# zhizdev/mvdfusion

Hardware: AMD Instinct MI355X
Metric: denoising-steps/sec (higher is better)
Workload: dtype f16x3 (f16 MFMA operands split hi+lo, 3 partial products, fp32 accumulate); 1 GPU; BASELINE.json configs[1]: V=4 views x 256^2 images (32x32 latents), D=1, 50-step DDIM (eta 1), cfg 2.5, SD1.x UNet 320ch + 10 view-aligned transformers + GridAttn, random-init (deterministic fill) weights; views=4, latent=32, depth_samples=1, parallelism=single GPU, CFG pair batched as 2V, hipgraph=True, gemm_tuning=mvdfusion_amd/tuned/gemm_f16.json: 426 problems; 0 problems tuned in this run

## Files before the change

include/mvd_hip.h:

```cpp
#ifndef MVD_HIP_H
#define MVD_HIP_H
#include <stddef.h>
#include <stdint.h>
#ifdef __cplusplus
extern "C" {
#endif

typedef void* mvd_stream_t;

#define MVD_VERSION 100
#define MVD_PREC_X1 1
#define MVD_PREC_X3 3
#define MVD_PREC_X4 4

int mvd_version(void);
const char* mvd_last_error(void);
int mvd_operand_format(void);

size_t mvd_packed_weight_bytes(int N, int K);
int mvd_pack_linear_weight(const float* w, int N, int K, int ldw, int geglu, float scale, void* packed,
                           mvd_stream_t stream);
int mvd_pack_linear_weight_t(const float* wt, int N, int K, int ldw, float scale, void* packed, mvd_stream_t stream);
int mvd_pack_conv3x3_weight(const float* w, int Cout, int Cin, int cin_pad, float scale, void* packed,
                            mvd_stream_t stream);

#define MVD_A_DENSE 0
#define MVD_A_CONV3X3 1

#define MVD_EPI_STORE 0
#define MVD_EPI_GEGLU 1
#define MVD_EPI_QKV 2

#define MVD_ACT_NONE 0
#define MVD_ACT_GELU 1
#define MVD_ACT_SILU 2
#define MVD_ACT_QUICKGELU 3

#define MVD_GEMM_TILES 5
#define MVD_GEMM_LOOPS 8
#define MVD_GEMM_CFG_STRIDE 32
#define MVD_B_PACKED 0
#define MVD_B_PLANES 1

typedef struct mvd_prefetch_item_s {
  const void* ptr;
  unsigned long long bytes;
  int start_after;
  int consumer;
} mvd_prefetch_item;

typedef struct mvd_gemm_desc {
  int M, N, K;
  const void* A;
  int lda;
  int a_mode;
  int B, Hin, Win, Cin, Hout, Wout, stride, upsample;
  int no_pad_tl;
  const void* Wp;
  int b_mode;
  int ldb;
  float acc_scale;
  int prec;
  int epi;
  int act;
  float* out;
  int ldo;
  void* out_sp;
  int ldp;
  int n_store;
  const float* bias;
  const float* bias_b;
  int rows_per_batch;
  int ldbb;
  const float* colscale;
  const float* res;
  int ldr;
  void *q_hi, *q_lo, *k_hi, *k_lo, *vt_hi, *vt_lo;
  int heads, dhead, L, Lpad;
  float qscale;
  int splitk;
  float* workspace;
  size_t workspace_elems;
  int cfg;
  long long* gn_stats;
  int gn_hw, gn_groups;
  float* rs_out;
  int* rs_count;
  int rs_ld;
  const float* ln_stats;
  const int* ln_count;
  const float* ln_colsum;
  int ln_ld, ln_dim;
  float ln_eps;
  void* gna_out_sp;
  const float* gna_gamma;
  const float* gna_beta;
  float gna_eps;
  int gna_flags;
  const float* cat_b;
  int cat_cb;
  void* cat_raw_sp;
  const float* acc_scale_dev;
  const struct mvd_prefetch_item_s* pf_items;
  int pf_n;
  int tap_mode;
  const void* A2;
  int lda2, Cin2;
} mvd_gemm_desc;
#define MVD_TAPS_FULL 0
#define MVD_TAPS_UP4 1
#define MVD_TAPS_CENTRE_TAIL 2
#define MVD_GNA_SILU 1
#define MVD_GNA_ROUND_F16 2
#define MVD_GNA_OUT_UNUSED 4

int mvd_gemm(const mvd_gemm_desc* d, mvd_stream_t stream);
int mvd_gemm_cfg_supported(const mvd_gemm_desc* d, int cfg);

int mvd_split_planes(const float* x, void* sp, size_t rows, int cols, int ldx, int ldp, mvd_stream_t stream);
int mvd_split_planes_scaled(const float* x, void* sp, size_t rows, int cols, int ldx, int ldp, const float* scale_dev, mvd_stream_t stream);

int mvd_gemv(const float* W, const float* bias, const float* x, float* y, int M, int N, int K, int ldx, int ldy,
             int act_in, int act_out, mvd_stream_t stream);

int mvd_groupnorm_chunks(int HW);
int mvd_groupnorm_nhwc(const float* x, void* y_sp, const float* gamma, const float* beta, int B, int HW, int C,
                       int groups, float eps, int silu, double* ws, size_t ws_elems, mvd_stream_t stream);
int mvd_groupnorm_from_stats(const float* x, void* y_sp, const float* gamma, const float* beta, const long long* stats, int B, int HW,
                             int C, int groups, float eps, int silu, mvd_stream_t stream);
int mvd_softmax_rows(const float* x, void* y_sp, int rows, int cols, int ldx, float scale, float out_scale,
                     mvd_stream_t stream);

int mvd_layernorm(const float* x, void* y_sp, float* y_f32, const float* w, const float* b, int rows, int C, float eps,
                  int w_plus_one, mvd_stream_t stream);
int mvd_layernorm_groups(const float* x, void* y_sp, float* y_f32, const float* w, const float* b, int ldw, int rows, int rows_per_group,
                         int C, float eps, int w_plus_one, mvd_stream_t stream);

size_t mvd_attn_qk_plane_elems(int B, int heads, int L, int dhead);
size_t mvd_attn_vt_plane_elems(int B, int heads, int L, int dhead);
int mvd_attn_lpad(int L);
int mvd_attention(const void* q_hi, const void* q_lo, const void* k_hi, const void* k_lo, const void* vt_hi,
                  const void* vt_lo, void* out_sp, int ldo, int B, int heads, int L, int Lkeys, int dhead, int prec,
                  mvd_stream_t stream);

int mvd_pixel_cross_attn(const float* q, const float* k, const float* v, void* out_sp, int P, int D, int heads,
                         int dhead, mvd_stream_t stream);

int mvd_unet_input(const float* x, const float* input_latents, void* out_sp, int V, int S, int cpad, int cfg,
                   mvd_stream_t stream);
int mvd_unet_input_scenes(const float* x, const float* input_latents, void* out_sp, int nscene, int V, int S, int cpad, int cfg,
                          mvd_stream_t stream);
int mvd_concat_channels(const float* a, int Ca, const float* b, int Cb, float* out, void* out_sp, int rows, long long* gn_stats,
                        int gn_hw, int gn_groups, mvd_stream_t stream);
int mvd_concat_groupnorm_fits(int Ca, int Cb, int hw, int groups);
int mvd_concat_groupnorm(const float* a, int Ca, const float* b, int Cb, float* out, void* raw_sp, void* y_sp, const float* gamma,
                         const float* beta, long long* gn_stats, int B, int hw, int groups, float eps, int silu, mvd_stream_t stream);
int mvd_area_pool(const float* vol, void* out_sp, int B, int S, int D, int C, int factor, int ldp, mvd_stream_t stream);
int mvd_fill_zero(float* p, size_t n, mvd_stream_t stream);

#define MVD_STEP_STRIDE 8
int mvd_timestep_embedding(const float* steps, const int* iter, const float* freqs, float* out, int dim,
                           mvd_stream_t stream);
int mvd_timestep_embedding_scenes(const float* steps, const int* iter, const float* freqs, float* out, int dim, int nscene,
                                  int steps_scene_stride, mvd_stream_t stream);
int mvd_advance_iter(int* iter, mvd_stream_t stream);

#define MVD_CAM_RECORD 20
#define MVD_TOKEN_DIM 723
#define MVD_TOKEN_LD 736
int mvd_zembed(const float* lat, const float* w, const float* b, float* feat, int N, int S, mvd_stream_t stream);
int mvd_gridattn_tokens(const float* x, const float* depth_noise, const float* steps, const int* iter,
                        const float* grid_lin ,
                        const float* feat, const float* in_feat, const float* cams, const float* in_cam,
                        void* tokens_sp, int V, int q0, int Vq, int S, int D, float depth_scale, float depth_shift,
                        mvd_stream_t stream);
int mvd_gridattn_tokens_scenes(const float* x, const float* depth_noise, const float* steps, const int* iter, const float* grid_lin,
                               const float* feat, const float* in_feat, const float* cams, const float* in_cam, void* tokens_sp,
                               int nscene, int V, int q0, int Vq, int S, int D, float depth_scale, float depth_shift,
                               mvd_stream_t stream);
int mvd_gridattn_tokens_scenes_t(const float* x, const float* depth_noise, const float* steps, const int* iter, const float* grid_lin,
                                 const float* feat, const float* in_feat, const float* cams, const float* in_cam, void* tokens_sp,
                                 int nscene, int V, int q0, int Vq, int S, int D, float depth_scale, float depth_shift,
                                 int steps_scene_stride, mvd_stream_t stream);
int mvd_gridattn_fused_slots(void);
size_t mvd_gridattn_fused_stream_bytes(void);
size_t mvd_gridattn_fused_vec_floats(void);
int mvd_gridattn_fused(const float* x, const float* depth_noise, const float* steps, const int* iter, const float* grid_lin,
                       const float* feat, const float* in_feat, const float* cams, const float* in_cam, const void* wstream,
                       const float* vecs, void* pooled_sp, int V, int q0, int Vq, int S, int D, float depth_scale,
                       float depth_shift, int prec ,
                       mvd_stream_t stream);
int mvd_gridattn_fused_scenes(const float* x, const float* depth_noise, const float* steps, const int* iter, const float* grid_lin,
                              const float* feat, const float* in_feat, const float* cams, const float* in_cam, const void* wstream,
                              const float* vecs, void* pooled_sp, int nscene, int V, int q0, int Vq, int S, int D, float depth_scale,
                              float depth_shift, int prec, mvd_stream_t stream);
int mvd_gridattn_fused_scenes_t(const float* x, const float* depth_noise, const float* steps, const int* iter, const float* grid_lin,
                                const float* feat, const float* in_feat, const float* cams, const float* in_cam, const void* wstream,
                                const float* vecs, void* pooled_sp, int nscene, int V, int q0, int Vq, int S, int D, float depth_scale,
                                float depth_shift, int prec, int steps_scene_stride, int vecs_scene_stride, mvd_stream_t stream);
int mvd_gridattn_tokens_window(const float* x, const float* depth_noise, const float* steps, const int* iter, const float* grid_lin,
                               const float* feat, const float* in_feat, const float* cams, const float* in_cam, void* tokens_sp,
                               int nscene, int V, int q0, int Vq, int S, int D, float depth_scale, float depth_shift,
                               int steps_scene_stride, int window, mvd_stream_t stream);
int mvd_gridattn_fused_window(const float* x, const float* depth_noise, const float* steps, const int* iter, const float* grid_lin,
                              const float* feat, const float* in_feat, const float* cams, const float* in_cam, const void* wstream,
                              const float* vecs, void* pooled_sp, int nscene, int V, int q0, int Vq, int S, int D, float depth_scale,
                              float depth_shift, int prec, int steps_scene_stride, int vecs_scene_stride, int window,
                              mvd_stream_t stream);
int mvd_view_mha(const float* qkv, void* out_sp, int Nseq, int V, int heads, int dhead,
                 mvd_stream_t stream);
int mvd_view_pool(const float* x, const float* w, const float* b, void* out_sp, int Nseq, int V, int C,
                  mvd_stream_t stream);

int mvd_cfg_ddim_update(const float* eps_nhwc, int ldc, float* x, float* x0, float* eps_out,
                        const float* ddim_noise, size_t noise_stride ,
                        const float* steps, const int* iter, int V, int S, int cfg, float cfg_scale, int do_update,
                        mvd_stream_t stream);

int mvd_pin_views(float* x, float* x0, const float* known, const float* noise, size_t noise_stride ,
                  const float* steps, const int* iter, int groups, int group_views, int K, int S, int mode, mvd_stream_t stream);

#define MVD_FUSE_FOREGROUND 1
#define MVD_FUSE_STAGE_AUTO 0
#define MVD_FUSE_STAGE_GLOBAL 1
#define MVD_FUSE_STAGE_LDS 2
int mvd_fuse_points(const float* lat, const float* rgb, const float* cams, const float* ndc_lin, float* xyz, float* color,
                    uint8_t* support, uint8_t* conflict, uint8_t* flags, int nscene, int V, int S, int up, float depth_scale,
                    float depth_shift, float lo, float hi, float tau, int stage, mvd_stream_t stream);
size_t mvd_compact_points_scratch(size_t npts);
int mvd_compact_points(const float* xyz, const float* color, const uint8_t* support, const uint8_t* conflict, const uint8_t* flags,
                       size_t npts, int min_support, int max_conflicts, float* out_xyz, float* out_color, uint8_t* out_support,
                       int* out_index, unsigned* count, void* scratch, size_t scratch_bytes, mvd_stream_t stream);

#define MVD_SPLAT_MAX_RADIUS 4
#define MVD_RENDER_FILL 1
#define MVD_RENDER_SPLAT 2
#define MVD_RENDER_RESOLVE 4
#define MVD_RENDER_ALL 7
size_t mvd_render_points_scratch(int ncam, int P);
int mvd_render_points(const float* xyz, const float* color, const int* scene_start, const float* cams, size_t n, int nscene, int M, int P,
                      int radius, float znear, float empty_depth, const float* background, int* index, float* depth, float* rgb,
                      void* scratch, size_t scratch_bytes, mvd_stream_t stream);
int mvd_render_points_stages(const float* xyz, const float* color, const int* scene_start, const float* cams, size_t n, int nscene, int M,
                             int P, int radius, float znear, float empty_depth, const float* background, int* index, float* depth,
                             float* rgb, void* scratch, size_t scratch_bytes, int stages, mvd_stream_t stream);

size_t mvd_render_mesh_scratch(int ncam, int P);
int mvd_render_mesh(const float* vertices, const float* colors, const int* faces, const int* vertex_start, const int* face_start,
                    const float* cams, size_t nvert, size_t nface, int nscene, int M, int P, int cull, float znear, float empty_depth,
                    const float* background, int* face_out, float* depth, float* bary, float* normal, float* rgb, void* scratch,
                    size_t scratch_bytes, mvd_stream_t stream);
int mvd_render_mesh_stages(const float* vertices, const float* colors, const int* faces, const int* vertex_start, const int* face_start,
                           const float* cams, size_t nvert, size_t nface, int nscene, int M, int P, int cull, float znear,
                           float empty_depth, const float* background, int* face_out, float* depth, float* bary, float* normal, float* rgb,
                           void* scratch, size_t scratch_bytes, int stages, mvd_stream_t stream);

#define MVD_NN_AUTO 0
#define MVD_NN_BRUTE 1
#define MVD_NN_GRID 2
#define MVD_NN_BUILD 1
#define MVD_NN_QUERY 2
#define MVD_NN_ALL 3
size_t mvd_nearest_points_scratch(size_t nt, int nscene, int method, int grid);
int mvd_nearest_points(const float* query, const int* query_start, const float* target, const int* target_start, size_t nq, size_t nt,
                       int nscene, int method, int grid, int* index, float* dist2, void* scratch, size_t scratch_bytes,
                       mvd_stream_t stream);
int mvd_nearest_points_stages(const float* query, const int* query_start, const float* target, const int* target_start, size_t nq,
                              size_t nt, int nscene, int method, int grid, int* index, float* dist2, void* scratch, size_t scratch_bytes,
                              int stages, mvd_stream_t stream);

#define MVD_KNN_MAX_K 32
#define MVD_NORMALS_MAX_K 256
#define MVD_NORMALS_SWEEPS 10
int mvd_knn_points(const float* query, const int* query_start, const float* target, const int* target_start, size_t nq, size_t nt,
                   int nscene, int k, int method, int grid, int* index, float* dist2, void* scratch, size_t scratch_bytes,
                   mvd_stream_t stream);
int mvd_knn_points_stages(const float* query, const int* query_start, const float* target, const int* target_start, size_t nq, size_t nt,
                          int nscene, int k, int method, int grid, int* index, float* dist2, void* scratch, size_t scratch_bytes,
                          int stages, mvd_stream_t stream);
int mvd_point_normals(const float* target, size_t nt, const int* index, size_t n, int k, const float* points, const float* toward,
                      float* normal, float* variation, mvd_stream_t stream);

#define MVD_ALIGN_SCALE 1
#define MVD_ALIGN_NO_STEP 2
#define MVD_ALIGN_CHUNK 1024
#define MVD_ALIGN_SUMS 19
#define MVD_ALIGN_HISTORY 3
#define MVD_ALIGN_MAX_ITERS 1024
size_t mvd_align_scratch(size_t nq, size_t nt, int nscene, int method, int grid);
int mvd_align_solve(const double* sums, int flags, double* step, double* scale);
int mvd_align_apply(const float* src, const int* src_start, size_t n, int nscene, const double* transform, float* out,
                    mvd_stream_t stream);
int mvd_align_fit(const float* moved, const int* start, const float* target, const int* index, const float* dist2, size_t n, size_t nt,
                  int nscene, int flags, float max_dist2, double* transform, double* history_row, void* scratch, size_t scratch_bytes,
                  mvd_stream_t stream);
int mvd_align_icp(const float* source, const int* source_start, const float* target, const int* target_start, size_t nq, size_t nt,
                  int nscene, int method, int grid, int iters, int flags, float max_dist2, double* transform, double* history,
                  float* moved, int* index, float* dist2, void* scratch, size_t scratch_bytes, mvd_stream_t stream);

#define MVD_PLANE_NO_STEP 2
#define MVD_PLANE_SUMS 30
#define MVD_PLANE_HISTORY 4
#define MVD_PLANE_EPS_RANK 1e-9
size_t mvd_plane_scratch(size_t nq, size_t nt, int nscene, int method, int grid);
int mvd_plane_solve(const double* sums, double* step, int* rank);
int mvd_plane_fit(const float* moved, const int* start, const float* target, const float* normals, const int* index, const float* dist2,
                  size_t n, size_t nt, int nscene, int flags, float max_dist2, double* transform, double* history_row, void* scratch,
                  size_t scratch_bytes, mvd_stream_t stream);
int mvd_plane_icp(const float* source, const int* source_start, const float* target, const int* target_start, const float* normals,
                  size_t nq, size_t nt, int nscene, int method, int grid, int iters, float max_dist2, double* transform, double* history,
                  float* moved, int* index, float* dist2, void* scratch, size_t scratch_bytes, mvd_stream_t stream);

#define MVD_MESH_SPAN 3
size_t mvd_nearest_on_mesh_scratch(size_t nf, int nscene, int method, int grid);
int mvd_nearest_on_mesh(const float* query, const int* query_start, const float* vertices, const int* faces, const int* face_start, size_t nq,
                        size_t nv, size_t nf, int nscene, int method, int grid, int* face, float* dist2, float* point, float* bary,
                        int* region, float* normal, void* scratch, size_t scratch_bytes, mvd_stream_t stream);
int mvd_nearest_on_mesh_stages(const float* query, const int* query_start, const float* vertices, const int* faces, const int* face_start,
                               size_t nq, size_t nv, size_t nf, int nscene, int method, int grid, int* face, float* dist2, float* point,
                               float* bary, int* region, float* normal, void* scratch, size_t scratch_bytes, int stages,
                               mvd_stream_t stream);
size_t mvd_mesh_icp_scratch(size_t nq, size_t nf, int nscene, int method, int grid);
int mvd_mesh_icp(const float* source, const int* source_start, const float* vertices, const int* faces, const int* face_start, size_t nq,
                 size_t nv, size_t nf, int nscene, int method, int grid, int iters, float max_dist2, double* transform, double* history,
                 float* moved, int* face, float* dist2, float* point, float* normal, void* scratch, size_t scratch_bytes,
                 mvd_stream_t stream);

int mvd_tsdf_integrate(const float* lat, const float* rgb, const float* cams, float* tsdf, uint8_t* weight, float* color, uint8_t* cweight,
                       int nscene, int V, int S, int up, int G, float cx, float cy, float cz, float half_extent, float trunc, int carve,
                       float depth_scale, float depth_shift, float lo, float hi, mvd_stream_t stream);
size_t mvd_mesh_scratch(int nscene, int G);
int mvd_mesh_count(const float* tsdf, const uint8_t* weight, int nscene, int G, int* vertex_start, int* face_start, void* scratch,
                   size_t scratch_bytes, mvd_stream_t stream);
int mvd_mesh_emit(const float* tsdf, const uint8_t* weight, const float* color, const uint8_t* cweight, int nscene, int G, float cx, float cy,
                  float cz, float half_extent, const float* fill, float* vertices, float* colors, int* faces, size_t nvert, size_t nface,
                  const void* scratch, size_t scratch_bytes, mvd_stream_t stream);

int mvd_graph_begin(mvd_stream_t stream);
int mvd_graph_end(mvd_stream_t stream, void** graph_exec);
int mvd_graph_launch(void* graph_exec, mvd_stream_t stream);
int mvd_graph_destroy(void* graph_exec);
int mvd_event_create(void** ev);
int mvd_event_record(void* ev, mvd_stream_t stream);
int mvd_event_elapsed_ms(void* start, void* stop, float* ms);
int mvd_event_destroy(void* ev);

int mvd_transpose_planes(const void* x, int src_planes, int rows, int cols, int ldx, void* out_sp, int ldo, mvd_stream_t stream);
int mvd_transpose_planes_scaled(const float* x, int rows, int cols, int ldx, void* out_sp, int ldo, const float* scale_dev,
                                mvd_stream_t stream);
int mvd_im2col3x3_t_planes(const void* x_sp, int B, int H, int W, int Cin, void* out_sp, int ldo, mvd_stream_t stream);
int mvd_pow2_scale(const float* x, size_t n, float* out2, unsigned* scratch2, mvd_stream_t stream);
int mvd_adamw_multi(const void* tensors, int n_tensors, int n_chunks, float lr, float beta1, float beta2, float eps, float weight_decay,
                    float bias_c1, float bias_c2_sqrt, float grad_scale, mvd_stream_t stream);
size_t mvd_col_sum_workspace_doubles(int rows, int cols);
int mvd_col_sum(const float* x, int rows, int cols, int ldx, float* out, double* ws, size_t ws_doubles, mvd_stream_t stream);
int mvd_col_sum_pow2(const float* x, int rows, int cols, int ldx, float* out, double* ws, size_t ws_doubles, float* out2, unsigned* scratch1,
                     mvd_stream_t stream);
int mvd_groupnorm_backward(const float* x, const float* dy, const float* gamma, const float* beta, int B, int HW, int C, int groups,
                           float eps, int silu, float* dx, float* dgamma, float* dbeta, float* ws, size_t ws_floats,
                           mvd_stream_t stream);

int mvd_layernorm_backward(const float* x, const float* dy, const float* w, int rows, int C, float eps, float* dx, float* dyxhat,
                           mvd_stream_t stream);
size_t mvd_col_sum_groups_workspace_doubles(int ngroups, int rows_per_group, int cols);
int mvd_col_sum_groups(const float* x, int ngroups, int rows_per_group, int cols, int ldx, float* out, double* ws, size_t ws_doubles,
                       mvd_stream_t stream);
int mvd_layernorm_backward_groups(const float* x, const float* dy, const float* w, int ldw, int rows, int rows_per_group, int C, float eps,
                                  float* dx, float* dyxhat, float* dw, float* db, double* ws, size_t ws_doubles, mvd_stream_t stream);
int mvd_act_planes(const float* x, void* sp, float* y, size_t rows, int cols, int ldx, int ldp, int ldy, int act, mvd_stream_t stream);
int mvd_act_backward(const float* dy, const float* x, float* dx, size_t n, int act, mvd_stream_t stream);
int mvd_geglu_backward(const float* h, const float* dy, int rows, int half, float* dh, mvd_stream_t stream);
int mvd_attention_backward(const float* q, const float* k, const float* v, const float* dout, int B, int heads, int L, int dhead,
                           float* dq, float* dk, float* dv, float* stats, size_t stats_floats, mvd_stream_t stream);
int mvd_pixel_cross_attn_backward(const float* q, const float* k, const float* v, const float* dout, int P, int D, int heads, int dhead,
                                  float* dq, float* dk, float* dv, mvd_stream_t stream);

int mvd_gridattn_tokens_backward(const float* x, const float* depth_noise, const float* steps, const int* iter, const float* grid_lin,
                                 const float* cams, const float* in_cam, const float* dtok, int ldt, long long* dfeat_acc,
                                 long long* din_feat_acc, float scale, int V, int q0, int Vq, int S, int D, float depth_scale,
                                 float depth_shift, mvd_stream_t stream);
int mvd_gridattn_tokens_backward_scenes(const float* x, const float* depth_noise, const float* steps, const int* iter, const float* grid_lin,
                                        const float* cams, const float* in_cam, const float* dtok, int ldt, long long* dfeat_acc,
                                        long long* din_feat_acc, float scale, int nscene, int V, int q0, int Vq, int S, int D,
                                        float depth_scale, float depth_shift, int steps_scene_stride, mvd_stream_t stream);
int mvd_gridattn_tokens_backward_window(const float* x, const float* depth_noise, const float* steps, const int* iter, const float* grid_lin,
                                        const float* cams, const float* in_cam, const float* dtok, int ldt, long long* dfeat_acc,
                                        long long* din_feat_acc, float scale, int nscene, int V, int q0, int Vq, int S, int D,
                                        float depth_scale, float depth_shift, int steps_scene_stride, int window, mvd_stream_t stream);

#ifdef __cplusplus
}
#endif
#endif
```

mvdfusion_amd/csrc/elementwise.hip:

```cpp
#include "common.hpp"
#include "../../include/mvd_hip.h"

namespace {

__device__ __forceinline__ float act_apply(float v, int act) {
  if (act == MVD_ACT_GELU) return gelu_erf(v);
  if (act == MVD_ACT_SILU) return silu_f(v);
  return v;
}

template <int MR>
__global__ __launch_bounds__(256) void gemv_kernel(const float* __restrict__ W, const float* __restrict__ bias,
                                                   const float* __restrict__ x, float* __restrict__ y, int M, int N, int K, int ldx,
                                                   int ldy, int act_in, int act_out) {
  const int lane = threadIdx.x & 63;
  const int n = blockIdx.x * 4 + (threadIdx.x >> 6);
  if (n >= N) return;
  float acc[MR];
#pragma unroll
  for (int m = 0; m < MR; ++m) acc[m] = 0.f;
  const float* wr = W + (size_t)n * K;
  if ((K & 3) == 0) {
    for (int k = lane * 4; k < K; k += 256) {
      const float4 w4 = *(const float4*)(wr + k);
#pragma unroll
      for (int m = 0; m < MR; ++m) {
        if (m < M) {
          float4 x4 = *(const float4*)(x + (size_t)m * ldx + k);
          if (act_in) {
            x4.x = act_apply(x4.x, act_in);
            x4.y = act_apply(x4.y, act_in);
            x4.z = act_apply(x4.z, act_in);
            x4.w = act_apply(x4.w, act_in);
          }
          acc[m] += w4.x * x4.x + w4.y * x4.y + w4.z * x4.z + w4.w * x4.w;
        }
      }
    }
  } else {
    for (int k = lane; k < K; k += 64) {
      const float w1 = wr[k];
#pragma unroll
      for (int m = 0; m < MR; ++m)
        if (m < M) acc[m] += w1 * act_apply(x[(size_t)m * ldx + k], act_in);
    }
  }
#pragma unroll
  for (int m = 0; m < MR; ++m) {
    if (m < M) {
      float v = wave_sum(acc[m]);
      if (lane == 0) {
        if (bias) v += bias[n];
        y[(size_t)m * ldy + n] = act_apply(v, act_out);
      }
    }
  }
}

__global__ __launch_bounds__(256) void unet_input_kernel(const float* __restrict__ x, const float* __restrict__ il,
                                                         u16* __restrict__ out_sp, int V, int Vs, int S, int cpad, int nb) {
  const int SS = S * S;
  const size_t total = (size_t)nb * SS * cpad;
  for (size_t e = (size_t)blockIdx.x * 256 + threadIdx.x; e < total; e += (size_t)gridDim.x * 256) {
    const int c = (int)(e % cpad);
    const int pix = (int)((e / cpad) % SS);
    const int b = (int)(e / ((size_t)cpad * SS));
    const int v = b < V ? b : b - V;
    float o = 0.f;
    if (c < 5) {
      o = x[((size_t)v * 5 + c) * SS + pix];
    } else if (c < 10 && b < V) {
      const float t = il[((size_t)(b / Vs) * 5 + (c - 5)) * SS + pix];
      o = (c < 9) ? t / 0.18215f : t;
    }
    store_sp1(out_sp, e / cpad, cpad, c, o);
  }
}

__global__ __launch_bounds__(256) void concat_kernel(const float4* __restrict__ a, int ca4, const float4* __restrict__ b, int cb4,
                                                     float4* __restrict__ out, u16* __restrict__ out_sp, size_t rows) {
  const int c4 = ca4 + cb4;
  const size_t total = rows * c4;
  for (size_t e = (size_t)blockIdx.x * 256 + threadIdx.x; e < total; e += (size_t)gridDim.x * 256) {
    const size_t r = e / c4;
    const int c = (int)(e - r * c4);
    const float4 v = c < ca4 ? a[r * ca4 + c] : b[r * cb4 + (c - ca4)];
    out[e] = v;
    if (out_sp) store_sp4(out_sp, r, c4 * 4, c * 4, v.x, v.y, v.z, v.w);
  }
}

__global__ __launch_bounds__(256) void concat_stats_kernel(const float4* __restrict__ a, int ca4, const float4* __restrict__ b, int cb4,
                                                           float4* __restrict__ out, u16* __restrict__ out_sp, long long* __restrict__ stats,
                                                           int hw, int groups) {
  __shared__ float cs[2][4][256];
  const int c4n = ca4 + cb4, C = c4n * 4;
  const size_t m0 = (size_t)blockIdx.x * 16;
  const int n0 = blockIdx.y * 256;
  const int c4 = blockIdx.y * 64 + (threadIdx.x & 63), rg = threadIdx.x >> 6;
  float4 s = make_float4(0.f, 0.f, 0.f, 0.f), q = make_float4(0.f, 0.f, 0.f, 0.f);
  if (c4 < c4n) {
    float4 v[4];
#pragma unroll
    for (int r = 0; r < 4; ++r) {
      const size_t row = m0 + rg * 4 + r;
      v[r] = c4 < ca4 ? a[row * ca4 + c4] : b[row * cb4 + (c4 - ca4)];
    }
#pragma unroll
    for (int r = 0; r < 4; ++r) {
      const size_t row = m0 + rg * 4 + r;
      out[row * c4n + c4] = v[r];
      if (out_sp) store_sp4(out_sp, row, C, c4 * 4, v[r].x, v[r].y, v[r].z, v[r].w);
      s.x += v[r].x; s.y += v[r].y; s.z += v[r].z; s.w += v[r].w;
      q.x += v[r].x * v[r].x; q.y += v[r].y * v[r].y; q.z += v[r].z * v[r].z; q.w += v[r].w * v[r].w;
    }
  }
  *(float4*)&cs[0][rg][(threadIdx.x & 63) * 4] = s;
  *(float4*)&cs[1][rg][(threadIdx.x & 63) * 4] = q;
  __syncthreads();
  const int c = threadIdx.x, nn = n0 + c;
  const float cs_ = cs[0][0][c] + cs[0][1][c] + cs[0][2][c] + cs[0][3][c];
  const float cq_ = cs[1][0][c] + cs[1][1][c] + cs[1][2][c] + cs[1][3][c];
  __syncthreads();
  cs[0][0][c] = cs_;
  cs[1][0][c] = cq_;
  __syncthreads();
  if (nn >= C) return;
  const int cg = C / groups;
  const int g = nn / cg, pos = nn - g * cg;
  if (c != 0 && pos != 0) return;
  int len = cg - pos;
  if (len > 256 - c) len = 256 - c;
  float ss = 0.f, qq = 0.f;
  for (int j = 0; j < len; ++j) {
    ss += cs[0][0][c + j];
    qq += cs[1][0][c + j];
  }
  gn_stats_add(stats, (int)(m0 / hw), g, groups, ss, qq);
}

#define MVD_CGN_THREADS 1024
__global__ __launch_bounds__(MVD_CGN_THREADS) void concat_gn_kernel(const float* __restrict__ a, int ca, const float* __restrict__ b, int cb,
                                                                    float* __restrict__ out, u16* __restrict__ raw_sp, u16* __restrict__ y_sp,
                                                                    const float* __restrict__ gamma, const float* __restrict__ beta,
                                                                    long long* __restrict__ stats, int hw, int groups, float eps, int flags) {
  constexpr int NT = MVD_CGN_THREADS, NWV = NT / 64, U = 4;
  extern __shared__ float s_val[];
  __shared__ double s_red[2][NWV];
  __shared__ float s_coef[2][128];
  const int C = ca + cb, cg = C / groups, cg2 = cg >> 1;
  int g, img;
  {
    const int bid = blockIdx.x;
    if ((groups & 7) == 0) {
      const int gpx = groups >> 3, x = bid & 7, r = bid >> 3;
      g = x * gpx + r % gpx;
      img = r / gpx;
    } else {
      g = bid % groups;
      img = bid / groups;
    }
  }
  const int tid = threadIdx.x, lane = tid & 63, wave = tid >> 6;
  const int c0 = g * cg;
  const size_t m0 = (size_t)img * hw;
  const int total = hw * cg2;
  const int dq = NT / cg2, dj = NT - dq * cg2;
  const int rs = tid / cg2, js = tid - rs * cg2;
  const int r0 = tid < total ? rs : 0, j0 = tid < total ? js : 0;
  float s = 0.f, q = 0.f;
  {
    int r = rs, j = js;
    for (int e0 = tid; e0 < total; e0 += NT * U) {
      float2 v[U];
      int rr[U], jj[U];
      bool ok[U];
#pragma unroll
      for (int u = 0; u < U; ++u) {
        ok[u] = e0 + u * NT < total;
        rr[u] = ok[u] ? r : r0;
        jj[u] = ok[u] ? j : j0;
        r += dq;
        j += dj;
        if (j >= cg2) {
          j -= cg2;
          ++r;
        }
      }
#pragma unroll
      for (int u = 0; u < U; ++u) {
        const size_t m = m0 + rr[u];
        const int n = c0 + 2 * jj[u];
        v[u] = *(const float2*)(n < ca ? a + m * ca + n : b + m * cb + (n - ca));
      }
#pragma unroll
      for (int u = 0; u < U; ++u) {
        if (ok[u]) {
          const size_t m = m0 + rr[u];
          const int n = c0 + 2 * jj[u];
          if (out) *(float2*)(out + m * C + n) = v[u];
          if (raw_sp) {
            uint32_t hh, ll;
            split_op16x2(v[u].x, v[u].y, hh, ll);
            u16* pp = raw_sp + sp_index(m, C, n);
            *(uint32_t*)pp = hh;
            *(uint32_t*)(pp + 32) = ll;
          }
          *(float2*)(s_val + 2 * (e0 + u * NT)) = v[u];
          s += v[u].x + v[u].y;
          q += v[u].x * v[u].x + v[u].y * v[u].y;
        }
      }
    }
  }
  {
    const double sd = wave_sum_d((double)s), qd = wave_sum_d((double)q);
    if (lane == 0) {
      s_red[0][wave] = sd;
      s_red[1][wave] = qd;
    }
  }
  __syncthreads();
  double S1 = 0.0, S2 = 0.0;
#pragma unroll
  for (int w = 0; w < NWV; ++w) {
    S1 += s_red[0][w];
    S2 += s_red[1][w];
  }
  const double cnt = (double)hw * cg;
  const double mean = S1 / cnt;
  double var = S2 / cnt - mean * mean;
  if (var < 0.0) var = 0.0;
  const float rstd = (float)(1.0 / sqrt(var + (double)eps));
  if (tid < cg) {
    const float aa = rstd * gamma[c0 + tid];
    s_coef[0][tid] = aa;
    s_coef[1][tid] = beta[c0 + tid] - (float)mean * aa;
  }
  if (tid == 0 && stats) gn_stats_add(stats, img, g, groups, (float)S1, (float)S2);
  __syncthreads();
  {
    int r = rs, j = js;
    for (int e = tid; e < total; e += NT) {
      float2 v = *(const float2*)(s_val + 2 * e);
      v.x = v.x * s_coef[0][2 * j] + s_coef[1][2 * j];
      v.y = v.y * s_coef[0][2 * j + 1] + s_coef[1][2 * j + 1];
      if (flags & 2) {
        v.x = (float)(_Float16)v.x;
        v.y = (float)(_Float16)v.y;
      }
      if (flags & 1) {
        v.x = silu_f(v.x);
        v.y = silu_f(v.y);
      }
      uint32_t hh, ll;
      split_op16x2(v.x, v.y, hh, ll);
      u16* pp = y_sp + sp_index(m0 + r, C, c0 + 2 * j);
      *(uint32_t*)pp = hh;
      *(uint32_t*)(pp + 32) = ll;
      r += dq;
      j += dj;
      if (j >= cg2) {
        j -= cg2;
        ++r;
      }
    }
  }
}

__global__ __launch_bounds__(256) void area_pool_kernel(const float4* __restrict__ vol, u16* __restrict__ out_sp, int B, int S,
                                                        int D, int C4, int f, int ldp) {
  const int So = S / f;
  const size_t total = (size_t)B * So * So * D * C4;
  const float inv = 1.0f / (float)(f * f);
  for (size_t e = (size_t)blockIdx.x * 256 + threadIdx.x; e < total; e += (size_t)gridDim.x * 256) {
    const int c = (int)(e % C4);
    size_t r = e / C4;
    const int d = (int)(r % D);
    r /= D;
    const int ox = (int)(r % So);
    r /= So;
    const int oy = (int)(r % So);
    const int b = (int)(r / So);
    float4 acc = make_float4(0.f, 0.f, 0.f, 0.f);
    for (int dy = 0; dy < f; ++dy)
#pragma unroll 8
      for (int dx = 0; dx < f; ++dx) {
        const float4 v = vol[((((size_t)b * S + oy * f + dy) * S + ox * f + dx) * D + d) * C4 + c];
        acc.x += v.x;
        acc.y += v.y;
        acc.z += v.z;
        acc.w += v.w;
      }
    store_sp4(out_sp, e / C4, ldp, c * 4, acc.x * inv, acc.y * inv, acc.z * inv, acc.w * inv);
  }
}

__global__ __launch_bounds__(256) void fill_zero_kernel(float* p, size_t n) {
  for (size_t e = (size_t)blockIdx.x * 256 + threadIdx.x; e < n; e += (size_t)gridDim.x * 256) p[e] = 0.f;
}

__global__ void timestep_embedding_kernel(const float* __restrict__ steps, const int* __restrict__ iter,
                                          const float* __restrict__ freqs, float* __restrict__ out, int dim, int steps_scene_stride) {
  const float t = steps[((size_t)iter[0] + (size_t)blockIdx.x * steps_scene_stride) * MVD_STEP_STRIDE + 0];
  out += (size_t)blockIdx.x * dim;
  const int half = dim / 2;
  for (int i = threadIdx.x; i < half; i += blockDim.x) {
    const float a = t * freqs[i];
    out[i] = cosf(a);
    out[half + i] = sinf(a);
  }
}

__global__ void advance_iter_kernel(int* iter) {
  if (threadIdx.x == 0) iter[0] += 1;
}

__global__ __launch_bounds__(256) void cfg_ddim_kernel(const float* __restrict__ eps_nhwc, int ldc, float* __restrict__ x,
                                                       float* __restrict__ x0, float* __restrict__ eps_out,
                                                       const float* __restrict__ noise, const float* __restrict__ steps,
                                                       const int* __restrict__ iter, int V, int S, int cfg, float cfg_scale,
                                                       int do_update, size_t noise_stride) {
  const int it = iter[0];
  const float* st = steps + (size_t)it * MVD_STEP_STRIDE;
  const float a_t = st[3], a_prev = st[4], sigma = st[5], s1m = st[6], has_noise = st[7];
  const int SS = S * S;
  const size_t total = (size_t)V * 5 * SS;
  for (size_t e = (size_t)blockIdx.x * 256 + threadIdx.x; e < total; e += (size_t)gridDim.x * 256) {
    const int pix = (int)(e % SS);
    const int c = (int)((e / SS) % 5);
    const int b = (int)(e / ((size_t)5 * SS));
    float ep = eps_nhwc[((size_t)b * SS + pix) * ldc + c];
    if (cfg) {
      const float eu = eps_nhwc[((size_t)(V + b) * SS + pix) * ldc + c];
      ep = eu + cfg_scale * (ep - eu);
    }
    if (eps_out) eps_out[e] = ep;
    if (do_update) {
      const float xv = x[e];
      const float px0 = (xv - s1m * ep) / sqrtf(a_t);
      const float dir = sqrtf(fmaxf(1.0f - a_prev - sigma * sigma, 1e-7f)) * ep;
      float xp = sqrtf(a_prev) * px0 + dir;
      if (has_noise != 0.f) xp = xp + sigma * noise[(size_t)it * noise_stride + e];
      x0[e] = px0;
      x[e] = xp;
    }
  }
}

template <typename T>
__device__ __forceinline__ T pin_axpy(float sa, const T& k, float s1, const T& n);
template <>
__device__ __forceinline__ float pin_axpy<float>(float sa, const float& k, float s1, const float& n) {
  return sa * k + s1 * n;
}
template <>
__device__ __forceinline__ float4 pin_axpy<float4>(float sa, const float4& k, float s1, const float4& n) {
  return make_float4(sa * k.x + s1 * n.x, sa * k.y + s1 * n.y, sa * k.z + s1 * n.z, sa * k.w + s1 * n.w);
}

template <typename T>
__global__ __launch_bounds__(256) void pin_views_kernel(T* __restrict__ x, T* __restrict__ x0, const T* __restrict__ known,
                                                        const T* __restrict__ noise, size_t nstride, const float* __restrict__ steps,
                                                        const int* __restrict__ iter, int group_views, int K, size_t rowlen, size_t total,
                                                        int mode) {
  float sa = 1.f, s1 = 0.f;
  size_t nbase = 0;
  if (mode == 1) {
    const int it = iter[0];
    const float* st = steps + (size_t)it * MVD_STEP_STRIDE;
    sa = st[1];
    s1 = st[6];
    nbase = (size_t)it * nstride;
  }
  for (size_t e = (size_t)blockIdx.x * 256 + threadIdx.x; e < total; e += (size_t)gridDim.x * 256) {
    const size_t p = e / rowlen;
    const size_t off = e - p * rowlen;
    const size_t dst = ((p / K) * group_views + p % K) * rowlen + off;
    const T kv = known[e];
    if (mode == 1) {
      x[dst] = pin_axpy<T>(sa, kv, s1, noise[nbase + e]);
      x0[dst] = kv;
    } else {
      x[dst] = kv;
    }
  }
}

inline int grid_for(size_t total, int cap = 2048) {
  size_t b = (total + 255) / 256;
  if (b > (size_t)cap) b = cap;
  if (b < 1) b = 1;
  return (int)b;
}

}

extern "C" int mvd_gemv(const float* W, const float* bias, const float* x, float* y, int M, int N, int K, int ldx, int ldy,
                        int act_in, int act_out, mvd_stream_t stream) {
  MVD_CHECK_ARG(W && x && y && M > 0 && M <= 16 && N > 0 && K > 0, "mvd_gemv: bad arguments (M <= 16)");
  if ((K & 3) == 0) MVD_CHECK_ARG((ldx & 3) == 0, "mvd_gemv: ldx must be a multiple of 4 when K is");
  hipStream_t s = (hipStream_t)stream;
  dim3 grid(cdiv(N, 4)), block(256);
  if (M <= 1)
    hipLaunchKernelGGL(gemv_kernel<1>, grid, block, 0, s, W, bias, x, y, M, N, K, ldx, ldy, act_in, act_out);
  else if (M <= 4)
    hipLaunchKernelGGL(gemv_kernel<4>, grid, block, 0, s, W, bias, x, y, M, N, K, ldx, ldy, act_in, act_out);
  else
    hipLaunchKernelGGL(gemv_kernel<16>, grid, block, 0, s, W, bias, x, y, M, N, K, ldx, ldy, act_in, act_out);
  MVD_CHECK_LAUNCH("mvd_gemv");
  return 0;
}

extern "C" int mvd_unet_input_scenes(const float* x, const float* input_latents, void* out_sp, int nscene, int V, int S, int cpad, int cfg,
                                     mvd_stream_t stream) {
  MVD_CHECK_ARG(x && input_latents && out_sp && cpad % 32 == 0 && V > 0 && S > 0 && cpad >= 10, "mvd_unet_input: bad arguments");
  MVD_CHECK_ARG(nscene >= 1 && (long long)nscene * V <= 0x3fffffff, "mvd_unet_input_scenes: nscene=%d (>= 1)", nscene);
  const int NV = nscene * V;
  const int nb = cfg ? 2 * NV : NV;
  const size_t total = (size_t)nb * S * S * cpad;
  hipLaunchKernelGGL(unet_input_kernel, dim3(grid_for(total)), dim3(256), 0, (hipStream_t)stream, x, input_latents, (u16*)out_sp, NV, V,
                     S, cpad, nb);
  MVD_CHECK_LAUNCH("mvd_unet_input");
  return 0;
}

extern "C" int mvd_unet_input(const float* x, const float* input_latents, void* out_sp, int V, int S, int cpad, int cfg,
                              mvd_stream_t stream) {
  return mvd_unet_input_scenes(x, input_latents, out_sp, 1, V, S, cpad, cfg, stream);
}

extern "C" int mvd_concat_channels(const float* a, int Ca, const float* b, int Cb, float* out, void* out_sp, int rows,
                                   long long* gn_stats, int gn_hw, int gn_groups, mvd_stream_t stream) {
  if (out_sp) MVD_CHECK_ARG((Ca + Cb) % 32 == 0, "mvd_concat_channels: split-planes output needs (Ca+Cb) %% 32 == 0");
  MVD_CHECK_ARG(a && b && out && rows > 0 && Ca > 0 && Cb > 0 && Ca % 4 == 0 && Cb % 4 == 0,
                "mvd_concat_channels: bad arguments (channel counts must be multiples of 4)");
  if (gn_stats) {
    MVD_CHECK_ARG(rows % 16 == 0 && gn_hw > 0 && gn_hw % 16 == 0 && gn_groups > 0 && (Ca + Cb) % gn_groups == 0,
                  "mvd_concat_channels: gn_stats needs rows %% 16 == 0, gn_hw %% 16 == 0, C %% groups == 0");
    hipLaunchKernelGGL(concat_stats_kernel, dim3(rows / 16, (Ca + Cb + 255) / 256), dim3(256), 0, (hipStream_t)stream, (const float4*)a, Ca / 4,
                       (const float4*)b, Cb / 4, (float4*)out, (u16*)out_sp, gn_stats, gn_hw, gn_groups);
    MVD_CHECK_LAUNCH("mvd_concat_channels/stats");
    return 0;
  }
  const size_t total = (size_t)rows * (Ca + Cb) / 4;
  hipLaunchKernelGGL(concat_kernel, dim3(grid_for(total)), dim3(256), 0, (hipStream_t)stream, (const float4*)a, Ca / 4,
                     (const float4*)b, Cb / 4, (float4*)out, (u16*)out_sp, (size_t)rows);
  MVD_CHECK_LAUNCH("mvd_concat_channels");
  return 0;
}

extern "C" int mvd_concat_groupnorm_fits(int Ca, int Cb, int hw, int groups) {
  const int C = Ca + Cb;
  if (groups <= 0 || C % groups || (Ca & 1) || (Cb & 1)) return 0;
  const int cg = C / groups;
  return (cg & 1) == 0 && cg <= 128 && (size_t)hw * cg * 4 <= 128 * 1024 ? 1 : 0;
}

extern "C" int mvd_concat_groupnorm(const float* a, int Ca, const float* b, int Cb, float* out, void* raw_sp, void* y_sp, const float* gamma,
                                    const float* beta, long long* gn_stats, int B, int hw, int groups, float eps, int silu,
                                    mvd_stream_t stream) {
  MVD_CHECK_ARG(a && b && y_sp && gamma && beta && B > 0 && hw > 0, "mvd_concat_groupnorm: null pointer / bad shape");
  MVD_CHECK_ARG((Ca + Cb) % 32 == 0 && mvd_concat_groupnorm_fits(Ca, Cb, hw, groups),
                "mvd_concat_groupnorm: needs (Ca+Cb) %% 32 == 0, even Ca / Cb / group width <= 128 and hw * (C / groups) * 4 <= 128 KiB of LDS "
                "(Ca=%d Cb=%d hw=%d groups=%d): use mvd_concat_channels + mvd_groupnorm_from_stats", Ca, Cb, hw, groups);
  MVD_CHECK_ARG(((uintptr_t)a & 7) == 0 && ((uintptr_t)b & 7) == 0 && ((uintptr_t)out & 7) == 0 && ((uintptr_t)y_sp & 127) == 0 &&
                    ((uintptr_t)raw_sp & 127) == 0, "mvd_concat_groupnorm: alignment");
  const size_t lds = (size_t)hw * ((Ca + Cb) / groups) * 4;
  {
    static unsigned long long raised = 0;
    const hipError_t e = mvd_raise_dynamic_lds((const void*)concat_gn_kernel, 128 * 1024, &raised);
    MVD_CHECK_ARG(e == hipSuccess, "mvd_concat_groupnorm: hipFuncSetAttribute(MaxDynamicSharedMemorySize): %s", hipGetErrorString(e));
  }
  hipLaunchKernelGGL(concat_gn_kernel, dim3(B * groups), dim3(MVD_CGN_THREADS), lds, (hipStream_t)stream, a, Ca, b, Cb, out, (u16*)raw_sp,
                     (u16*)y_sp, gamma, beta, gn_stats, hw, groups, eps, silu);
  MVD_CHECK_LAUNCH("mvd_concat_groupnorm");
  return 0;
}

extern "C" int mvd_area_pool(const float* vol, void* out_sp, int B, int S, int D, int C, int factor, int ldp,
                             mvd_stream_t stream) {
  MVD_CHECK_ARG(vol && out_sp && C % 32 == 0 && B > 0 && S > 0 && D > 0 && C % 4 == 0 && factor >= 1 && S % factor == 0,
                "mvd_area_pool: bad arguments");
  if (ldp == 0) ldp = C;
  MVD_CHECK_ARG(ldp >= C && ldp % 32 == 0 && ((uintptr_t)out_sp & 127) == 0, "mvd_area_pool: ldp=%d must be >= C, %% 32 == 0", ldp);
  const int So = S / factor;
  const size_t total = (size_t)B * So * So * D * (C / 4);
  hipLaunchKernelGGL(area_pool_kernel, dim3(grid_for(total)), dim3(256), 0, (hipStream_t)stream, (const float4*)vol,
                     (u16*)out_sp, B, S, D, C / 4, factor, ldp);
  MVD_CHECK_LAUNCH("mvd_area_pool");
  return 0;
}

extern "C" int mvd_fill_zero(float* p, size_t n, mvd_stream_t stream) {
  MVD_CHECK_ARG(p != nullptr, "mvd_fill_zero: null pointer");
  if (n == 0) return 0;
  hipLaunchKernelGGL(fill_zero_kernel, dim3(grid_for(n)), dim3(256), 0, (hipStream_t)stream, p, n);
  MVD_CHECK_LAUNCH("mvd_fill_zero");
  return 0;
}

extern "C" int mvd_timestep_embedding(const float* steps, const int* iter, const float* freqs, float* out, int dim,
                                      mvd_stream_t stream) {
  MVD_CHECK_ARG(steps && iter && freqs && out && dim > 0 && dim % 2 == 0, "mvd_timestep_embedding: bad arguments");
  hipLaunchKernelGGL(timestep_embedding_kernel, dim3(1), dim3(256), 0, (hipStream_t)stream, steps, iter, freqs, out, dim, 0);
  MVD_CHECK_LAUNCH("mvd_timestep_embedding");
  return 0;
}

extern "C" int mvd_timestep_embedding_scenes(const float* steps, const int* iter, const float* freqs, float* out, int dim, int nscene,
                                             int steps_scene_stride, mvd_stream_t stream) {
  MVD_CHECK_ARG(steps && iter && freqs && out && dim > 0 && dim % 2 == 0, "mvd_timestep_embedding: bad arguments");
  MVD_CHECK_ARG(nscene >= 1 && nscene <= 65535 && steps_scene_stride >= 0 && (nscene > 1 || steps_scene_stride == 0),
                "mvd_timestep_embedding_scenes: nscene=%d (1 ... 65535), steps_scene_stride=%d (>= 0; 0 when nscene = 1)", nscene,
                steps_scene_stride);
  hipLaunchKernelGGL(timestep_embedding_kernel, dim3(nscene), dim3(256), 0, (hipStream_t)stream, steps, iter, freqs, out, dim,
                     steps_scene_stride);
  MVD_CHECK_LAUNCH("mvd_timestep_embedding_scenes");
  return 0;
}

extern "C" int mvd_advance_iter(int* iter, mvd_stream_t stream) {
  MVD_CHECK_ARG(iter != nullptr, "mvd_advance_iter: null pointer");
  hipLaunchKernelGGL(advance_iter_kernel, dim3(1), dim3(64), 0, (hipStream_t)stream, iter);
  MVD_CHECK_LAUNCH("mvd_advance_iter");
  return 0;
}

extern "C" int mvd_cfg_ddim_update(const float* eps_nhwc, int ldc, float* x, float* x0, float* eps_out,
                                   const float* ddim_noise, size_t noise_stride, const float* steps, const int* iter, int V,
                                   int S, int cfg, float cfg_scale, int do_update, mvd_stream_t stream) {
  MVD_CHECK_ARG(eps_nhwc && steps && iter && V > 0 && S > 0 && ldc >= 5, "mvd_cfg_ddim_update: bad arguments");
  if (do_update) MVD_CHECK_ARG(x && x0 && ddim_noise, "mvd_cfg_ddim_update: update needs x, x0, ddim_noise");
  const size_t total = (size_t)V * 5 * S * S;
  hipLaunchKernelGGL(cfg_ddim_kernel, dim3(grid_for(total)), dim3(256), 0, (hipStream_t)stream, eps_nhwc, ldc, x, x0, eps_out,
                     ddim_noise, steps, iter, V, S, cfg, cfg_scale, do_update, noise_stride);
  MVD_CHECK_LAUNCH("mvd_cfg_ddim_update");
  return 0;
}

extern "C" int mvd_pin_views(float* x, float* x0, const float* known, const float* noise, size_t noise_stride, const float* steps,
                             const int* iter, int groups, int group_views, int K, int S, int mode, mvd_stream_t stream) {
  MVD_CHECK_ARG(x && known && groups > 0 && group_views > 0 && S > 0 && (mode == 0 || mode == 1),
                "mvd_pin_views: bad arguments (null x / known, groups=%d, group_views=%d, S=%d, mode=%d)", groups, group_views, S, mode);
  MVD_CHECK_ARG(K > 0 && K <= group_views, "mvd_pin_views: K=%d pinned views of a %d-view group (0 < K <= group_views)", K, group_views);
  MVD_CHECK_ARG((long long)groups * group_views <= 0x3fffffff, "mvd_pin_views: groups * group_views too large");
  const size_t row = (size_t)5 * S * S;
  if (mode == 1)
    MVD_CHECK_ARG(x0 && noise && steps && iter && noise_stride >= (size_t)groups * K * row,
                  "mvd_pin_views: mode 1 needs x0, noise, steps, iter and noise_stride >= groups * K * 5 * S * S");
  const size_t total = (size_t)groups * K * row;
  hipStream_t s = (hipStream_t)stream;
  if (((size_t)S * S) % 4 == 0) {
    MVD_CHECK_ARG(((uintptr_t)x & 15) == 0 && ((uintptr_t)known & 15) == 0, "mvd_pin_views: x / known must be 16-byte aligned");
    if (mode == 1)
      MVD_CHECK_ARG(((uintptr_t)x0 & 15) == 0 && ((uintptr_t)noise & 15) == 0 && noise_stride % 4 == 0,
                    "mvd_pin_views: x0 / noise must be 16-byte aligned and noise_stride a multiple of 4");
    hipLaunchKernelGGL(pin_views_kernel<float4>, dim3(grid_for(total / 4)), dim3(256), 0, s, (float4*)x, (float4*)x0, (const float4*)known,
                       (const float4*)noise, noise_stride / 4, steps, iter, group_views, K, row / 4, total / 4, mode);
  } else {
    hipLaunchKernelGGL(pin_views_kernel<float>, dim3(grid_for(total)), dim3(256), 0, s, x, x0, known, noise, noise_stride, steps, iter,
                       group_views, K, row, total, mode);
  }
  MVD_CHECK_LAUNCH("mvd_pin_views");
  return 0;
}
```

mvdfusion_amd/engine.py:

```python
import os

import torch

from . import hip


GN_SLOTS = 256
GN_SLOT_ELEMS = 64 * 32 * 2


class Workspace:

    def __init__(self, device):
        self.device = torch.device(device)
        self.bufs = {}
        self.frozen = False

    def get(self, tag, shape, dtype=torch.float32, zero=False):
        key = (tag, tuple(int(s) for s in shape), dtype)
        t = self.bufs.get(key)
        if t is None:
            assert not self.frozen, f"workspace buffer {key} requested during graph capture (the eager warm-up step must " \
                                    "allocate every buffer the captured step uses)"
            t = (torch.zeros if zero else torch.empty)(key[1], dtype=dtype, device=self.device)
            self.bufs[key] = t
        return t

    def planes(self, tag, rows, cols):
        assert cols % 32 == 0, (tag, cols)
        return self.get(tag, (rows, 2 * cols), torch.int16)

    def attn_planes(self, B, heads, L, dhead):
        key = ("attn_planes", B, heads, L, dhead)
        t = self.bufs.get(key)
        if t is None:
            assert not self.frozen, f"attention planes {key} requested during graph capture"
            t = hip.alloc_attn_planes(B, heads, L, dhead, self.device)
            self.bufs[key] = t
        return t

    def nbytes(self):
        n = 0
        for v in self.bufs.values():
            for t in (v if isinstance(v, tuple) else (v,)):
                n += t.numel() * t.element_size()
        return n


class Ctx:
    gn_from_producer = True
    ln_fold = True
    gn_fuse = True

    def __init__(self, device, prec=hip.PREC_X4, policy=None):
        self.device = torch.device(device)
        self.ws = Workspace(device)
        self.prec = prec
        self.policy = dict(policy or {})
        self.B = 0
        self.D = 1
        self.context = None
        self.vol_levels = None
        self.emb_bias = None
        self._rot = {}
        self.capturing = False
        self.gemm_ws = torch.empty(64 * 1024 * 1024, dtype=torch.float32, device=self.device)
        self.gn_arena = torch.zeros(GN_SLOTS * GN_SLOT_ELEMS, dtype=torch.int64, device=self.device)
        self._gn_next = 0
        self._gn = {}
        self._rs = {}
        self.next_gn = None
        self._gn_done = {}
        self._unwritten = set()
        self.next_cat = None
        self._cat_done = set()
        self.keep_fp32 = False

    def begin_step(self):
        self._rot.clear()
        self._gn.clear()
        self._gn_done.clear()
        self._unwritten.clear()
        self._cat_done.clear()
        self.next_gn = None
        self.next_cat = None
        self._gn_next = 0
        if self.gn_from_producer:
            hip.check(hip.lib().mvd_fill_zero(hip.ptr(self.gn_arena), self.gn_arena.numel() * 2, hip.stream()))

    def gn_slot(self, out, B, HW, C):
        n = B * 32 * 2
        if n > GN_SLOT_ELEMS or self._gn_next >= GN_SLOTS:
            return None
        st = self.gn_arena[self._gn_next * GN_SLOT_ELEMS:self._gn_next * GN_SLOT_ELEMS + n]
        self._gn_next += 1
        self._gn[out.data_ptr()] = (st, B, HW, C)
        return st

    def _forget(self, out):
        ptr = out.data_ptr()
        self._gn.pop(ptr, None)
        self._unwritten.discard(ptr)
        if self._gn_done:
            for k in [k for k in self._gn_done if k[0] == ptr]:
                del self._gn_done[k]

    def row_stats(self, tag, rows, width):
        key = (tag, int(rows), int(width))
        rs = self._rs.get(key)
        if rs is None:
            assert not self.ws.frozen, f"row statistics {key} requested during graph capture"
            rs = hip.RowStats(rows, width, self.device)
            self._rs[key] = rs
        return rs

    def act(self, shape):
        key = tuple(int(s) for s in shape)
        i = self._rot.get(key, 0)
        self._rot[key] = (i + 1) % 3
        return self.ws.get(f"act{i}", key)

    def prec_of(self, kind):
        return self.policy.get(kind, self.prec)

    def ln_fold_enabled(self):
        return (self.ln_fold and hip.OPERAND_FORMAT == "f16" and self.prec_of("qkv") >= hip.PREC_X3 and
                self.prec_of("geglu") >= hip.PREC_X3 and self.prec_of("proj") >= hip.PREC_X3)

    def gemm(self, A, W, out, gn=None, kind=None, gn_apply=None, **kw):
        kw.setdefault("prec", self.prec_of(kind))
        kw.setdefault("workspace", self.gemm_ws)
        applied = False
        if out is not None:
            self._forget(out)
            handled = False
            if gn is not None and gn_apply is None and self.next_cat is not None and self.gn_fuse and self.gn_from_producer and \
                    gn[1] % 16 == 0 and out.is_contiguous():
                sk, cat, catp, norm, pname, silu = self.next_cat
                N, cb = out.shape[-1], sk.shape[-1]
                if norm.num_groups == 32 and norm.num_channels == N + cb and sk.shape[0] == out.shape[0] == gn[0] * gn[1] and \
                        sk.is_contiguous() and hip.lib().mvd_concat_groupnorm_fits(N, cb, gn[1], 32):
                    st = self.gn_slot(cat, gn[0], gn[1], N + cb)
                    if st is not None:
                        planes = self.ws.planes(pname, out.shape[0], N + cb)
                        kw.update(gn_stats=st, gn_hw=gn[1], gn_groups=32, cat=(sk, catp),
                                  gn_apply=(norm.weight, norm.bias, norm.eps, (hip.GNA_SILU if silu else 0) | hip.GNA_OUT_UNUSED, planes))
                        self._gn.pop(cat.data_ptr(), None)
                        self._gn_done[(cat.data_ptr(), id(norm))] = (planes, bool(silu))
                        self._unwritten.add(cat.data_ptr())
                        self._unwritten.add(out.data_ptr())
                        self._cat_done.add(cat.data_ptr())
                        handled = True
            if not handled and gn is not None and self.gn_from_producer and gn[1] % 16 == 0 and out.shape[-1] % 32 == 0:
                st = self.gn_slot(out, gn[0], gn[1], out.shape[-1])
                if st is not None:
                    kw.update(gn_stats=st, gn_hw=gn[1], gn_groups=32)
                    if gn_apply is not None and self.gn_fuse and gn_apply[0].num_groups == 32 and out.is_contiguous():
                        norm, planes, silu, unused = gn_apply
                        kw["gn_apply"] = (norm.weight, norm.bias, norm.eps, (hip.GNA_SILU if silu else 0) | (hip.GNA_OUT_UNUSED if unused else 0),
                                          planes)
                        applied = True
                    elif gn_apply is None and self.next_gn is not None and self.gn_fuse and out.is_contiguous():
                        norm, pname, silu = self.next_gn
                        if norm.num_groups == 32 and norm.num_channels == out.shape[-1] and out.shape[0] == gn[0] * gn[1]:
                            planes = self.ws.planes(pname, out.shape[0], out.shape[-1])
                            kw["gn_apply"] = (norm.weight, norm.bias, norm.eps, hip.GNA_SILU if silu else 0, planes)
                            self._gn_done[(out.data_ptr(), id(norm))] = (planes, bool(silu))
        if gn is not None:
            if os.environ.get("MVD_GN_DEBUG") and not self.capturing:
                print(f"[gn] kind={kind} M={out.shape[0]} N={out.shape[-1]} explicit={gn_apply is not None} hint={self.next_gn is not None} "
                      f"cat={self.next_cat is not None} -> fused_apply={'gn_apply' in kw} cat={'cat' in kw}", flush=True)
            if gn_apply is None:
                self.next_gn = None
                self.next_cat = None
        r = hip.gemm(A, W, out, **kw)
        if gn_apply is not None and not applied:
            self.groupnorm(out, gn_apply[1], gn_apply[0], gn[0], gn[1], out.shape[-1], gn_apply[2])
        return r

    def groupnorm(self, x, y, norm, B, HW, C, silu):
        done = self._gn_done.pop((x.data_ptr(), id(norm)), None)
        if done is not None and done[0].data_ptr() == y.data_ptr() and done[0].shape == y.shape and done[1] == bool(silu) and silu in (True, False):
            return y
        if x.data_ptr() in self._unwritten:
            raise RuntimeError("GroupNorm of a tensor whose fused producer left the fp32 data unwritten (Ctx.concat(need_out=False))")
        ent = self._gn.get(x.data_ptr())
        if ent is not None and ent[1:] == (B, HW, C) and norm.num_groups == 32:
            return hip.groupnorm_from_stats(x, y, norm.weight, norm.bias, ent[0], B, HW, C, norm.eps, silu)
        ws = self.ws.get("gn_ws", (B * hip.lib().mvd_groupnorm_chunks(HW) * 32 * 2,), torch.float64)
        return hip.groupnorm(x, y, norm.weight, norm.bias, B, HW, C, norm.eps, silu, ws)

    def concat(self, a, ca, b, cb, out, out_planes, B, HW, gn_apply=None, need_out=True):
        self._forget(out)
        st = None
        if gn_apply is not None and self.gn_fuse and self.gn_from_producer and HW % 16 == 0 and (ca + cb) % 32 == 0 and \
                gn_apply[0].num_groups == 32 and gn_apply[0].num_channels == ca + cb and \
                hip.lib().mvd_concat_groupnorm_fits(ca, cb, HW, 32):
            norm, pname, silu = gn_apply
            st = self.gn_slot(out, B, HW, ca + cb)
            planes = self.ws.planes(pname, B * HW, ca + cb)
            hip.check(hip.lib().mvd_concat_groupnorm(hip.ptr(a), ca, hip.ptr(b), cb, hip.ptr(out) if need_out else None, hip.ptr(out_planes),
                                                     hip.ptr(planes), hip.ptr(norm.weight), hip.ptr(norm.bias),
                                                     hip.ptr(st) if st is not None else None, B, HW, 32, norm.eps, 1 if silu else 0,
                                                     hip.stream()))
            if not need_out:
                self._gn.pop(out.data_ptr(), None)
                self._unwritten.add(out.data_ptr())
            self._gn_done[(out.data_ptr(), id(norm))] = (planes, bool(silu))
            return out
        if self.gn_from_producer and HW % 16 == 0 and (ca + cb) % 32 == 0:
            st = self.gn_slot(out, B, HW, ca + cb)
        hip.check(hip.lib().mvd_concat_channels(hip.ptr(a), ca, hip.ptr(b), cb, hip.ptr(out), hip.ptr(out_planes), B * HW,
                                                hip.ptr(st) if st is not None else None, HW, 32, hip.stream()))
        return out

    def layernorm(self, x, y, norm, rows, C):
        return hip.layernorm(x, y, norm.weight, norm.bias, rows, C, norm.eps)

    def gemv_rows(self, W, bias, x, y, act_in=hip.ACT_NONE, act_out=hip.ACT_NONE):
        for r in range(0, x.shape[0], 16):
            hip.gemv(W, bias, x[r:r + 16], y[r:r + 16], act_in, act_out)
        return y


def ddim_step_table(scheduler_tables, ddim, iters):
    rows = []
    for index in iters:
        t = int(ddim["timesteps"][index])
        sac = float(scheduler_tables["sqrt_alphas_cumprod"][t])
        s1m = float(scheduler_tables["sqrt_one_minus_alphas_cumprod"][t])
        dstd = (scheduler_tables["sqrt_one_minus_alphas_cumprod"][t] / scheduler_tables["sqrt_alphas_cumprod"][t] / 10.0)
        rows.append([float(t), sac, float(dstd), float(ddim["alphas"][index]), float(ddim["alphas_prev"][index]),
                     float(ddim["sigmas"][index]), float(ddim["sqrt_one_minus_alphas"][index]),
                     1.0 if index > 0 else 0.0])
        del s1m
    return torch.tensor(rows, dtype=torch.float32)
```

mvdfusion_amd/hip.py:

```python
import ctypes as C
import os

import torch

_HERE = os.path.dirname(os.path.abspath(__file__))
LIB_PATHS = {"f16": os.path.join(_HERE, "csrc", "libmvd_hip.so"), "bf16": os.path.join(_HERE, "csrc", "libmvd_hip_bf16.so")}
if os.environ.get("MVD_HIP_LIB"):
    LIB_PATHS["f16"] = os.environ["MVD_HIP_LIB"]
LIB_PATH = LIB_PATHS["f16"]
OPERAND_FORMAT = os.environ.get("MVD_OPERAND_FORMAT", "f16")

PREC_X1, PREC_X3, PREC_X4 = 1, 3, 4
PREC_KINDS = ("conv", "skip", "proj", "qkv", "attn", "out", "geglu", "ffproj", "xattn", "ga")


def parse_precision(name):
    base, _, over = name.partition(":")
    names = {"f16": ("f16", PREC_X1), "bf16": ("bf16", PREC_X1), "f16x3": ("f16", PREC_X3), "f16x4": ("f16", PREC_X4),
             "bf16x3": ("bf16", PREC_X3), "bf16x4": ("bf16", PREC_X4)}
    if base not in names:
        raise ValueError(f"precision '{name}': base must be one of {sorted(names)}")
    fmt, default = names[base]
    policy = {}
    for item in filter(None, over.split(",")):
        k, _, v = item.partition("=")
        k = k.strip()
        if k not in PREC_KINDS or int(v) not in (PREC_X1, PREC_X3, PREC_X4):
            raise ValueError(f"precision policy '{name}': '{item}' is not <kind>=<1|3|4> with kind in {PREC_KINDS}")
        policy[k] = int(v)
    return fmt, default, policy
A_DENSE, A_CONV3X3 = 0, 1
TAPS_FULL, TAPS_CENTRE_TAIL = 0, 2
TAPS_UP4 = 1
EPI_STORE, EPI_GEGLU, EPI_QKV = 0, 1, 2
ACT_NONE, ACT_GELU, ACT_SILU, ACT_QUICKGELU = 0, 1, 2, 3
STEP_STRIDE = 8
CAM_RECORD = 20
TOKEN_DIM, TOKEN_LD = 723, 736
FUSE_FOREGROUND = 1
FUSE_STAGE_AUTO, FUSE_STAGE_GLOBAL, FUSE_STAGE_LDS = 0, 1, 2
SPLAT_MAX_RADIUS = 4
RENDER_FILL, RENDER_SPLAT, RENDER_RESOLVE, RENDER_ALL = 1, 2, 4, 7
NN_AUTO, NN_BRUTE, NN_GRID = 0, 1, 2
NN_BUILD, NN_QUERY, NN_ALL = 1, 2, 3
NN_MAX_GRID = 256
KNN_MAX_K = 32
NORMALS_MAX_K, NORMALS_SWEEPS = 256, 10
ALIGN_SCALE, ALIGN_NO_STEP = 1, 2
ALIGN_CHUNK = 1024
ALIGN_SUMS, ALIGN_HISTORY = 19, 3
PLANE_NO_STEP = 2
PLANE_SUMS, PLANE_HISTORY = 30, 4
PLANE_EPS_RANK = 1e-9
ALIGN_MAX_ITERS = 1024
MESH_SPAN = 3

_vp, _i, _f, _sz = C.c_void_p, C.c_int, C.c_float, C.c_size_t
c_void_p = C.c_void_p


class GemmDesc(C.Structure):
    _fields_ = [
        ("M", _i), ("N", _i), ("K", _i),
        ("A", _vp), ("lda", _i), ("a_mode", _i),
        ("B", _i), ("Hin", _i), ("Win", _i), ("Cin", _i), ("Hout", _i), ("Wout", _i), ("stride", _i), ("upsample", _i), ("no_pad_tl", _i),
        ("Wp", _vp), ("b_mode", _i), ("ldb", _i), ("acc_scale", _f), ("prec", _i),
        ("epi", _i), ("act", _i), ("out", _vp), ("ldo", _i), ("out_sp", _vp), ("ldp", _i),
        ("n_store", _i),
        ("bias", _vp), ("bias_b", _vp), ("rows_per_batch", _i), ("ldbb", _i), ("colscale", _vp), ("res", _vp), ("ldr", _i),
        ("q_hi", _vp), ("q_lo", _vp), ("k_hi", _vp), ("k_lo", _vp), ("vt_hi", _vp), ("vt_lo", _vp),
        ("heads", _i), ("dhead", _i), ("L", _i), ("Lpad", _i), ("qscale", _f),
        ("splitk", _i), ("workspace", _vp), ("workspace_elems", _sz), ("cfg", _i),
        ("gn_stats", _vp), ("gn_hw", _i), ("gn_groups", _i),
        ("rs_out", _vp), ("rs_count", _vp), ("rs_ld", _i),
        ("ln_stats", _vp), ("ln_count", _vp), ("ln_colsum", _vp), ("ln_ld", _i), ("ln_dim", _i), ("ln_eps", _f),
        ("gna_out_sp", _vp), ("gna_gamma", _vp), ("gna_beta", _vp), ("gna_eps", _f), ("gna_flags", _i),
        ("cat_b", _vp), ("cat_cb", _i), ("cat_raw_sp", _vp),
        ("acc_scale_dev", _vp), ("pf_items", _vp), ("pf_n", _i),
        ("tap_mode", _i), ("A2", _vp), ("lda2", _i), ("Cin2", _i),
    ]


class PrefetchItem(C.Structure):
    _fields_ = [("ptr", _vp), ("bytes", C.c_ulonglong), ("start_after", _i), ("consumer", _i)]


SIGNATURES = {
    "mvd_version": (_i, []),
    "mvd_last_error": (C.c_char_p, []),
    "mvd_packed_weight_bytes": (_sz, [_i, _i]),
    "mvd_operand_format": (_i, []),
    "mvd_pack_linear_weight": (_i, [_vp, _i, _i, _i, _i, _f, _vp, _vp]),
    "mvd_pack_linear_weight_t": (_i, [_vp, _i, _i, _i, _f, _vp, _vp]),
    "mvd_pack_conv3x3_weight": (_i, [_vp, _i, _i, _i, _f, _vp, _vp]),
    "mvd_gemm": (_i, [C.POINTER(GemmDesc), _vp]),
    "mvd_gemm_cfg_supported": (_i, [C.POINTER(GemmDesc), _i]),
    "mvd_split_planes": (_i, [_vp, _vp, _sz, _i, _i, _i, _vp]),
    "mvd_gemv": (_i, [_vp, _vp, _vp, _vp, _i, _i, _i, _i, _i, _i, _i, _vp]),
    "mvd_groupnorm_chunks": (_i, [_i]),
    "mvd_groupnorm_nhwc": (_i, [_vp, _vp, _vp, _vp, _i, _i, _i, _i, _f, _i, _vp, _sz, _vp]),
    "mvd_layernorm": (_i, [_vp, _vp, _vp, _vp, _vp, _i, _i, _f, _i, _vp]),
    "mvd_layernorm_groups": (_i, [_vp, _vp, _vp, _vp, _vp, _i, _i, _i, _i, _f, _i, _vp]),
    "mvd_softmax_rows": (_i, [_vp, _vp, _i, _i, _i, _f, _f, _vp]),
    "mvd_attn_qk_plane_elems": (_sz, [_i, _i, _i, _i]),
    "mvd_attn_vt_plane_elems": (_sz, [_i, _i, _i, _i]),
    "mvd_attn_lpad": (_i, [_i]),
    "mvd_attention": (_i, [_vp] * 7 + [_i, _i, _i, _i, _i, _i, _i, _vp]),
    "mvd_pixel_cross_attn": (_i, [_vp, _vp, _vp, _vp, _i, _i, _i, _i, _vp]),
    "mvd_unet_input": (_i, [_vp, _vp, _vp, _i, _i, _i, _i, _vp]),
    "mvd_unet_input_scenes": (_i, [_vp, _vp, _vp, _i, _i, _i, _i, _i, _vp]),
    "mvd_concat_channels": (_i, [_vp, _i, _vp, _i, _vp, _vp, _i, _vp, _i, _i, _vp]),
    "mvd_concat_groupnorm_fits": (_i, [_i, _i, _i, _i]),
    "mvd_concat_groupnorm": (_i, [_vp, _i, _vp, _i, _vp, _vp, _vp, _vp, _vp, _vp, _i, _i, _i, _f, _i, _vp]),
    "mvd_transpose_planes": (_i, [_vp, _i, _i, _i, _i, _vp, _i, _vp]),
    "mvd_im2col3x3_t_planes": (_i, [_vp, _i, _i, _i, _i, _vp, _i, _vp]),
    "mvd_col_sum_workspace_doubles": (_sz, [_i, _i]),
    "mvd_col_sum": (_i, [_vp, _i, _i, _i, _vp, _vp, _sz, _vp]),
    "mvd_col_sum_groups_workspace_doubles": (_sz, [_i, _i, _i]),
    "mvd_col_sum_groups": (_i, [_vp, _i, _i, _i, _i, _vp, _vp, _sz, _vp]),
    "mvd_col_sum_pow2": (_i, [_vp, _i, _i, _i, _vp, _vp, _sz, _vp, _vp, _vp]),
    "mvd_gridattn_tokens_backward": (_i, [_vp, _vp, _vp, _vp, _vp, _vp, _vp, _vp, _i, _vp, _vp, _f, _i, _i, _i, _i, _i, _f, _f, _vp]),
    "mvd_gridattn_tokens_backward_scenes": (_i, [_vp, _vp, _vp, _vp, _vp, _vp, _vp, _vp, _i, _vp, _vp, _f, _i, _i, _i, _i, _i, _i, _f, _f, _i,
                                                 _vp]),
    "mvd_gridattn_tokens_backward_window": (_i, [_vp, _vp, _vp, _vp, _vp, _vp, _vp, _vp, _i, _vp, _vp, _f, _i, _i, _i, _i, _i, _i, _f, _f, _i,
                                                 _i, _vp]),
    "mvd_layernorm_backward": (_i, [_vp, _vp, _vp, _i, _i, _f, _vp, _vp, _vp]),
    "mvd_layernorm_backward_groups": (_i, [_vp, _vp, _vp, _i, _i, _i, _i, _f, _vp, _vp, _vp, _vp, _vp, _sz, _vp]),
    "mvd_geglu_backward": (_i, [_vp, _vp, _i, _i, _vp, _vp]),
    "mvd_act_planes": (_i, [_vp, _vp, _vp, _sz, _i, _i, _i, _i, _i, _vp]),
    "mvd_act_backward": (_i, [_vp, _vp, _vp, _sz, _i, _vp]),
    "mvd_attention_backward": (_i, [_vp, _vp, _vp, _vp, _i, _i, _i, _i, _vp, _vp, _vp, _vp, _sz, _vp]),
    "mvd_pixel_cross_attn_backward": (_i, [_vp, _vp, _vp, _vp, _i, _i, _i, _i, _vp, _vp, _vp, _vp]),
    "mvd_groupnorm_backward": (_i, [_vp, _vp, _vp, _vp, _i, _i, _i, _i, _f, _i, _vp, _vp, _vp, _vp, _sz, _vp]),
    "mvd_groupnorm_from_stats": (_i, [_vp, _vp, _vp, _vp, _vp, _i, _i, _i, _i, _f, _i, _vp]),
    "mvd_area_pool": (_i, [_vp, _vp, _i, _i, _i, _i, _i, _i, _vp]),
    "mvd_fill_zero": (_i, [_vp, _sz, _vp]),
    "mvd_pow2_scale": (_i, [_vp, _sz, _vp, _vp, _vp]),
    "mvd_split_planes_scaled": (_i, [_vp, _vp, _sz, _i, _i, _i, _vp, _vp]),
    "mvd_transpose_planes_scaled": (_i, [_vp, _i, _i, _i, _vp, _i, _vp, _vp]),
    "mvd_adamw_multi": (_i, [_vp, _i, _i, _f, _f, _f, _f, _f, _f, _f, _f, _vp]),
    "mvd_timestep_embedding": (_i, [_vp, _vp, _vp, _vp, _i, _vp]),
    "mvd_timestep_embedding_scenes": (_i, [_vp, _vp, _vp, _vp, _i, _i, _i, _vp]),
    "mvd_advance_iter": (_i, [_vp, _vp]),
    "mvd_zembed": (_i, [_vp, _vp, _vp, _vp, _i, _i, _vp]),
    "mvd_gridattn_tokens": (_i, [_vp] * 10 + [_i, _i, _i, _i, _i, _f, _f, _vp]),
    "mvd_gridattn_tokens_scenes": (_i, [_vp] * 10 + [_i, _i, _i, _i, _i, _i, _f, _f, _vp]),
    "mvd_gridattn_tokens_scenes_t": (_i, [_vp] * 10 + [_i, _i, _i, _i, _i, _i, _f, _f, _i, _vp]),
    "mvd_gridattn_fused_slots": (_i, []),
    "mvd_gridattn_fused_stream_bytes": (_sz, []),
    "mvd_gridattn_fused_vec_floats": (_sz, []),
    "mvd_gridattn_fused": (_i, [_vp] * 12 + [_i, _i, _i, _i, _i, _f, _f, _i, _vp]),
    "mvd_gridattn_fused_scenes": (_i, [_vp] * 12 + [_i, _i, _i, _i, _i, _i, _f, _f, _i, _vp]),
    "mvd_gridattn_fused_scenes_t": (_i, [_vp] * 12 + [_i, _i, _i, _i, _i, _i, _f, _f, _i, _i, _i, _vp]),
    "mvd_gridattn_tokens_window": (_i, [_vp] * 10 + [_i, _i, _i, _i, _i, _i, _f, _f, _i, _i, _vp]),
    "mvd_gridattn_fused_window": (_i, [_vp] * 12 + [_i, _i, _i, _i, _i, _i, _f, _f, _i, _i, _i, _i, _vp]),
    "mvd_view_mha": (_i, [_vp, _vp, _i, _i, _i, _i, _vp]),
    "mvd_view_pool": (_i, [_vp, _vp, _vp, _vp, _i, _i, _i, _vp]),
    "mvd_cfg_ddim_update": (_i, [_vp, _i, _vp, _vp, _vp, _vp, _sz, _vp, _vp, _i, _i, _i, _f, _i, _vp]),
    "mvd_pin_views": (_i, [_vp, _vp, _vp, _vp, _sz, _vp, _vp, _i, _i, _i, _i, _i, _vp]),
    "mvd_fuse_points": (_i, [_vp] * 9 + [_i, _i, _i, _i, _f, _f, _f, _f, _f, _i, _vp]),
    "mvd_compact_points_scratch": (_sz, [_sz]),
    "mvd_compact_points": (_i, [_vp] * 5 + [_sz, _i, _i, _vp, _vp, _vp, _vp, _vp, _vp, _sz, _vp]),
    "mvd_render_points_scratch": (_sz, [_i, _i]),
    "mvd_render_points": (_i, [_vp] * 4 + [_sz, _i, _i, _i, _i, _f, _f, C.POINTER(_f), _vp, _vp, _vp, _vp, _sz, _vp]),
    "mvd_render_points_stages": (_i, [_vp] * 4 + [_sz, _i, _i, _i, _i, _f, _f, C.POINTER(_f), _vp, _vp, _vp, _vp, _sz, _i, _vp]),
    "mvd_render_mesh_scratch": (_sz, [_i, _i]),
    "mvd_render_mesh": (_i, [_vp] * 6 + [_sz, _sz, _i, _i, _i, _i, _f, _f, C.POINTER(_f)] + [_vp] * 6 + [_sz, _vp]),
    "mvd_render_mesh_stages": (_i, [_vp] * 6 + [_sz, _sz, _i, _i, _i, _i, _f, _f, C.POINTER(_f)] + [_vp] * 6 + [_sz, _i, _vp]),
    "mvd_nearest_points_scratch": (_sz, [_sz, _i, _i, _i]),
    "mvd_nearest_points": (_i, [_vp] * 4 + [_sz, _sz, _i, _i, _i, _vp, _vp, _vp, _sz, _vp]),
    "mvd_nearest_points_stages": (_i, [_vp] * 4 + [_sz, _sz, _i, _i, _i, _vp, _vp, _vp, _sz, _i, _vp]),
    "mvd_knn_points": (_i, [_vp] * 4 + [_sz, _sz, _i, _i, _i, _i, _vp, _vp, _vp, _sz, _vp]),
    "mvd_knn_points_stages": (_i, [_vp] * 4 + [_sz, _sz, _i, _i, _i, _i, _vp, _vp, _vp, _sz, _i, _vp]),
    "mvd_point_normals": (_i, [_vp, _sz, _vp, _sz, _i, _vp, _vp, _vp, _vp, _vp]),
    "mvd_align_scratch": (_sz, [_sz, _sz, _i, _i, _i]),
    "mvd_align_solve": (_i, [_vp, _i, _vp, _vp]),
    "mvd_align_apply": (_i, [_vp, _vp, _sz, _i, _vp, _vp, _vp]),
    "mvd_align_fit": (_i, [_vp] * 5 + [_sz, _sz, _i, _i, _f, _vp, _vp, _vp, _sz, _vp]),
    "mvd_align_icp": (_i, [_vp] * 4 + [_sz, _sz, _i, _i, _i, _i, _i, _f] + [_vp] * 6 + [_sz, _vp]),
    "mvd_plane_scratch": (_sz, [_sz, _sz, _i, _i, _i]),
    "mvd_plane_solve": (_i, [_vp, _vp, _vp]),
    "mvd_plane_fit": (_i, [_vp] * 6 + [_sz, _sz, _i, _i, _f, _vp, _vp, _vp, _sz, _vp]),
    "mvd_plane_icp": (_i, [_vp] * 5 + [_sz, _sz, _i, _i, _i, _i, _f] + [_vp] * 6 + [_sz, _vp]),
    "mvd_nearest_on_mesh_scratch": (_sz, [_sz, _i, _i, _i]),
    "mvd_nearest_on_mesh": (_i, [_vp] * 5 + [_sz, _sz, _sz, _i, _i, _i] + [_vp] * 7 + [_sz, _vp]),
    "mvd_nearest_on_mesh_stages": (_i, [_vp] * 5 + [_sz, _sz, _sz, _i, _i, _i] + [_vp] * 7 + [_sz, _i, _vp]),
    "mvd_mesh_icp_scratch": (_sz, [_sz, _sz, _i, _i, _i]),
    "mvd_mesh_icp": (_i, [_vp] * 5 + [_sz, _sz, _sz, _i, _i, _i, _i, _f] + [_vp] * 8 + [_sz, _vp]),
    "mvd_tsdf_integrate": (_i, [_vp] * 7 + [_i, _i, _i, _i, _i, _f, _f, _f, _f, _f, _i, _f, _f, _f, _f, _vp]),
    "mvd_mesh_scratch": (_sz, [_i, _i]),
    "mvd_mesh_count": (_i, [_vp, _vp, _i, _i, _vp, _vp, _vp, _sz, _vp]),
    "mvd_mesh_emit": (_i, [_vp] * 4 + [_i, _i, _f, _f, _f, _f, C.POINTER(_f), _vp, _vp, _vp, _sz, _sz, _vp, _sz, _vp]),
    "mvd_graph_begin": (_i, [_vp]),
    "mvd_graph_end": (_i, [_vp, C.POINTER(_vp)]),
    "mvd_graph_launch": (_i, [_vp, _vp]),
    "mvd_graph_destroy": (_i, [_vp]),
    "mvd_event_create": (_i, [C.POINTER(_vp)]),
    "mvd_event_record": (_i, [_vp, _vp]),
    "mvd_event_elapsed_ms": (_i, [_vp, _vp, C.POINTER(_f)]),
    "mvd_event_destroy": (_i, [_vp]),
}

_lib = None


def lib():
    global _lib
    if _lib is None:
        path = LIB_PATHS[OPERAND_FORMAT]
        if not os.path.exists(path):
            raise RuntimeError(
                f"{path} not found: build it with `python -m mvdfusion_amd.csrc.build` "
                "(or `python -c 'import __graft_entry__ as g; g.build()'`). mvdfusion_amd has no CPU fallback.")
        l = C.CDLL(path)
        for name, (res, args) in SIGNATURES.items():
            fn = getattr(l, name)
            fn.restype, fn.argtypes = res, args
        assert l.mvd_operand_format() == {"f16": 0xf16, "bf16": 0xbf16}[OPERAND_FORMAT]
        _lib = l
        load_default_tuned()
    return _lib


def set_operand_format(fmt):
    global OPERAND_FORMAT
    assert fmt in LIB_PATHS
    if _lib is not None and fmt != OPERAND_FORMAT:
        raise RuntimeError(f"operand format already fixed to {OPERAND_FORMAT} for this process")
    OPERAND_FORMAT = fmt


def check(rc):
    if rc != 0:
        raise RuntimeError(f"mvd_hip error {rc}: {lib().mvd_last_error().decode()}")


try:
    _raw_stream = torch._C._cuda_getCurrentRawStream
    _cur_device = torch._C._cuda_getDevice
except AttributeError:
    _raw_stream = None


def stream():
    if _raw_stream is not None:
        return C.c_void_p(_raw_stream(_cur_device()))
    return C.c_void_p(torch.cuda.current_stream().cuda_stream)


def ptr(t):
    if t is None:
        return None
    return C.c_void_p(t.data_ptr())


def _req(t, dtype=torch.float32):
    assert t.is_cuda and t.dtype == dtype and t.is_contiguous(), (t.device, t.dtype, t.shape, t.stride())
    return t


class PackedWeight:

    __slots__ = ("data", "N", "K", "n_real", "bias", "geglu", "conv_cin", "acc_scale", "tail_cin", "up4")

    def __init__(self, data, N, K, n_real, bias, geglu=False, conv_cin=0, acc_scale=1.0, tail_cin=0, up4=False):
        self.data, self.N, self.K, self.n_real, self.bias, self.geglu, self.conv_cin = data, N, K, n_real, bias, geglu, conv_cin
        self.acc_scale = acc_scale
        self.tail_cin = tail_cin
        self.up4 = up4


class RowStats:

    __slots__ = ("slots", "count", "ld")

    def __init__(self, rows, n_max, device):
        self.ld = (n_max + 31) // 32
        self.slots = torch.zeros(rows, self.ld, 2, dtype=torch.float32, device=device)
        self.count = torch.zeros(1, dtype=torch.int32, device=device)


class LnFold:

    __slots__ = ("w", "colsum", "dim", "eps")

    def __init__(self, weight, bias, norm, geglu=False):
        Wd = weight.detach().double()
        g, b = norm.weight.detach().double(), norm.bias.detach().double()
        Wf = Wd * g[None, :]
        bf = Wd @ b + (bias.detach().double() if bias is not None else 0.0)
        self.w = pack_linear(Wf.float().contiguous(), bf.float().contiguous(), geglu=geglu)
        Np = self.w.N if not geglu else Wd.shape[0]
        cs = torch.zeros(max(Np, Wd.shape[0]), dtype=torch.float32, device=weight.device)
        cs[:Wd.shape[0]] = Wf.sum(dim=1).float()
        self.colsum, self.dim, self.eps = cs, int(Wd.shape[1]), float(norm.eps)


class PlanesOperand:

    __slots__ = ("data", "N", "K", "n_real", "bias", "geglu", "conv_cin", "acc_scale", "ld")

    def __init__(self, planes, N=None, K=None, bias=None, acc_scale=1.0, ld=None):
        assert planes.dtype == torch.int16 and planes.dim() == 2
        self.data, self.ld = planes, int(ld if ld is not None else planes.shape[-1] // 2)
        self.N = int(N if N is not None else planes.shape[0])
        self.K = int(K if K is not None else self.ld)
        assert self.N % 16 == 0 and self.K % 32 == 0 and self.K <= self.ld, (self.N, self.K, self.ld)
        self.n_real, self.bias, self.geglu, self.conv_cin, self.acc_scale = self.N, bias, False, 0, acc_scale


_PARAM_MAX = {}


def register_param_maxima(params):
    import weakref
    ps = [p for p in params if p.dtype == torch.float32 and p.numel() > 0]
    _PARAM_MAX.clear()
    if not ps:
        return 0
    with torch.no_grad():
        try:
            norms = torch._foreach_norm([p.detach().reshape(-1) for p in ps], float("inf"))
        except Exception:
            norms = [torch.linalg.vector_norm(p.detach().reshape(-1), ord=float("inf")) for p in ps]
        vals = torch.stack([n.reshape(()) for n in norms]).tolist()
    for p, v in zip(ps, vals):
        _PARAM_MAX[p.data_ptr()] = (weakref.ref(p), p.numel(), float(v), p._version)
    return len(ps)


def forget_param_maxima():
    _PARAM_MAX.clear()


def _known_max(t):
    ent = _PARAM_MAX.get(t.data_ptr())
    if ent is None:
        return None
    ref, numel, mx, version = ent
    p = ref()
    if p is None or p.data_ptr() != t.data_ptr() or numel != t.numel() or p._version != version:
        return None
    return mx


def _pack_scale(w, like=None):
    import math
    mx = None
    srcs = [w] if like is None else (list(like) if isinstance(like, (list, tuple)) else [like])
    known = [_known_max(s.detach()) for s in srcs]
    if all(k is not None for k in known):
        mx = max(known)
    if mx is None:
        mx = float(torch.linalg.vector_norm(w.detach().reshape(-1), ord=float("inf")))
    if not (mx > 0.0) or not math.isfinite(mx):
        return 1.0
    return 2.0 ** (10 - math.floor(math.log2(mx)))


def pack_linear(weight, bias=None, geglu=False, like=None):
    w = weight.detach().reshape(weight.shape[0], -1).contiguous().float()
    N, K = w.shape
    Np, Kp = (N + 15) // 16 * 16, (K + 31) // 32 * 32
    data = torch.empty(lib().mvd_packed_weight_bytes(N, K), dtype=torch.uint8, device=w.device)
    scale = _pack_scale(w, like if like is not None else weight)
    check(lib().mvd_pack_linear_weight(ptr(w), N, K, K, int(geglu), scale, ptr(data), stream()))
    b = None
    if bias is not None:
        b = torch.zeros(Np, dtype=torch.float32, device=w.device)
        b[:N] = bias.detach().float()
    return PackedWeight(data, Np, Kp, N, b, geglu, acc_scale=1.0 / scale)


def pack_linear_t(weight, like=None):
    w = weight.detach()
    assert w.dim() == 2 and w.dtype == torch.float32 and w.is_contiguous()
    K, N = w.shape
    Np, Kp = (N + 15) // 16 * 16, (K + 31) // 32 * 32
    data = torch.empty(lib().mvd_packed_weight_bytes(N, K), dtype=torch.uint8, device=w.device)
    scale = _pack_scale(w, like if like is not None else weight)
    check(lib().mvd_pack_linear_weight_t(ptr(w), N, K, N, scale, ptr(data), stream()))
    return PackedWeight(data, Np, Kp, N, None, False, acc_scale=1.0 / scale)


def pack_linear_cat(weights):
    return pack_linear(torch.cat([w.detach().float() for w in weights], dim=0), like=list(weights))


def pack_conv3x3(weight, bias=None, like=None):
    w = weight.detach().contiguous().float()
    Cout, Cin = w.shape[0], w.shape[1]
    cin_pad = (Cin + 31) // 32 * 32
    Np = (Cout + 15) // 16 * 16
    data = torch.empty(Np * 9 * cin_pad * 4, dtype=torch.uint8, device=w.device)
    scale = _pack_scale(w, like if like is not None else weight)
    check(lib().mvd_pack_conv3x3_weight(ptr(w), Cout, Cin, cin_pad, scale, ptr(data), stream()))
    b = None
    if bias is not None:
        b = torch.zeros(Np, dtype=torch.float32, device=w.device)
        b[:Cout] = bias.detach().float()
    return PackedWeight(data, Np, 9 * cin_pad, Cout, b, conv_cin=cin_pad, acc_scale=1.0 / scale)


def tap_schedule(cin, cin2=0):
    assert cin % 32 == 0 and cin2 % 32 == 0
    return [(0, cb, tap) for cb in range(cin // 32) for tap in range(9)] + [(1, cb, 4) for cb in range(cin2 // 32)]


def up4_schedule(weight):
    w = weight.detach()
    assert w.dim() == 4 and tuple(w.shape[2:]) == (3, 3)
    rows = torch.tensor([[[1, 0, 0], [0, 1, 1]], [[1, 1, 0], [0, 0, 1]]], dtype=torch.float64, device=w.device)
    wq = torch.einsum("ayk,cxl,oikl->acoiyx", rows, rows, w.double()).reshape(4, w.shape[0], w.shape[1], 2, 2).to(w.dtype)
    nb = (w.shape[1] + 31) // 32
    return wq, [(par, cb, tap) for par in range(4) for cb in range(nb) for tap in range(4)]


def pack_conv3x3_up4(weight, bias=None):
    wq, _ = up4_schedule(weight.detach().float())
    Cout, Cin = wq.shape[1], wq.shape[2]
    cin_pad, Np = (Cin + 31) // 32 * 32, (Cout + 15) // 16 * 16
    K = 4 * cin_pad
    m = torch.zeros(4, Cout, cin_pad, 4, dtype=torch.float32, device=wq.device)
    m[:, :, :Cin] = wq.reshape(4, Cout, Cin, 4)
    m = m.reshape(4, Cout, cin_pad // 32, 32, 4).permute(0, 1, 2, 4, 3).reshape(4, Cout, K).contiguous()
    img = Np * K * 4
    data = torch.empty(4 * img, dtype=torch.uint8, device=wq.device)
    scale = _pack_scale(m)
    for par in range(4):
        check(lib().mvd_pack_linear_weight(ptr(m[par]), Cout, K, K, 0, scale, ptr(data[par * img:]), stream()))
    b = None
    if bias is not None:
        b = torch.zeros(Np, dtype=torch.float32, device=wq.device)
        b[:Cout] = bias.detach().float()
    return PackedWeight(data, Np, K, Cout, b, conv_cin=cin_pad, acc_scale=1.0 / scale, up4=True)


UP4_MIN_ROWS = int(os.environ.get("MVD_UP4_MIN_ROWS", "128"))

# ... 204 lines not shown
    return out


GEMM_SEQUENCE = None
SELF_PREFETCH_MIN = int(os.environ.get("MVD_SELF_PREFETCH_MIN", "0"))


class WeightPrefetcher:

    def __init__(self, device, window=24 << 20, max_items=24, gn_hosts=0, self_min=None):
        self.device = device
        self.window, self.max_items = int(window), int(max_items)
        self.self_min = int(SELF_PREFETCH_MIN if self_min is None else self_min)
        self.gn_hosts = bool(gn_hosts)
        self.seq, self.recording, self.table, self.n, self.launch_idx, self.shares = [], False, None, 0, 0, {}

    class _Following:
        def __init__(self, pf, record):
            self.pf, self.record = pf, record

        def __enter__(self):
            global GEMM_SEQUENCE
            self.prev, GEMM_SEQUENCE = GEMM_SEQUENCE, self.pf
            self.pf.recording = self.record
            self.pf.launch_idx = 0
            if self.record:
                self.pf.seq = []
            return self.pf

        def __exit__(self, *exc):
            global GEMM_SEQUENCE
            GEMM_SEQUENCE = self.prev
            if self.record and exc[0] is None:
                self.pf._build()
            self.pf.recording = False
            return False

    def following(self, record=False):
        return WeightPrefetcher._Following(self, record)

    def note(self, d, W):
        j = self.launch_idx
        self.launch_idx += 1
        is_ws = bool(d.cfg) and _cfg_parts(d.cfg)[1] == WS_LOOP
        host = 1 if is_ws else (2 if (d.gna_out_sp and d.splitk != 1 and self.gn_hosts) else 0)
        if self.recording:
            packed = not isinstance(W, PlanesOperand)
            self.seq.append((W.data.data_ptr(), W.data.numel() * W.data.element_size(), host) if packed else (0, 0, host))
            return
        if host and j in self.shares:
            first, n = self.shares[j]
            d.pf_items, d.pf_n = self.table.data_ptr() + first * C.sizeof(PrefetchItem), n

    def _build(self):
        items = []
        self.shares = {}
        hosts = [j for j, e in enumerate(self.seq) if e[2]]
        sure = [j for j, e in enumerate(self.seq) if e[2] == 1]
        for j in hosts:
            nxt = [k for k in sure if k > j]
            end = nxt[0] if nxt else len(self.seq) - 1
            first, acc, seen = len(items), 0, set()
            if self.self_min > 0 and self.seq[j][2] == 1 and self.seq[j][1] >= self.self_min:
                items.append((self.seq[j][0], self.seq[j][1], j, j))
                seen.add(self.seq[j][0])
            for k in range(j + 1, end + 1):
                ptr_, nbytes, _ = self.seq[k]
                if not nbytes or ptr_ in seen or acc + nbytes > self.window or len(items) - first >= self.max_items:
                    continue
                seen.add(ptr_)
                acc += nbytes
                items.append((ptr_, nbytes, j, k))
            if len(items) > first:
                self.shares[j] = (first, len(items) - first)
        self.n = len(items)
        arr = (PrefetchItem * max(self.n, 1))()
        for i, (ptr_, nbytes, sa, cons) in enumerate(items):
            arr[i].ptr, arr[i].bytes, arr[i].start_after, arr[i].consumer = ptr_, nbytes, sa, cons
        self.table = torch.frombuffer(bytearray(bytes(arr)), dtype=torch.uint8).clone().to(self.device)
        self.items = items


CFG_STRIDE = 32
GNA_SILU, GNA_ROUND_F16, GNA_OUT_UNUSED = 1, 2, 4
TUNE_CACHE_VERSION = 12
GEMM_TILES = ((64, 64, 2, 2), (128, 128, 2, 4), (128, 80, 4, 1), (64, 80, 4, 1), (128, 160, 4, 2))
GEMM_LOOPS = (2, 3, 4, None, 6, 7, "patch", "ws")
REMOVED_LOOPS = tuple(i for i, l in enumerate(GEMM_LOOPS) if l is None)
PATCH_LOOP = 6
WS_LOOP = 7


def _cfg_parts(cfg):
    return (cfg - 1) // CFG_STRIDE, ((cfg - 1) % CFG_STRIDE) >> 1, (cfg - 1) & 1


def make_cfg(tile, loop, order=0):
    return 1 + CFG_STRIDE * tile + 2 * loop + order


def _cfg_valid(cfg, epi, b_mode=0):
    tile, loop, _ = _cfg_parts(cfg)
    if loop >= len(GEMM_LOOPS):
        return False
    bm, bn, wm, wn = GEMM_TILES[tile]
    waves = wm * wn
    return loop not in REMOVED_LOOPS and (loop != 2 or waves == 8) and (loop != 5 or waves == 4) and \
        (loop != PATCH_LOOP or tile in (1, 2, 4)) and (tile < 2 or epi == EPI_STORE) and \
        (loop != WS_LOOP or tile == 1 or (tile in (2, 4) and epi == EPI_STORE))


_ALL_CONFIGS = tuple(c for c in range(1, CFG_STRIDE * len(GEMM_TILES) + 1) if _cfg_valid(c, EPI_STORE))
GEMM_CONFIGS = tuple(c for c in _ALL_CONFIGS if _cfg_parts(c)[1] != PATCH_LOOP)
PATCH_CONFIGS = tuple(c for c in _ALL_CONFIGS if _cfg_parts(c)[1] == PATCH_LOOP)
GEMM_CONFIGS_CONV = GEMM_CONFIGS + PATCH_CONFIGS


def gemm_configs(epi=EPI_STORE, b_mode=0, conv=False):
    return tuple(c for c in (GEMM_CONFIGS_CONV if conv else GEMM_CONFIGS) if _cfg_valid(c, epi, b_mode))


def cfg_supported(d, cfg):
    return bool(lib().mvd_gemm_cfg_supported(C.byref(d), cfg))


def kernel_symbol(cfg, prec, conv):
    if not cfg:
        return f"gemm_kernel<auto, {prec}, {1 if conv else 0}>"
    tile, loop, _ = _cfg_parts(cfg)
    bm, bn, wm, wn = GEMM_TILES[tile]
    if loop == PATCH_LOOP:
        return f"conv_patch_kernel<{bm}, {bn}, {wm}, {wn}, {prec}>"
    if loop == WS_LOOP:
        cm, cn = {1: (2, 2), 2: (4, 1), 4: (2, 2)}[tile]
        return f"gemm_ws_kernel<{bm}, {bn}, {cm}, {cn}, {prec}, {1 if conv else 0}>"
    return f"gemm_kernel<{bm}, {bn}, {wm}, {wn}, {prec}, {1 if conv else 0}, {GEMM_LOOPS[loop]}>"


def gemm_fingerprint():
    import glob
    import hashlib
    h = hashlib.sha256()
    root = os.path.dirname(_HERE)
    pats = ("mvdfusion_amd/csrc/gemm*.hip", "mvdfusion_amd/csrc/gemm*.hpp", "mvdfusion_amd/csrc/common.hpp")
    for f in sorted(f for pat in pats for f in glob.glob(os.path.join(root, pat))):
        h.update(os.path.relpath(f, root).encode())
        h.update(open(f, "rb").read())
    return h.hexdigest()[:16]


def default_tuned_path(fmt=None):
    return os.path.join(_HERE, "tuned", f"gemm_{fmt or OPERAND_FORMAT}.json")


TUNED_IN_RUN = 0
TUNED_SOURCE = None


def load_default_tuned():
    global TUNED_SOURCE
    env = os.environ.get("MVD_TUNE_CACHE", "")
    if env == "0":
        TUNED_SOURCE = "none (MVD_TUNE_CACHE=0): tuned in this run"
        return 0
    path = env or default_tuned_path()
    if not os.path.exists(path):
        TUNED_SOURCE = f"none ({os.path.relpath(path, os.path.dirname(_HERE))} missing): tuned in this run"
        return 0
    n = load_tuned(path, require_fingerprint=os.environ.get("MVD_TUNE_CACHE_ANY") != "1")
    rel = os.path.relpath(path, os.path.dirname(_HERE))
    TUNED_SOURCE = f"{rel}: {n} problems" if n else f"none ({rel} was tuned on other GEMM sources or another cfg encoding): tuned in this run"
    return n


def save_tuned(path, merge=False):
    import json
    entries = {}
    if merge and os.path.exists(path):
        doc = json.load(open(path))
        if _tuned_doc_ok(doc) and doc.get("gemm_fingerprint") == gemm_fingerprint():
            entries = {tuple(k): tuple(v) for k, v in doc["entries"]}
    entries.update(_TUNED)
    os.makedirs(os.path.dirname(os.path.abspath(path)), exist_ok=True)
    with open(path, "w") as f:
        json.dump({"version": TUNE_CACHE_VERSION, "cfg_stride": CFG_STRIDE, "operand_format": OPERAND_FORMAT,
                   "gemm_fingerprint": gemm_fingerprint(),
                   "entries": sorted([list(k), list(v)] for k, v in entries.items())}, f, indent=0)


def _tuned_doc_ok(doc):
    return isinstance(doc, dict) and doc.get("version") == TUNE_CACHE_VERSION and doc.get("cfg_stride") == CFG_STRIDE and \
        doc.get("operand_format") == OPERAND_FORMAT


def load_tuned(path, require_fingerprint=False):
    import json
    doc = json.load(open(path))
    if not _tuned_doc_ok(doc) or (require_fingerprint and doc.get("gemm_fingerprint") != gemm_fingerprint()):
        return 0
    n = 0
    for k, v in doc["entries"]:
        cfg = int(v[0])
        if cfg != 0 and not (1 <= cfg <= CFG_STRIDE * len(GEMM_TILES) and _cfg_parts(cfg)[1] < len(GEMM_LOOPS) and
                             _cfg_parts(cfg)[1] not in REMOVED_LOOPS):
            continue
        _TUNED[tuple(k)] = tuple(v)
        n += 1
    return n


LAST_CFG = 0
AUTOTUNE = False
AUTOTUNE_MIN_FLOPS = 0.0
_TUNED = {}


_TRASH = None
TUNE_SPLITS = os.environ.get("MVD_TUNE_SPLITS") == "1"
TUNE_COLD = True


def _flush_caches():
    global _TRASH
    if _TRASH is None:
        _TRASH = torch.zeros(160 * 1024 * 1024, dtype=torch.float32, device="cuda")
    _TRASH.add_(1.0)


def release_tuning_buffers():
    global _TRASH
    _TRASH = None


_TUNE_STATS = {}


def _autotune(d, A=None, reps=4, trials=int(os.environ.get("MVD_TUNE_TRIALS", "3")), W_data=None):
    best, best_ms = (0, d.splitk), float("inf")
    e0, e1 = Event(), Event()
    stats_ptr, d.gn_stats = d.gn_stats, None
    if d.gna_out_sp:
        n = (d.M // d.gn_hw) * d.gn_groups * 2
        n = (n, str(A.device) if A is not None else "cuda")
        scratch = _TUNE_STATS.get(n)
        if scratch is None:
            scratch = _TUNE_STATS[n] = torch.zeros(n[0], dtype=torch.int64, device=A.device if A is not None else "cuda")
        d.gn_stats = scratch.data_ptr()
    skip = set()
    skip |= {int(t) for t in os.environ.get("MVD_TUNE_EXCLUDE_LOOPS", "").split(",") if t}
    fixed_split = d.splitk
    cands = [(c, sk) for c in gemm_configs(d.epi, d.b_mode, conv=d.a_mode == A_CONV3X3) if cfg_supported(d, c) and _cfg_parts(c)[1] not in skip
             for sk in ((0, 1) if d.splitk == 0 else (d.splitk,))]
    timed, second_pass = [], False
    wp0 = d.Wp
    rot = [wp0]
    if TUNE_COLD and A is not None and d.b_mode == 0:
        if W_data is not None and W_data.data_ptr() == wp0:
            rot += [W_data.clone(), W_data.clone()]
    ptrs = [wp0] + [t.data_ptr() for t in rot[1:]]
    for cfg, sk in cands:
        d.cfg, d.splitk = cfg, sk
        check(lib().mvd_gemm(C.byref(d), stream()))
        ms = float("inf")
        if TUNE_COLD and A is not None:
            for _ in range(trials + 1):
                _flush_caches()
                A.view(-1)[:A.numel() // 2 * 2].view(torch.int32).sum()
                e0.record()
                for wp in ptrs:
                    d.Wp = wp
                    check(lib().mvd_gemm(C.byref(d), stream()))
                e1.record()
                ms = min(ms, e0.elapsed_ms(e1) / len(ptrs))
            d.Wp = wp0
        else:
            for _ in range(trials):
                e0.record()
                for _ in range(reps):
                    check(lib().mvd_gemm(C.byref(d), stream()))
                e1.record()
                ms = min(ms, e0.elapsed_ms(e1))
        if sk != 1:
            ms += 0.0015
        timed.append((ms, cfg, sk))
        if ms < best_ms * 0.99:
            best, best_ms = (cfg, sk), ms
        if len(timed) == len(cands) and TUNE_SPLITS and fixed_split == 0 and not second_pass:
            second_pass = True
            nk = d.K // 32
            extra = [s_ for s_ in (2, 3, 4, 6, 8, 12, 16, 24, 32) if s_ <= max(1, nk // 2)]
            top = sorted(timed)[:3]
            cands.extend((c, s_) for _, c, _ in top for s_ in extra if (c, s_) not in cands)
    d.gn_stats = stats_ptr
    return best


def gemv(W, bias, x, y, act_in=ACT_NONE, act_out=ACT_NONE):
    M, K = x.shape
    N = W.shape[0]
    check(lib().mvd_gemv(ptr(W), ptr(bias), ptr(x), ptr(y), M, N, K, x.stride(0), y.stride(0), act_in, act_out, stream()))
    return y


def groupnorm(x, y, gamma, beta, B, HW, Cc, eps, silu, ws):
    check(lib().mvd_groupnorm_nhwc(ptr(x), ptr(y), ptr(gamma), ptr(beta), B, HW, Cc, 32, eps, int(silu), ptr(ws), ws.numel(),
                                   stream()))
    return y


def groupnorm_from_stats(x, y, gamma, beta, stats, B, HW, Cc, eps, silu, groups=32):
    check(lib().mvd_groupnorm_from_stats(ptr(x), ptr(y), ptr(gamma), ptr(beta), ptr(stats), B, HW, Cc, groups, eps, int(silu), stream()))
    return y


def layernorm(x, y, w, b, rows, Cc, eps=1e-5, w_plus_one=False, y_f32=None):
    check(lib().mvd_layernorm(ptr(x), ptr(y), ptr(y_f32), ptr(w), ptr(b), rows, Cc, eps, int(w_plus_one), stream()))
    return y


def layernorm_groups(x, y, w, b, rows, Cc, rows_per_group, eps=1e-5, w_plus_one=False, y_f32=None):
    assert w.stride(0) == b.stride(0) and w.stride(-1) == 1 and b.stride(-1) == 1, (w.stride(), b.stride())
    check(lib().mvd_layernorm_groups(ptr(x), ptr(y), ptr(y_f32), ptr(w), ptr(b), w.stride(0), rows, int(rows_per_group), Cc, eps,
                                     int(w_plus_one), stream()))
    return y


def softmax_rows(x, y, scale=1.0, out_scale=1.0):
    rows, cols = x.shape
    check(lib().mvd_softmax_rows(ptr(x), ptr(y), rows, cols, x.stride(0), float(scale), float(out_scale), stream()))
    return y


def attention(planes, out, B, heads, L, dhead, prec=PREC_X4, Lkeys=0):
    qh, ql, kh, kl, vh, vl = planes
    check(lib().mvd_attention(ptr(qh), ptr(ql), ptr(kh), ptr(kl), ptr(vh), ptr(vl), ptr(out), out.shape[-1] // 2, B, heads,
                              L, Lkeys, dhead, prec, stream()))
    return out


def alloc_attn_planes(B, heads, L, dhead, device):
    nqk = lib().mvd_attn_qk_plane_elems(B, heads, L, dhead)
    nvt = lib().mvd_attn_vt_plane_elems(B, heads, L, dhead)
    mk = lambda n: torch.zeros(n, dtype=torch.int16, device=device)
    return (mk(nqk), mk(nqk), mk(nqk), mk(nqk), mk(nvt), mk(nvt))


class Graph:

    def __init__(self):
        self.exec = C.c_void_p()

    def __enter__(self):
        self._side = torch.cuda.Stream()
        self._side.wait_stream(torch.cuda.current_stream())
        self._ctx = torch.cuda.stream(self._side)
        self._ctx.__enter__()
        check(lib().mvd_graph_begin(stream()))
        return self

    def __exit__(self, et, ev, tb):
        rc = lib().mvd_graph_end(stream(), C.byref(self.exec))
        self._ctx.__exit__(et, ev, tb)
        torch.cuda.current_stream().wait_stream(self._side)
        if et is None:
            check(rc)
        return False

    def launch(self):
        check(lib().mvd_graph_launch(self.exec, stream()))

    def __del__(self):
        try:
            if self.exec:
                lib().mvd_graph_destroy(self.exec)
        except Exception:
            pass


class Event:
    def __init__(self):
        self.h = C.c_void_p()
        check(lib().mvd_event_create(C.byref(self.h)))

    def record(self):
        check(lib().mvd_event_record(self.h, stream()))

    def elapsed_ms(self, stop):
        ms = C.c_float()
        check(lib().mvd_event_elapsed_ms(self.h, stop.h, C.byref(ms)))
        return ms.value
```

mvdfusion_amd/unet.py:

```python
import math

import torch
import torch.nn as nn

from . import hip
from .attention import SpatialTransformer, ViewAlignedFeatureTransformer
from .engine import Ctx


class GroupNorm32(nn.GroupNorm):
    pass


def normalization(channels):
    return GroupNorm32(32, channels)


class TimestepBlock(nn.Module):
    pass


class Upsample(nn.Module):
    def __init__(self, channels, use_conv, dims=2, out_channels=None, padding=1):
        super().__init__()
        self.channels, self.out_channels = channels, out_channels or channels
        self.conv = nn.Conv2d(self.channels, self.out_channels, 3, padding=padding)
        self._p = self._p4 = None

    def run(self, ctx, x, H, W, out=None):
        if hip.use_up4(ctx.B, H, W, training=ctx.keep_fp32):
            if self._p4 is None:
                self._p4 = hip.pack_conv3x3_up4(self.conv.weight, self.conv.bias)
            wp = self._p4
        else:
            if self._p is None:
                self._p = hip.pack_conv3x3(self.conv.weight, self.conv.bias)
            wp = self._p
        if out is None:
            out = ctx.act((ctx.B * 4 * H * W, self.out_channels))
        xp = hip.split_planes(x, ctx.ws.planes("updown.x", ctx.B * H * W, self.channels))
        ctx.gemm(xp, wp, out, conv=dict(B=ctx.B, Hin=H, Win=W, Cin=self.channels, Hout=2 * H, Wout=2 * W,
                                            stride=1, upsample=1), gn=(ctx.B, 4 * H * W), kind="conv")
        return out, 2 * H, 2 * W


class Downsample(nn.Module):
    def __init__(self, channels, use_conv, dims=2, out_channels=None, padding=1):
        super().__init__()
        self.channels, self.out_channels = channels, out_channels or channels
        self.op = nn.Conv2d(self.channels, self.out_channels, 3, stride=2, padding=padding)
        self._p = None

    def run(self, ctx, x, H, W, out=None):
        if self._p is None:
            self._p = hip.pack_conv3x3(self.op.weight, self.op.bias)
        Ho, Wo = H // 2, W // 2
        if out is None:
            out = ctx.act((ctx.B * Ho * Wo, self.out_channels))
        xp = hip.split_planes(x, ctx.ws.planes("updown.x", ctx.B * H * W, self.channels))
        ctx.gemm(xp, self._p, out, conv=dict(B=ctx.B, Hin=H, Win=W, Cin=self.channels, Hout=Ho, Wout=Wo, stride=2,
                                            upsample=0), gn=(ctx.B, Ho * Wo), kind="conv")
        return out, Ho, Wo


class ResBlock(TimestepBlock):

    def __init__(self, channels, emb_channels, dropout, out_channels=None, dims=2, use_checkpoint=False,
                 use_scale_shift_norm=False):
        super().__init__()
        assert not use_scale_shift_norm
        self.channels, self.out_channels = channels, out_channels or channels
        self.in_layers = nn.Sequential(normalization(channels), nn.SiLU(),
                                       nn.Conv2d(channels, self.out_channels, 3, padding=1))
        self.emb_layers = nn.Sequential(nn.SiLU(), nn.Linear(emb_channels, self.out_channels))
        self.out_layers = nn.Sequential(normalization(self.out_channels), nn.SiLU(), nn.Dropout(p=dropout),
                                        nn.Conv2d(self.out_channels, self.out_channels, 3, padding=1))
        self.skip_connection = nn.Identity() if self.out_channels == channels else \
            nn.Conv2d(channels, self.out_channels, 1)
        self._p = None

    def packed(self, fuse_skip=True):
        c1, c2, sk = self.in_layers[2], self.out_layers[3], self.skip_connection
        fuse = bool(fuse_skip) and not isinstance(sk, nn.Identity)
        if self._p is None:
            self._p = (hip.pack_conv3x3(c1.weight, None), None, None)
        if self._p[1] is None or bool(self._p[1].tail_cin) != fuse:
            w2 = hip.pack_conv3x3_tail(c2.weight, c2.bias, sk.weight, sk.bias) if fuse else hip.pack_conv3x3(c2.weight, c2.bias)
            wsk = None if fuse or isinstance(sk, nn.Identity) else hip.pack_linear(sk.weight, sk.bias)
            self._p = (self._p[0], w2, wsk)
        return self._p

    def run(self, ctx, x, H, W, out=None, x_planes=None):
        B, Ci, Co = ctx.B, self.channels, self.out_channels
        M = B * H * W
        w1, w2, wsk = self.packed(fuse_skip=ctx.prec_of("skip") == ctx.prec_of("conv"))
        geo = dict(B=B, Hin=H, Win=W, Hout=H, Wout=W, stride=1, upsample=0)
        a = ctx.ws.planes("res.a", M, Ci)
        ctx.groupnorm(x, a, self.in_layers[0], B, H * W, Ci, silu=True)
        h = ctx.ws.get("res.h", (M, Co))
        a2 = ctx.ws.planes("res.a2", M, Co)
        eb = ctx.emb_bias[self]
        ctx.gemm(a, w1, h, conv=dict(Cin=Ci, **geo), bias=False, bias_b=eb, rows_per_batch=M // eb.shape[0],
                 gn=(B, H * W), kind="conv",
                 gn_apply=(self.out_layers[0], a2, True, True))
        if (wsk is not None or w2.tail_cin) and x_planes is None:
            x_planes = hip.split_planes(x, ctx.ws.planes("res.xp", M, Ci))
        if out is None:
            out = ctx.act((M, Co))
        if w2.tail_cin:
            ctx.gemm(a2, w2, out, conv=dict(Cin=Co, **geo), a2=x_planes, gn=(B, H * W), kind="conv")
            return out
        skip = x
        if wsk is not None:
            skip = ctx.ws.get("res.skip", (M, Co))
            ctx.gemm(x_planes, wsk, skip, kind="skip")
        ctx.gemm(a2, w2, out, conv=dict(Cin=Co, **geo), res=skip, gn=(B, H * W), kind="conv")
        return out


def gn_hint(layer):
    from .attention import SpatialTransformer, ViewAlignedFeatureTransformer
    if isinstance(layer, tuple):
        return layer
    if isinstance(layer, ResBlock):
        return layer.in_layers[0], "res.a", True
    if isinstance(layer, SpatialTransformer):
        return layer.norm, "tf.n", False
    if isinstance(layer, ViewAlignedFeatureTransformer):
        return layer.aligned_attn_norm, "tf.n", False
    return None


class TimestepEmbedSequential(nn.Sequential, TimestepBlock):
    def run(self, ctx, x, H, W, out=None, x_planes=None, next_layer=None, next_cat=None):
        n = len(self)
        for i, layer in enumerate(self):
            dst = out if i == n - 1 else None
            ctx.next_gn = gn_hint(self[i + 1] if i + 1 < n else next_layer)
            ctx.next_cat = next_cat if i == n - 1 else None
            if isinstance(layer, (Upsample, Downsample)):
                x, H, W = layer.run(ctx, x, H, W, out=dst)
            elif isinstance(layer, ResBlock):
                x = layer.run(ctx, x, H, W, out=dst, x_planes=x_planes if i == 0 else None)
            else:
                x = layer.run(ctx, x, H, W, out=dst)
            ctx.next_gn = None
            ctx.next_cat = None
        return x, H, W


class _StemConv(nn.Conv2d):
    _p = None

    def run(self, ctx, x, H, W, out):
        if self._p is None:
            self._p = hip.pack_conv3x3(self.weight, self.bias)
        ctx.gemm(x, self._p, out, conv=dict(B=ctx.B, Hin=H, Win=W, Cin=self._p.conv_cin, Hout=H, Wout=W, stride=1,
                                            upsample=0), gn=(ctx.B, H * W), kind="conv")
        return out


class UNetModel(nn.Module):
    def __init__(self, image_size, in_channels, model_channels, out_channels, num_res_blocks, attention_resolutions,
                 dropout=0, channel_mult=(1, 2, 4, 8), conv_resample=True, dims=2, num_classes=None,
                 use_checkpoint=False, use_fp16=False, num_heads=-1, num_head_channels=-1, num_heads_upsample=-1,
                 use_scale_shift_norm=False, resblock_updown=False, use_new_attention_order=False,
                 use_spatial_transformer=True, use_view_aligned_transformer=True, transformer_depth=1,
                 context_dim=None, n_embed=None, legacy=True):
        super().__init__()
        assert use_view_aligned_transformer and use_spatial_transformer and context_dim is not None
        assert dims == 2 and num_classes is None and not resblock_updown and n_embed is None and conv_resample
        assert num_heads != -1 and num_head_channels == -1, "this build supports the num_heads form (configs/*.yaml)"
        if isinstance(context_dim, (list, tuple)) or type(context_dim).__name__ == "ListConfig":
            context_dim = list(context_dim)[0]
        channel_mult = tuple(channel_mult)
        attention_resolutions = tuple(attention_resolutions)
        self.image_size, self.in_channels, self.model_channels = image_size, in_channels, model_channels
        self.out_channels, self.num_res_blocks, self.channel_mult = out_channels, num_res_blocks, channel_mult
        self.attention_resolutions, self.num_heads, self.context_dim = attention_resolutions, num_heads, context_dim
        ted = model_channels * 4
        self.time_embed = nn.Sequential(nn.Linear(model_channels, ted), nn.SiLU(), nn.Linear(ted, ted))

        def res(cin, cout):
            return ResBlock(cin, ted, dropout, out_channels=cout, use_checkpoint=use_checkpoint)

        def st(c):
            return SpatialTransformer(c, num_heads, c // num_heads, depth=transformer_depth, context_dim=context_dim)

        def vaft(c):
            return ViewAlignedFeatureTransformer(c, num_heads, c // num_heads, depth=transformer_depth,
                                                 context_dim=context_dim, image_size=image_size)

        self.input_blocks = nn.ModuleList([TimestepEmbedSequential(_StemConv(in_channels, model_channels, 3, padding=1))])
        skip_chans = [model_channels]
        ch, ds = model_channels, 1
        for level, mult in enumerate(channel_mult):
            for _ in range(num_res_blocks):
                layers = [res(ch, mult * model_channels)]
                ch = mult * model_channels
                if ds in attention_resolutions:
                    layers.append(st(ch))
                self.input_blocks.append(TimestepEmbedSequential(*layers))
                skip_chans.append(ch)
            if level != len(channel_mult) - 1:
                self.input_blocks.append(TimestepEmbedSequential(Downsample(ch, True, out_channels=ch)))
                skip_chans.append(ch)
                ds *= 2
        self.middle_block = TimestepEmbedSequential(res(ch, ch), st(ch), vaft(ch), res(ch, ch))
        self.output_blocks = nn.ModuleList([])
        for level, mult in list(enumerate(channel_mult))[::-1]:
            for i in range(num_res_blocks + 1):
                layers = [res(ch + skip_chans.pop(), model_channels * mult)]
                ch = model_channels * mult
                if ds in attention_resolutions:
                    layers += [st(ch), vaft(ch)]
                if level and i == num_res_blocks:
                    layers.append(Upsample(ch, True, out_channels=ch))
                    ds //= 2
                self.output_blocks.append(TimestepEmbedSequential(*layers))
        self.out = nn.Sequential(normalization(ch), nn.SiLU(), nn.Conv2d(model_channels, out_channels, 3, padding=1))
        self._head = None
        self._temb = None
        self._xattn = None
        self._head_saved = None
        self._record = None

    def get_cross_attn_parameters(self, finetune_cross_attn, finetune_view_attn):
        out = []
        for name, p in self.named_parameters():
            if finetune_cross_attn and any(k in name for k in (".norm.", ".proj_in.", ".transformer_blocks.", ".proj_out.")):
                out.append(p)
            if finetune_view_attn and ".aligned_attn_" in name:
                out.append(p)
        return out

    def disable_unet_grad(self):
        for name, p in self.named_parameters():
            if ".aligned_attn_" not in name:
                p.requires_grad_(False)

    def _resblocks(self):
        return [m for m in self.modules() if isinstance(m, ResBlock)]

    def time_biases(self, ctx, t_sin):
        if self._temb is None:
            blocks = self._resblocks()
            w = torch.cat([b.emb_layers[1].weight.detach() for b in blocks], 0).contiguous()
            bias = torch.cat([b.emb_layers[1].bias.detach() + b.in_layers[2].bias.detach() for b in blocks], 0).contiguous()
            offs, o = {}, 0
            for b in blocks:
                offs[b] = (o, o + b.out_channels)
                o += b.out_channels
            self._temb = (w, bias, offs)
        w, bias, offs = self._temb
        ted = self.model_channels * 4
        R = t_sin.shape[0]
        e1, emb = ctx.ws.get("temb.e1", (R, ted)), ctx.ws.get("temb.emb", (R, ted))
        out = ctx.ws.get("temb.bias", (R, w.shape[0]))
        ctx.gemv_rows(self.time_embed[0].weight, self.time_embed[0].bias, t_sin, e1, act_out=hip.ACT_SILU)
        ctx.gemv_rows(self.time_embed[2].weight, self.time_embed[2].bias, e1, emb)
        ctx.gemv_rows(w, bias, emb, out, act_in=hip.ACT_SILU)
        ctx.emb_bias = {b: out[:, lo:hi] for b, (lo, hi) in offs.items()}

    def cross_attn_vectors(self, ctx):
        if self._xattn is None:
            sts = [m for m in self.modules() if isinstance(m, SpatialTransformer)]
            ws, bs, offs, o = [], [], {}, 0
            for st in sts:
                a2 = st.transformer_blocks[0].attn2
                wo, wv = a2.to_out[0].weight.detach().double(), a2.to_v.weight.detach().double()
                ws.append((wo @ wv).float())
                bs.append(a2.to_out[0].bias.detach().float())
                offs[st] = (o, o + st.in_channels)
                o += st.in_channels
            self._xattn = (torch.cat(ws, 0).contiguous(), torch.cat(bs, 0).contiguous(), offs, o)
        w, bias, offs, total = self._xattn
        out = ctx.ws.get("xattn.vec", (ctx.context.shape[0], total))
        ctx.gemv_rows(w, bias, ctx.context, out)
        ctx.xattn_vec = {st: out[:, lo:hi] for st, (lo, hi) in offs.items()}

    def run(self, ctx, x_in, t_sin, S):
        B = ctx.B
        self.time_biases(ctx, t_sin)
        self.cross_attn_vectors(ctx)
        hs = []
        H = W = S
        h = x_in
        rec = self._record
        for bi, blk in enumerate(self.input_blocks):
            if rec is not None:
                rec.append((blk, h.clone(), H, W, 0))
            if bi == 0:
                o = ctx.ws.get("hs0", (B * H * W, self.model_channels))
                ctx.next_gn = gn_hint(self.input_blocks[1][0])
                h = blk[0].run(ctx, h, H, W, o)
                ctx.next_gn = None
            else:
                last = blk[-1]
                Ho, Wo = (H // 2, W // 2) if isinstance(last, Downsample) else (H, W)
                co = last.out_channels if isinstance(last, (ResBlock, Downsample)) else last.in_channels
                o = ctx.ws.get(f"hs{bi}", (B * Ho * Wo, co))
                nxt = self.input_blocks[bi + 1][0] if bi + 1 < len(self.input_blocks) else self.middle_block[0]
                h, H, W = blk.run(ctx, h, H, W, out=o, next_layer=nxt)
            hs.append((h, H, W))
        if rec is not None:
            rec.append((self.middle_block, h.clone(), H, W, 0))
        keep = rec is not None or ctx.keep_fp32

        def cat_hint(nblk, co, Hn, Wn):
            first = nblk[0]
            if keep or not isinstance(first, ResBlock) or isinstance(first.skip_connection, nn.Identity):
                return None
            nsk = hs[-1][0]
            Mn = B * Hn * Wn
            return (nsk, ctx.ws.get("cat", (Mn, co + nsk.shape[-1])), ctx.ws.planes("catp", Mn, co + nsk.shape[-1])) + gn_hint(first)

        def out_geometry(blk, H, W):
            last = blk[-1]
            co = last.out_channels if isinstance(last, (ResBlock, Upsample)) else last.in_channels
            return (co, 2 * H, 2 * W) if isinstance(last, Upsample) else (co, H, W)

        h, H, W = self.middle_block.run(ctx, h, H, W, next_cat=cat_hint(self.output_blocks[0], *out_geometry(self.middle_block, H, W)))
        for bi, blk in enumerate(self.output_blocks):
            sk, _, _ = hs.pop()
            M = B * H * W
            ca, cb = h.shape[-1], sk.shape[-1]
            cat = ctx.ws.get("cat", (M, ca + cb))
            catp = ctx.ws.planes("catp", M, ca + cb)
            first = blk[0]
            if cat.data_ptr() in ctx._cat_done:
                ctx._cat_done.discard(cat.data_ptr())
            else:
                need_cat = keep or not isinstance(first, ResBlock) or isinstance(first.skip_connection, nn.Identity)
                ctx.concat(h, ca, sk, cb, cat, catp, B, H * W, gn_apply=gn_hint(first), need_out=need_cat)
            if rec is not None:
                rec.append((blk, cat.clone(), H, W, ca))
            last_blk = bi + 1 == len(self.output_blocks)
            h, H, W = blk.run(ctx, cat, H, W, x_planes=catp, next_layer=(self.out[0], "res.a", True) if last_blk else None,
                              next_cat=None if last_blk else cat_hint(self.output_blocks[bi + 1], *out_geometry(blk, H, W)))
        if self._head is None:
            self._head = hip.pack_conv3x3(self.out[2].weight, self.out[2].bias)
        M = B * H * W
        a = ctx.ws.planes("res.a", M, self.model_channels)
        ctx.groupnorm(h, a, self.out[0], B, H * W, self.model_channels, silu=True)
        y = ctx.ws.get("head", (M, 8))
        ctx.gemm(a, self._head, y, conv=dict(B=B, Hin=H, Win=W, Cin=self.model_channels, Hout=H, Wout=W, stride=1,
                                             upsample=0), ldo=8, kind="conv")
        self._head_saved = (h, a)
        return y


class UNetWrapper(nn.Module):

    def __init__(self, unet_config, unet_path=None, drop_conditions=False, drop_scheme="default", use_zero_123=False,
                 finetune_unet=False, finetune_cross_attn=False, finetune_view_attn=True, remove_keys=()):
        super().__init__()
        params = unet_config.get("params", unet_config) if hasattr(unet_config, "get") else unet_config
        self.unet_model = UNetModel(**dict(params))
        if unet_path:
            from .load_model import load_unet_checkpoint
            load_unet_checkpoint(self.unet_model, unet_path, remove_keys=remove_keys)
        if not finetune_unet:
            self.unet_model.disable_unet_grad()
        self.drop_conditions, self.drop_scheme, self.use_zero_123 = drop_conditions, drop_scheme, use_zero_123
        self.finetune_unet, self.finetune_cross_attn, self.finetune_view_attn = \
            finetune_unet, finetune_cross_attn, finetune_view_attn

    def get_trainable_parameters(self):
        if self.finetune_unet:
            return self.unet_model.parameters()
        return self.unet_model.get_cross_attn_parameters(finetune_cross_attn=self.finetune_cross_attn,
                                                         finetune_view_attn=self.finetune_view_attn)

    def level_channels(self):
        u = self.unet_model
        return [u.model_channels * m for m in u.channel_mult]

    def level0_operand(self, ctx, B, S, D):
        rows = B * S * S * D
        if D == 1:
            c0 = self.level_channels()[0]
            return ctx.ws.get("ovol0", (rows, 2 * (c0 + 768)), torch.int16, zero=True), c0
        return ctx.ws.get("vol0", (rows, 2 * 768), torch.int16, zero=True), 0

    def volume_pyramid(self, ctx, vol, B, S, D):
        levels = [self.level0_operand(ctx, B, S, D)]
        Cc = vol.shape[-1]
        chans = self.level_channels()
        for i in range(1, len(self.unet_model.channel_mult)):
            f = 2 ** i
            rows = B * (S // f) * (S // f) * D
            if D == 1:
                ld, col = chans[i] + Cc, chans[i]
                o = ctx.ws.get(f"ovol{i}", (rows, 2 * ld), torch.int16, zero=True)
            else:
                ld, col = Cc, 0
                o = ctx.ws.planes(f"vol{i}", rows, Cc)
            hip.check(hip.lib().mvd_area_pool(hip.ptr(vol), hip.c_void_p(o.data_ptr() + 4 * col), B, S, D, Cc, f, ld, hip.stream()))
            levels.append((o, col))
        return levels
```

mvdfusion_amd/view_attn_efficient2.py:

```python
import torch
import torch.nn as nn

from . import hip
from .cameras import pack_cameras


_G4_VEC_BLOCK, _G4_VEC_MISC = 3328, 3 * 3328


def window_size(keep_top_k_views, top_k):
    return 2 * (int(top_k) // 2) + 1 if keep_top_k_views else 0


def window_view_table(V, top_k):
    half = int(top_k) // 2
    return (torch.arange(-half, half + 1)[:, None] + torch.arange(int(V))[None, :]) % int(V)


_MT_INDEX = {}


def _microtile_index(dev):
    t = _MT_INDEX.get(str(dev))
    if t is None:
        perm = torch.tensor([(4 * c + j) if j < 4 else (16 + 4 * c + j - 4) for c in range(4) for j in range(8)], device=dev)
        R, c8 = torch.arange(16, device=dev), torch.arange(8, device=dev)
        gran = (R >> 3)[:, None].expand(16, 8)
        pos = ((R & 7) * 8)[:, None] + (c8[None, :] ^ ((R >> 1) & 7)[:, None])
        t = _MT_INDEX[str(dev)] = (perm, gran, pos)
    return t


def _microtiles(W, scale, bf16):
    N, K = W.shape
    assert N % 16 == 0 and K % 32 == 0, (N, K)
    w = (W.detach().double() * scale).float()
    dt = torch.bfloat16 if bf16 else torch.float16
    hi = w.to(dt)
    lo = (w - hi.float()).to(dt)
    perm, gran, pos = _microtile_index(W.device)

    def chunks(t):
        return t.contiguous().view(torch.int16).view(N // 16, 16, K // 32, 32)[..., perm].reshape(N // 16, 16, K // 32, 4, 8)

    data = torch.cat([chunks(hi), chunks(lo)], dim=3).permute(0, 2, 1, 3, 4)
    img = torch.empty(N // 16, K // 32, 2, 64, 8, dtype=torch.int16, device=W.device)
    img[:, :, gran, pos, :] = data
    return img.reshape(N // 16, K // 32, 1024)


def pack_fused_stream(ga, bf16=False):
    C = ga.hidden_size
    blocks = list(ga.aggregation_transformer.layer_list)
    assert C == 256 and len(blocks) == 3 and all(b.num_heads == 8 and b.mlp.fc1.out_features == 512 for b in blocks)
    dev = ga.pre_layer_b[0].weight.device
    vecs = torch.zeros(hip.lib().mvd_gridattn_fused_vec_floats(), dtype=torch.float32, device=dev)
    tiles = []

    def scaled(Wt, like):
        sc = hip._pack_scale(Wt.detach(), like=like)
        return _microtiles(Wt, sc, bf16), 1.0 / sc

    def put(o, t):
        t = t.detach().float().reshape(-1)
        vecs[o:o + t.numel()] = t

    wpre = torch.zeros(C, 736, device=dev)
    wpre[:, :723] = ga.pre_layer_b[0].weight.detach().float()
    pre, s_pre = scaled(wpre, ga.pre_layer_b[0].weight)
    tiles.append(pre.permute(1, 0, 2).reshape(-1, 1024))
    put(_G4_VEC_MISC, ga.pre_layer_b[0].bias)
    wl = ga.aggregation_transformer.weight_layer
    put(_G4_VEC_MISC + 256, wl.weight)
    put(_G4_VEC_MISC + 512, wl.bias)
    host = {_G4_VEC_MISC + 520: s_pre}
    for bi, blk in enumerate(blocks):
        q, s_q = scaled(blk.attn.qkv.weight.detach().float(), blk.attn.qkv.weight)
        pj, s_p = scaled(blk.attn.proj.weight.detach().float(), blk.attn.proj.weight)
        f1, s_1 = scaled(blk.mlp.fc1.weight.detach().float(), blk.mlp.fc1.weight)
        f2, s_2 = scaled(blk.mlp.fc2.weight.detach().float(), blk.mlp.fc2.weight)
        for hd in range(8):
            rows = [2 * hd, 2 * hd + 1, 16 + 2 * hd, 16 + 2 * hd + 1, 32 + 2 * hd, 32 + 2 * hd + 1]
            tiles.append(q[rows].permute(1, 0, 2).reshape(-1, 1024))
            tiles.append(pj[:, hd])
        for ch in range(8):
            tiles.append(f1[4 * ch:4 * ch + 4].permute(1, 0, 2).reshape(-1, 1024))
            tiles.append(f2[:, 2 * ch:2 * ch + 2].permute(1, 0, 2).reshape(-1, 1024))
        o = bi * _G4_VEC_BLOCK
        put(o + 1536, blk.attn.qkv.bias)
        put(o + 2304, blk.attn.proj.bias)
        put(o + 2560, blk.mlp.fc1.bias)
        put(o + 3072, blk.mlp.fc2.bias)
        for k, v in enumerate((s_q, s_p, s_1, s_2)):
            host[_G4_VEC_MISC + 521 + 4 * bi + k] = v
    idx = sorted(host)
    vecs[torch.tensor(idx, device=dev)] = torch.tensor([host[k] for k in idx], dtype=torch.float32).to(dev)
    stream = torch.cat(tiles, 0).contiguous()
    assert stream.shape[0] == 16 * hip.lib().mvd_gridattn_fused_slots(), stream.shape
    return stream, vecs


class _TimmAttention(nn.Module):
    def __init__(self, dim, num_heads):
        super().__init__()
        self.num_heads = num_heads
        self.qkv = nn.Linear(dim, dim * 3, bias=True)
        self.proj = nn.Linear(dim, dim)


class _TimmMlp(nn.Module):
    def __init__(self, dim, hidden):
        super().__init__()
        self.fc1 = nn.Linear(dim, hidden)
        self.fc2 = nn.Linear(hidden, dim)


class DiTBlock(nn.Module):

    def __init__(self, hidden_size, num_heads, cond_dim=None, mlp_ratio=4.0):
        super().__init__()
        cond_dim = hidden_size if cond_dim is None else cond_dim
        self.attn = _TimmAttention(hidden_size, num_heads)
        self.mlp = _TimmMlp(hidden_size, int(hidden_size * mlp_ratio))
        self.adaLN_modulation = nn.Sequential(nn.SiLU(), nn.Linear(cond_dim, 6 * hidden_size, bias=True))
        self.hidden_size, self.num_heads = hidden_size, num_heads
        self._p = None

    def packed(self):
        if self._p is None:
            self._p = (hip.pack_linear(self.attn.qkv.weight, self.attn.qkv.bias),
                       hip.pack_linear(self.attn.proj.weight, self.attn.proj.bias),
                       hip.pack_linear(self.mlp.fc1.weight, self.mlp.fc1.bias),
                       hip.pack_linear(self.mlp.fc2.weight, self.mlp.fc2.bias))
        return self._p

    def run(self, ctx, h, h_alt, c, T, V):
        C = self.hidden_size
        wqkv, wproj, wfc1, wfc2 = self.packed()
        lin = self.adaLN_modulation[1]
        mod = ctx.ws.get("ga.mod", (1, 6 * C))
        hip.gemv(lin.weight, lin.bias, c, mod, act_in=hip.ACT_SILU)
        sh1, sc1, g1, sh2, sc2, g2 = (mod[0, i * C:(i + 1) * C] for i in range(6))
        ln = ctx.ws.planes("ga.ln", T, C)
        hip.layernorm(h, ln, sc1, sh1, T, C, eps=1e-6, w_plus_one=True)
        qkv = ctx.ws.get("ga.qkv", (T, 3 * C))
        ctx.gemm(ln, wqkv, qkv, kind="ga")
        att = ctx.ws.planes("ga.att", T, C)
        hip.check(hip.lib().mvd_view_mha(hip.ptr(qkv), hip.ptr(att), T // V, V, self.num_heads, C // self.num_heads,
                                         hip.stream()))
        ctx.gemm(att, wproj, h_alt, res=h, colscale=g1, kind="ga")
        hip.layernorm(h_alt, ln, sc2, sh2, T, C, eps=1e-6, w_plus_one=True)
        f1 = ctx.ws.planes("ga.f1", T, wfc1.N)
        ctx.gemm(ln, wfc1, None, act=hip.ACT_GELU, out_planes=f1, kind="ga")
        ctx.gemm(f1, wfc2, h, res=h_alt, colscale=g2, kind="ga")
        return h


class AggregationTransformer(nn.Module):
    def __init__(self, hidden_size, num_layers=3, num_heads=8, mlp_ratio=2.0, use_t=False):
        super().__init__()
        if not use_t:
            raise NotImplementedError
        self.use_t = use_t
        self.layer_list = nn.ModuleList([DiTBlock(hidden_size, num_heads=num_heads, mlp_ratio=mlp_ratio)
                                         for _ in range(num_layers)])
        self.weight_layer = nn.Linear(hidden_size, 1)


class _TimestepEmbedder(nn.Module):
    def __init__(self, hidden_size, frequency_embedding_size=256):
        super().__init__()
        self.mlp = nn.Sequential(nn.Linear(frequency_embedding_size, hidden_size, bias=True), nn.SiLU(),
                                 nn.Linear(hidden_size, hidden_size, bias=True))


class GridAttn(nn.Module):
    def __init__(self, input_size=32, in_channels=4, hidden_size=256, output_dim=768, num_heads=8, mlp_ratio=2.0,
                 num_layers=3, side_length=32, world_scale=0.6, z_near_far_scale=0.8, depth_scale=2.0,
                 depth_shift=0.5, n_pts_per_ray=3, use_t=True, keep_top_k_views=False, top_k=4, device="cpu"):
        super().__init__()
        self.keep_top_k_views, self.top_k = bool(keep_top_k_views), int(top_k)
        assert not self.keep_top_k_views or 1 <= self.window <= 16, f"top_k={top_k}: the window {self.window} exceeds 16 rows per 3-D point"
        assert hidden_size == 256, "the token kernel is specialised for 256-channel feature maps"
        assert in_channels == 5, "mvd_zembed reads 4 VAE + 1 depth latent channels (configs/*.yaml: in_channels: 5)"
        self.input_size, self.hidden_size, self.output_dim = input_size, hidden_size, output_dim
        self.depth_scale, self.depth_shift, self.n_pts_per_ray = depth_scale, depth_shift, n_pts_per_ray
        self.z_near_far_scale = z_near_far_scale
        self.z_embedder = nn.Sequential(nn.Linear(in_channels, 256), nn.GELU())
        self.t_embedder = _TimestepEmbedder(hidden_size)
        self.use_t = use_t
        self.pre_layer_b = nn.Sequential(nn.Linear(256 * 2 + 90 * 2 + 15 * 2 + 1, hidden_size), nn.GELU())
        self.aggregation_transformer = AggregationTransformer(hidden_size, num_layers, num_heads, mlp_ratio, use_t)
        self.final_layer_b = nn.Linear(hidden_size, output_dim)
        for blk in self.aggregation_transformer.layer_list:
            nn.init.constant_(blk.adaLN_modulation[-1].weight, 0)
            nn.init.constant_(blk.adaLN_modulation[-1].bias, 0)
        self._p = None
        self._fused = None

    def packed(self):
        if self._p is None:
            self._p = (hip.pack_linear(self.pre_layer_b[0].weight, self.pre_layer_b[0].bias),
                       hip.pack_linear(self.final_layer_b.weight, self.final_layer_b.bias))
        return self._p

    def packed_fused(self, device):
        if self._fused is None:
            stream, vecs = pack_fused_stream(self, bf16=hip.OPERAND_FORMAT == "bf16")
            self._fused = (stream.to(device), vecs.to(device))
        return self._fused

    @property
    def window(self):
        return window_size(self.keep_top_k_views, self.top_k)

    def rows_per_point(self, V):
        return self.window or int(V)

    def fused_supported(self, V, T):
        blocks = self.aggregation_transformer.layer_list
        R = self.rows_per_point(V)
        Vp = 1 << max(R - 1, 0).bit_length()
        return (V >= 1 and 1 <= R <= 16 and (T // R * Vp) % 64 == 0 and T % R == 0 and self.hidden_size == 256 and len(blocks) == 3 and
                all(b.num_heads == 8 and b.mlp.fc1.out_features == 512 for b in blocks))

    def run(self, ctx, x, depth_noise, steps, it, cams_rec, in_cam_rec, input_latents, c, vol_out, V, S, D, q0=0, Vq=None,
            vol_planes=None, vol_planes_col=0, fused=None, depth_src=None, depth_steps=None, scenes=1, steps_scene_stride=0):
        Vq = V if Vq is None else Vq
        N = int(scenes)
        L = hip.lib()
        assert x.shape[1] == 5, "depth wise efficient attention requires 4+1 channels"
        assert N == 1 or (N > 1 and x.shape[0] == N * V and input_latents.shape[0] == N and q0 == 0 and Vq == V), \
            (N, V, q0, Vq, tuple(x.shape), tuple(input_latents.shape))
        w_pre, w_fin = self.packed()
        z = self.z_embedder[0]
        feat = ctx.ws.get("ga.feat", (N * V, S, S, 256))
        in_feat = ctx.ws.get("ga.infeat", (N, S, S, 256))
        hip.check(L.mvd_zembed(hip.ptr(x), hip.ptr(z.weight), hip.ptr(z.bias), hip.ptr(feat), N * V, S, hip.stream()))
        hip.check(L.mvd_zembed(hip.ptr(input_latents), hip.ptr(z.weight), hip.ptr(z.bias), hip.ptr(in_feat), N, S,
                               hip.stream()))
        nseq = N * Vq * S * S * D
        W = self.window
        R = self.rows_per_point(V)
        T = nseq * R
        dsrc = x if depth_src is None else depth_src
        dsteps = steps if depth_steps is None else depth_steps
        assert (depth_src is None) == (depth_steps is None) and dsrc.shape == x.shape
        grid_lin = ctx.ws.bufs.get(("ga.lin", S))
        if grid_lin is None:
            half = 1.0 / float(S)
            grid_lin = torch.linspace(1.0 - half, -1.0 + half, S, dtype=torch.float32).to(ctx.device)
            ctx.ws.bufs[("ga.lin", S)] = grid_lin
        if fused is None:
            fused = self.fused_supported(V, T // N)
        sst = int(steps_scene_stride)
        if sst:
            assert N > 1 and c.shape[0] == N, (N, tuple(c.shape))
            if fused is False or not self.fused_supported(V, T // N):
                raise NotImplementedError(f"GridAttn.run: per-scene timesteps need the fused aggregation kernel (V={V}, T={T // N} per scene); "
                                          "the unfused chain shares one adaLN modulation")
            fused = True
        if fused:
            assert self.fused_supported(V, T // N), (V, T // N)
            stream, vecs = self.packed_fused(ctx.device)
            nv = vecs.numel()
            vecs = vecs.view(1, nv)
            if sst:
                vecs = ctx.ws.get("ga.vecs_scenes", (N, nv)).copy_(vecs.expand(N, nv))
            for bi, blk in enumerate(self.aggregation_transformer.layer_list):
                lin = blk.adaLN_modulation[1]
                ctx.gemv_rows(lin.weight, lin.bias, c, vecs[:, bi * _G4_VEC_BLOCK:bi * _G4_VEC_BLOCK + 1536], act_in=hip.ACT_SILU)
            pool = ctx.ws.planes("ga.pool", nseq, self.hidden_size)
            hip.check(L.mvd_gridattn_fused_window(hip.ptr(dsrc), hip.ptr(depth_noise), hip.ptr(dsteps), hip.ptr(it), hip.ptr(grid_lin),
                                                  hip.ptr(feat), hip.ptr(in_feat), hip.ptr(cams_rec), hip.ptr(in_cam_rec), hip.ptr(stream),
                                                  hip.ptr(vecs), hip.ptr(pool), N, V, q0, Vq, S, D, float(self.depth_scale),
                                                  float(self.depth_shift), 3 if ctx.prec_of("ga") == 3 else 4, sst, sst * nv, W, hip.stream()))
            ctx.gemm(pool, w_fin, vol_out, M=nseq, out_planes=vol_planes, out_planes_col=vol_planes_col, kind="ga")
            return vol_out
        tokens = ctx.ws.planes("ga.tokens", T, hip.TOKEN_LD)
        hip.check(L.mvd_gridattn_tokens_window(hip.ptr(dsrc), hip.ptr(depth_noise), hip.ptr(dsteps), hip.ptr(it), hip.ptr(grid_lin),
                                               hip.ptr(feat), hip.ptr(in_feat), hip.ptr(cams_rec), hip.ptr(in_cam_rec),
                                               hip.ptr(tokens), N, V, q0, Vq, S, D, float(self.depth_scale), float(self.depth_shift),
                                               0, W, hip.stream()))
        h = ctx.ws.get("ga.h", (T, self.hidden_size))
        h_alt = ctx.ws.get("ga.h_alt", (T, self.hidden_size))
        ctx.gemm(tokens, w_pre, h, act=hip.ACT_GELU, kind="ga")
        for blk in self.aggregation_transformer.layer_list:
            h = blk.run(ctx, h, h_alt, c, T, R)
        wl = self.aggregation_transformer.weight_layer
        pool = ctx.ws.planes("ga.pool", nseq, self.hidden_size)
        hip.check(L.mvd_view_pool(hip.ptr(h), hip.ptr(wl.weight), hip.ptr(wl.bias), hip.ptr(pool), nseq, R, self.hidden_size,
                                  hip.stream()))
        ctx.gemm(pool, w_fin, vol_out, M=nseq, out_planes=vol_planes, out_planes_col=vol_planes_col, kind="ga")
        return vol_out
```

mvdfusion_amd/viewfusion_zero_depth_rgb.py:

```python
import math

import torch
import torch.nn as nn

from . import hip
from .cameras import Cameras, get_camera_slice, get_relative_camera, pack_cameras
from .engine import Ctx, ddim_step_table
from .sampler import DDIMSampler
from .scheduler import DDPMScheduler
from .unet import UNetWrapper
from .view_attn_efficient2 import GridAttn

import os

PREFETCH_WEIGHTS = os.environ.get("MVD_PREFETCH", "ws")
PREFETCH_OPTIONS = {k: int(v) for k, v in (kv.split("=") for kv in os.environ.get("MVD_PREFETCH_OPTS", "").split(",") if kv)}


def _sinusoid_freqs(dim, max_period=10000):
    half = dim // 2
    return torch.exp(-math.log(max_period) * torch.arange(start=0, end=half, dtype=torch.float32) / half)


class StepEngine:

    def __init__(self, model, V, S, D, cfg, device, prec, q0=0, Vq=None, policy=None, scenes=1):
        self.m, self.V, self.S, self.D, self.cfg = model, V, S, D, bool(cfg)
        self.q0, self.Vq = q0, (V if Vq is None else Vq)
        self.N = N = int(scenes)
        if N < 1 or (N > 1 and (self.q0 != 0 or self.Vq != V)):
            raise ValueError(f"StepEngine(scenes={scenes}, q0={q0}, Vq={Vq}, V={V}): view-parallel sharding is single-scene only")
        NV = N * V
        self.ctx = Ctx(device, prec, policy)
        dev = self.ctx.device
        B = 2 * N * self.Vq if cfg else N * self.Vq
        self.B = B
        z = lambda *s: torch.zeros(*s, dtype=torch.float32, device=dev)
        self.x = z(NV, 5, S, S)
        self.x0 = z(NV, 5, S, S)
        self.eps = z(NV, 5, S, S)
        self.input_latents = z(N, 5, S, S)
        self.clip_v_embed = z(NV, 796)
        self.cams = z(NV, hip.CAM_RECORD)
        self.in_cam = z(N, hip.CAM_RECORD)
        self.context = z(B, 768)
        self.vol = z(B * S * S * D, 768)
        self.vol_planes, self.vol_col = model.unet_model.level0_operand(self.ctx, B, S, D)
        self.x_in = torch.zeros(B * S * S, 2 * 32, dtype=torch.int16, device=dev)
        self.iter = torch.zeros(1, dtype=torch.int32, device=dev)
        self.steps = z(1, hip.STEP_STRIDE)
        self.steps_nodiv = z(1, hip.STEP_STRIDE)
        self.prev = z(NV, 5, S, S)
        self.depth_mode = 0
        self.pin = None
        self.known = z(1, 5, S, S)
        self.pin_noise = None
        self.depth_noise = z(1, NV, D, S, S)
        self.ddim_noise = z(1, NV, 5, S, S)
        self.f256 = _sinusoid_freqs(256).to(dev)
        self.funet = _sinusoid_freqs(model.unet_model.unet_model.model_channels).to(dev)
        self.graphs = {}
        self.prefetchers = {}
        self.drop_masks = None
        self.n_rows = 1
        self.steps_scene_stride = 0
        self.done = 0

    def set_conditioning(self, batch_cameras, input_latents, input_cameras, clip_v_embed):
        self.set_conditioning_scenes([(batch_cameras, input_latents, input_cameras, clip_v_embed)])

    def set_conditioning_scenes(self, conds):
        if len(conds) != self.N:
            raise ValueError(f"set_conditioning_scenes: {len(conds)} scenes for a {self.N}-scene engine")
        V, S = self.V, self.S
        for n, (bc, il, ic, ce) in enumerate(conds):
            self.cams[n * V:(n + 1) * V].copy_(pack_cameras(bc).to(self.cams.device))
            self.in_cam[n:n + 1].copy_(pack_cameras(ic).to(self.cams.device))
            self.input_latents[n:n + 1].copy_(il.reshape(1, 5, S, S))
            self.clip_v_embed[n * V:(n + 1) * V].copy_(ce.reshape(V, 796))

    def set_schedule(self, steps_table, depth_noise, ddim_noise):
        self._set_tables(steps_table, depth_noise, ddim_noise, scene_stride=0)

    def set_schedule_scenes(self, steps_table, depth_noise, ddim_noise=None):
        if self.cfg:
            raise ValueError("StepEngine.set_schedule_scenes: per-scene timesteps need a cfg=False engine (the training step); "
                             "guided sampling steps share one timestep")
        if tuple(steps_table.shape) != (self.N, hip.STEP_STRIDE):
            raise ValueError(f"StepEngine.set_schedule_scenes: step table {tuple(steps_table.shape)} for {self.N} scenes "
                             f"(expected ({self.N}, {hip.STEP_STRIDE}))")
        if ddim_noise is None:
            ddim_noise = torch.zeros(1, self.N * self.V, 5, self.S, self.S)
        self._set_tables(steps_table, depth_noise, ddim_noise, scene_stride=1 if self.N > 1 else 0)

    def _set_tables(self, steps_table, depth_noise, ddim_noise, scene_stride):
        dev = self.ctx.device
        if self.steps.shape != steps_table.shape:
            self.graphs.clear()
            self.prefetchers.clear()
            self.steps = steps_table.to(dev).contiguous()
            self.steps_nodiv = self.steps.clone()
            self.depth_noise = depth_noise.to(dev).contiguous()
            self.ddim_noise = ddim_noise.to(dev).contiguous()
        else:
            self.steps.copy_(steps_table)
            self.depth_noise.copy_(depth_noise)
            self.ddim_noise.copy_(ddim_noise)
        self.steps_nodiv.copy_(self.steps)
        self.steps_nodiv[:, 1] = 1.0
        self.steps_scene_stride = scene_stride
        self.n_rows = int(steps_table.shape[0]) - (self.N - 1) * scene_stride
        self.rewind()

    def set_pin(self, mode, known, noise=None):
        dev = self.ctx.device
        nk = int(known.shape[0])
        K = nk // self.N
        if mode not in (0, 1) or K < 1 or K * self.N != nk or K > self.V or tuple(known.shape[1:]) != (5, self.S, self.S):
            raise ValueError(f"StepEngine.set_pin: mode {mode}, known {tuple(known.shape)} for {self.N} scene(s) of {self.V} views at "
                             f"S = {self.S} (expected (N*K, 5, S, S), 1 <= K <= V)")
        if mode == 1 and (noise is None or tuple(noise.shape) != (int(self.steps.shape[0]), nk, 5, self.S, self.S)):
            raise ValueError(f"StepEngine.set_pin: mode 1 needs noise ({int(self.steps.shape[0])}, {nk}, 5, {self.S}, {self.S}), got "
                             f"{None if noise is None else tuple(noise.shape)}")
        if self.known.shape != known.shape:
            self.graphs.clear()
            self.prefetchers.clear()
            self.known = known.to(dev, torch.float32).contiguous().clone()
        else:
            self.known.copy_(known)
        if mode == 1:
            if self.pin_noise is None or self.pin_noise.shape != noise.shape:
                self.graphs.clear()
                self.prefetchers.clear()
                self.pin_noise = noise.to(dev, torch.float32).contiguous().clone()
            else:
                self.pin_noise.copy_(noise)
        self.pin = (int(mode), K)

    def clear_pin(self):
        self.pin = None

    def rewind(self, it=0):
        assert 0 <= it < self.n_rows
        self.iter.fill_(it)
        self.done = it

    def depth_geo(self):
        if self.depth_mode == 0:
            return self.x, self.steps
        return (self.x0 if self.depth_mode == 1 else self.prev), self.steps_nodiv

    def enqueue(self, cfg_scale, do_update, prefetcher=None):
        m, ctx, L = self.m, self.ctx, hip.lib()
        V, S, D, B, q0, Vq, N = self.V, self.S, self.D, self.B, self.q0, self.Vq, self.N
        NVq = N * Vq
        ctx.B, ctx.D = B, D
        ctx.begin_step()
        st = hip.stream
        sst, R = self.steps_scene_stride, self.t_rows
        if sst and do_update:
            raise ValueError("StepEngine: per-scene timesteps (set_schedule_scenes) are a training step: no DDIM update")
        if self.pin is not None:
            mode, K = self.pin
            pn = self.pin_noise if mode == 1 else None
            hip.check(L.mvd_pin_views(hip.ptr(self.x), hip.ptr(self.x0), hip.ptr(self.known), hip.ptr(pn), N * K * 5 * S * S,
                                      hip.ptr(self.steps), hip.ptr(self.iter), N, V, K, S, mode, st()))
        ts = ctx.ws.get("vf.tsin", (R, 256))
        te1 = ctx.ws.get("vf.te1", (R, 256))
        c = ctx.ws.get("vf.c", (R, 256))
        hip.check(L.mvd_timestep_embedding_scenes(hip.ptr(self.steps), hip.ptr(self.iter), hip.ptr(self.f256), hip.ptr(ts), 256, R, sst,
                                                  st()))
        ctx.gemv_rows(m.time_embed[0].weight, m.time_embed[0].bias, ts, te1, act_out=hip.ACT_SILU)
        ctx.gemv_rows(m.time_embed[2].weight, m.time_embed[2].bias, te1, c)
        dsrc, dsteps = self.depth_geo()
        m.view_attn.run(ctx, self.x, self.depth_noise, self.steps, self.iter, self.cams, self.in_cam,
                        self.input_latents, c, self.vol, V, S, D, q0=q0, Vq=Vq, vol_planes=self.vol_planes,
                        vol_planes_col=self.vol_col, depth_src=None if self.depth_mode == 0 else dsrc,
                        depth_steps=None if self.depth_mode == 0 else dsteps, scenes=N, steps_scene_stride=sst)
        p = m.cc_projection
        c1 = ctx.ws.get("vf.cc1", (NVq, 768))
        c2 = ctx.ws.get("vf.cc2", (NVq, 768))
        ctx.gemv_rows(p[0].weight, p[0].bias, self.clip_v_embed[q0:q0 + NVq], c1, act_out=hip.ACT_SILU)
        ctx.gemv_rows(p[2].weight, p[2].bias, c1, c2, act_out=hip.ACT_SILU)
        ctx.gemv_rows(p[4].weight, p[4].bias, c2, self.context[:NVq])
        if self.drop_masks is not None:
            clip_m, vol_m, cat_m = self.drop_masks
            self.context[:NVq] *= clip_m[:, None]
            self.vol.view(B, -1)[:NVq] *= vol_m[:, None]
            vp = self.vol_planes.view(B, S * S * D, -1)
            vp[:NVq, :, 2 * self.vol_col:] *= vol_m.to(torch.int16)[:, None, None]
        ctx.context = self.context
        xq, x0q, epsq = self.x[q0:q0 + NVq], self.x0[q0:q0 + NVq], self.eps[q0:q0 + NVq]
        hip.check(L.mvd_unet_input_scenes(hip.ptr(xq), hip.ptr(self.input_latents), hip.ptr(self.x_in), N, Vq, S, 32,
                                          int(self.cfg), st()))
        if self.drop_masks is not None:
            xin = self.x_in.view(B, S * S, 64)
            cm = self.drop_masks[2].to(torch.int16)[:, None, None]
            xin[:NVq, :, 5:10] *= cm
            xin[:NVq, :, 37:42] *= cm
        unet = m.unet_model.unet_model
        ctx.vol_levels = m.unet_model.volume_pyramid(ctx, self.vol.view(B, S, S, D, 768), B, S, D)
        tsu = ctx.ws.get("vf.tsin_unet", (R, unet.model_channels))
        hip.check(L.mvd_timestep_embedding_scenes(hip.ptr(self.steps), hip.ptr(self.iter), hip.ptr(self.funet), hip.ptr(tsu),
                                                  unet.model_channels, R, sst, st()))
        y = unet.run(ctx, self.x_in, tsu, S)
        hip.check(L.mvd_cfg_ddim_update(hip.ptr(y), 8, hip.ptr(xq), hip.ptr(x0q), hip.ptr(epsq),
                                        hip.ptr(self.ddim_noise[:, q0:q0 + NVq]), N * V * 5 * S * S, hip.ptr(self.steps),
                                        hip.ptr(self.iter), NVq, S, int(self.cfg), float(cfg_scale), int(do_update), st()))
        if do_update:
            hip.check(L.mvd_advance_iter(hip.ptr(self.iter), st()))

    @property
    def t_rows(self):
        return self.N if self.steps_scene_stride else 1

    def step(self, cfg_scale, do_update, use_graph=True):
        key = (float(cfg_scale), bool(do_update), int(self.depth_mode), self.steps_scene_stride, self.pin)
        if self.done >= self.n_rows:
            raise IndexError(f"StepEngine.step: iteration {self.done} is past the {self.n_rows}-row step table "
                             "(set_schedule() / rewind() before stepping again)")
        if do_update:
            self.done += 1
        if not use_graph:
            return self.enqueue(cfg_scale, do_update)
        g = self.graphs.get(key)
        if g is None:
            it0 = self.iter.clone()
            x_keep, x0_keep = self.x.clone(), self.x0.clone()
            hip.AUTOTUNE = True
            try:
                self.enqueue(cfg_scale, do_update)
            finally:
                hip.AUTOTUNE = False
                hip.release_tuning_buffers()
            torch.cuda.synchronize()
            pf = None
            if PREFETCH_WEIGHTS == "ws":
                pf = hip.WeightPrefetcher(self.x.device, **PREFETCH_OPTIONS)
                self.iter.copy_(it0)
                self.x.copy_(x_keep)
                self.x0.copy_(x0_keep)
                with pf.following(record=True):
                    self.enqueue(cfg_scale, do_update)
                torch.cuda.synchronize()
            self.iter.copy_(it0)
            self.x.copy_(x_keep)
            self.x0.copy_(x0_keep)
            g = hip.Graph()
            self.ctx.ws.frozen = True
            try:
                with g:
                    if pf is None:
                        self.enqueue(cfg_scale, do_update)
                    else:
                        with pf.following():
                            self.enqueue(cfg_scale, do_update, prefetcher=pf)
            finally:
                self.ctx.ws.frozen = False
            self.graphs[key] = g
            self.prefetchers[key] = pf
        g.launch()


class _HipTrainingLoss(torch.autograd.Function):

    @staticmethod
    def forward(ctx, model, batch, trainer_config, names, *params):
        loss, grads = model.gradients(batch, trainer_config, noise_source=getattr(model, "_noise_source", None), only_trainable=True)
        ctx.grads = [grads.get(n) for n in names]
        ctx.shapes = [p.shape for p in params]
        return loss.clone()

    @staticmethod
    def backward(ctx, grad_out):
        if getattr(ctx, "_scaled", False):
            raise RuntimeError("_HipTrainingLoss.backward ran twice on one node: the step's gradient buffers were already scaled in place "
                               "(call model(batch, cfg) again instead of retain_graph=True)")
        ctx._scaled = True
        live, seen, spans = [], set(), []
        for g in ctx.grads:
            if g is None:
                continue
            key = (g.untyped_storage().data_ptr(), g.storage_offset(), tuple(g.shape), tuple(g.stride()))
            if key in seen:
                continue
            seen.add(key)
            live.append(g)
            spans.append((g.data_ptr(), g.data_ptr() + g.numel() * g.element_size()) if g.is_contiguous() else None)
        disjoint = all(sp is not None for sp in spans)
        if disjoint:
            srt = sorted(spans)
            disjoint = all(srt[i][1] <= srt[i + 1][0] for i in range(len(srt) - 1))
        if live and disjoint:
            torch._foreach_mul_(live, grad_out.to(live[0].dtype))
            pick = lambda g: g
        else:
            pick = lambda g: g * grad_out.to(g.dtype)
        outs = [torch.zeros(s, dtype=grad_out.dtype, device=grad_out.device) if g is None else pick(g).reshape(s)
                for g, s in zip(ctx.grads, ctx.shapes)]
        return (None, None, None, None, *outs)


class ViewFusion(nn.Module):
    def __init__(self, view_attn_config, unet_config, ddpm_config, vae_config=None, unet_path="", vae_path="",
                 clip_path="", unet_cc_path="", z_scale_factor=0.18215, vae_max_batch=8, objective="noise",
                 loss_type="l2", embed_camera_pose=True, finetune_projection=False, finetune_unet=False,
                 finetune_cross_attn=True, finetune_view_attn=True, feed_prev_depth=False, drop_conditions=False,
                 vae=None, clip_image_encoder=None, precision=None, reference_eval_dropout=False, overwrite_x_noisy=False, **kwargs):
        super().__init__()
        assert embed_camera_pose, "this build implements the embed_camera_pose=True configuration of configs/*.yaml"
        self.finetune_projection, self.finetune_unet, self.z_scale_factor = finetune_projection, finetune_unet, z_scale_factor
        self.vae_max_batch, self.objective, self.loss_type = vae_max_batch, objective, loss_type
        self.embed_camera_pose, self.finetune_cross_attn, self.finetune_view_attn = \
            embed_camera_pose, finetune_cross_attn, finetune_view_attn
        self.feed_prev_depth, self.drop_conditions = feed_prev_depth, drop_conditions
        self.reference_eval_dropout = bool(reference_eval_dropout)
        from .configs import DEFAULT_PRECISION
        precision = precision or DEFAULT_PRECISION
        fmt, self.precision, self.precision_policy = hip.parse_precision(precision)
        hip.set_operand_format(fmt)
        self.precision_name = precision

        def params(cfg):
            return dict(cfg.get("params", cfg)) if hasattr(cfg, "get") else dict(cfg)

        self.view_attn = GridAttn(**params(view_attn_config))
        self.unet_model = UNetWrapper(unet_config, unet_path=unet_path or None, drop_conditions=drop_conditions,
                                      drop_scheme="default", finetune_unet=finetune_unet,
                                      finetune_cross_attn=finetune_cross_attn, finetune_view_attn=finetune_view_attn,
                                      use_zero_123=True,
                                      remove_keys=["input_blocks.0.0.weight", "out.2.weight", "out.2.bias"])
        self.scheduler = DDPMScheduler(**params(ddpm_config))
        if vae is not None:
            self.vae = vae
        elif vae_config is not None:
            from .load_model import instantiate_from_config
            self.vae = instantiate_from_config(vae_config)
            if vae_path:
                sd = torch.load(vae_path, map_location="cpu")
                sd = sd.get("state_dict", sd)
                self.vae.load_state_dict({k.replace("first_stage_model.", ""): v for k, v in sd.items()}, strict=False)
        if clip_image_encoder is not None:
            self.clip_image_encoder = clip_image_encoder
        elif clip_path:
            from .encoders import FrozenCLIPImageEmbedder
            self.clip_image_encoder = FrozenCLIPImageEmbedder(model=clip_path, precision=precision)
            for prm in self.clip_image_encoder.parameters():
                prm.requires_grad_(False)
        self.cc_projection = nn.Sequential(nn.Linear(768 + 14 * 2, 768), nn.SiLU(True), nn.Linear(768, 768),
                                           nn.SiLU(True), nn.Linear(768, 768))
        nn.init.eye_(list(self.cc_projection.parameters())[0][:768, :768])
        nn.init.zeros_(list(self.cc_projection.parameters())[1])
        self.time_embed_dim = 256
        self.time_embed = nn.Sequential(nn.Linear(256, 256), nn.SiLU(True), nn.Linear(256, 256))
        self.register_buffer("_device", torch.tensor([0.0]), persistent=False)
        self.latent_size = int(self.view_attn.input_size)
        self.ddim = DDIMSampler(self, ddim_num_steps=50, ddim_discretize="uniform", ddim_eta=1.0,
                                latent_size=self.latent_size, z_dim=4, feed_prev_depth=feed_prev_depth,
                                overwrite_x_noisy=overwrite_x_noisy)
        self._engines = {}
        self._packed_sig = None
        assert self.finetune_view_attn is True, "must finetune new view attention layers"

    train_autotune_min_flops = 2.0e9

    def invalidate_packed(self, keep_engines=False):
        hip.drop_packed_caches(self)
        hip.forget_param_maxima()
        if keep_engines:
            for e in self._engines.values():
                e.graphs.clear()
                e.prefetchers.clear()
        else:
            self._engines.clear()

    def load_state_dict(self, state_dict, strict=True, **kw):
        r = super().load_state_dict(state_dict, strict=strict, **kw)
        self.invalidate_packed()
        self._packed_sig = None
        return r

    def _apply(self, fn, *a, **kw):
        r = super()._apply(fn, *a, **kw)
        if "_engines" in self.__dict__:
            self.invalidate_packed()
            self._packed_sig = None
        return r

    def engine(self, V, S, D, cfg, q0=0, Vq=None, scenes=1):
        if int(scenes) < 1:
            raise ValueError(f"engine(scenes={scenes}): at least one scene")
        if int(scenes) > 1 and (q0 != 0 or (Vq is not None and Vq != V)):
            raise ValueError(f"engine(V={V}, q0={q0}, Vq={Vq}, scenes={scenes}): view-parallel sharding is single-scene only")
        sig = hip.params_signature(self)
        if sig != self._packed_sig:
            if self._packed_sig is not None:
                dev_now = self._device.device
                same_dev = all(e.ctx.device == dev_now for e in self._engines.values())
                self.invalidate_packed(keep_engines=same_dev)
            self._packed_sig = sig
            hip.register_param_maxima(self.parameters())
        if Vq is not None and Vq <= 0:
            raise ValueError(f"engine(V={V}, q0={q0}, Vq={Vq}): a rank must own at least one query view")
        key = (V, S, D, bool(cfg), q0, Vq) if int(scenes) == 1 else (V, S, D, bool(cfg), q0, Vq, int(scenes))
        e = self._engines.get(key)
        if e is None:
            dev = self._device.device
            if dev.type != "cuda":
                raise RuntimeError("mvdfusion_amd.ViewFusion runs on the GPU only (model.cuda() first); "
                                   "there is no CPU path in the product")
            e = StepEngine(self, V, S, D, cfg, dev, self.precision, q0=q0, Vq=Vq, policy=self.precision_policy, scenes=int(scenes))
            self._engines[key] = e
        return e

    def _print_parameter_count(self):
        va = sum(p.numel() for p in self.view_attn.parameters())
        un = sum(p.numel() for p in self.unet_model.get_trainable_parameters())
        uf = sum(p.numel() for p in self.unet_model.parameters())
        tp = sum(p.numel() for p in self.time_embed.parameters())
        pp = sum(p.numel() for p in self.cc_projection.parameters()) if self.finetune_projection else 0
        print(f"view_attn {va * 1e-6:.2f}M | unet trainable {un * 1e-6:.2f}M / full {uf * 1e-6:.2f}M | "
              f"total trainable {(va + un + tp + pp) * 1e-6:.2f}M / full {(va + uf + tp + pp) * 1e-6:.2f}M")

    @torch.no_grad()
    def encode_clip(self, x):
        return self.clip_image_encoder.encode(x)

    @torch.no_grad()
    def encode(self, x):
        return self.vae.encode(torch.clip(x * 2 - 1.0, -1.0, 1.0)).mode() * self.z_scale_factor

    @torch.no_grad()
    def decode(self, z):
        return torch.clip((self.vae.decode(z * 1 / self.z_scale_factor) + 1.0) / 2.0, 0.0, 1.0).clip(0.0, 1.0)

    def prepare_batch(self, batch, trainer_config, generator=None):
        images = batch["images"]
        dev = images.device
        Bn, _, H, W = images.shape
        n_in, n_tr = trainer_config["input_batch_size"], trainer_config["train_batch_size"]
        if trainer_config["random_views"]:
            rand = torch.randperm(Bn, generator=generator) if generator is not None else torch.randperm(Bn)
        else:
            rand = torch.linspace(0, Bn - 1, n_in + n_tr).long()
        in_idx, b_idx = rand[:n_in], rand[n_in:n_in + n_tr]
        input_latents = self.encode(images[in_idx])
        batch_latents = self.encode(images[b_idx])
        area = lambda d: torch.nn.functional.interpolate(d, scale_factor=0.125, mode="area")
        in_depth = torch.zeros_like(area(torch.zeros((n_in, 1, H, W), device=dev)))
        input_latents = torch.cat((input_latents, in_depth), dim=1)
        if "depths" in batch:
            b_depth = torch.clip(batch["depths"][b_idx].to(dev) * 2 - 1.0, -1.0, 1.0)
        else:
            b_depth = torch.zeros((n_tr, 1, H, W), device=dev)
        batch_latents = torch.cat((batch_latents, area(b_depth)), dim=1)
        cams = get_relative_camera(Cameras(batch["R"].float().cpu(), batch["T"].float().cpu(),
                                           batch["f"].float().cpu(), batch["c"].float().cpu()), in_idx)
        input_cameras, batch_cameras = get_camera_slice(cams, in_idx), get_camera_slice(cams, b_idx)
        clip_embed = self.encode_clip(images[in_idx]).expand(n_tr, -1, -1)
        from .synthetic import cam_embed
        clip_v_embed = torch.cat((clip_embed, cam_embed(input_cameras, batch_cameras).to(dev)), dim=-1)
        return batch_latents, batch_cameras, input_latents, input_cameras, clip_v_embed

    def embed_time(self, t):
        dev = self._device.device
        e = torch.cat([torch.cos(t[:, None].float() * self._f256(dev)), torch.sin(t[:, None].float() * self._f256(dev))], -1)
        h = torch.empty(t.shape[0], 256, device=dev)
        out = torch.empty(t.shape[0], 256, device=dev)
        for r in range(0, t.shape[0], 16):
            hip.gemv(self.time_embed[0].weight, self.time_embed[0].bias, e[r:r + 16].contiguous(), h[r:r + 16], act_out=hip.ACT_SILU)
            hip.gemv(self.time_embed[2].weight, self.time_embed[2].bias, h[r:r + 16], out[r:r + 16])
        return out

    def _f256(self, dev):
        if not hasattr(self, "_f256_cache") or self._f256_cache.device != dev:
            self._f256_cache = _sinusoid_freqs(256).to(dev)
        return self._f256_cache[None]

    @torch.no_grad()
    def apply_model(self, noisy_latents, batch_cameras, input_latents, input_cameras, clip_v_embed, t, prev_depth=None,
                    cfg_scale=1.0, depth_noise=None, drop_rand=None):
        V, _, S, _ = noisy_latents.shape
        if depth_noise is None:
            depth_noise = torch.randn(V, self.view_attn.n_pts_per_ray, S, S, device=noisy_latents.device)
        return self._step_scenes(noisy_latents, [(batch_cameras, input_latents, input_cameras, clip_v_embed)], [int(t[0])],
                                 None if prev_depth is None else [prev_depth], depth_noise, drop_rand, cfg_scale)

    def _step_scenes(self, noisy, conds, ts, prev_depth, depth_noise, drop_rand, cfg_scale=1.0):
        N = len(conds)
        NV, _, S, _ = noisy.shape
        V = NV // N
        D = self.view_attn.n_pts_per_ray
        cfg = cfg_scale != 1.0
        eng = self.engine(V, S, D, cfg, scenes=N)
        eng.set_conditioning_scenes(conds)
        rows = []
        for tv in ts:
            sac = self.scheduler.sqrt_alphas_cumprod[tv]
            dstd = self.scheduler.sqrt_one_minus_alphas_cumprod[tv] / sac / 10.0
            rows.append([float(tv), float(sac), float(dstd), 1.0, 1.0, 0.0, 0.0, 0.0])
        table = torch.tensor(rows, dtype=torch.float32)
        if cfg:
            eng.set_schedule(table, depth_noise.reshape(1, NV, D, S, S), torch.zeros(1, NV, 5, S, S))
        else:
            eng.set_schedule_scenes(table, depth_noise.reshape(1, NV, D, S, S))
        eng.x.copy_(noisy)
        eng.depth_mode = 0
        if prev_depth is not None:
            for n, pd in enumerate(prev_depth):
                eng.prev[n * V:(n + 1) * V, 4:5].copy_(pd.to(eng.prev.device).expand(V, 1, S, S))
            eng.depth_mode = 2
        eng.drop_masks = None
        if not cfg and self.drop_conditions and (self.training or self.reference_eval_dropout):
            r = torch.rand(NV, device=noisy.device) if drop_rand is None else drop_rand.to(noisy.device).float()
            drop_clip, drop_vol = (r > 0.15) & (r <= 0.2), (r > 0.1) & (r <= 0.15)
            drop_cat, drop_all = (r > 0.05) & (r <= 0.1), r <= 0.05
            eng.drop_masks = tuple(1.0 - (dm | drop_all).float() for dm in (drop_clip, drop_vol, drop_cat))
        self._last_drop_masks = eng.drop_masks
        self._train_engine = eng
        keep = eng.ctx.keep_fp32
        eng.ctx.keep_fp32 = keep or bool(getattr(self, "_train_keep_fp32", False))
        try:
            eng.step(cfg_scale, do_update=False, use_graph=eng.drop_masks is None and not getattr(self, "_force_eager", False))
        finally:
            eng.ctx.keep_fp32 = keep
            eng.drop_masks = None
        return hip.check_finite(eng.eps.clone(), "ViewFusion.apply_model")

    def sample(self, batch, trainer_config, cfg_scale, return_input=False, depth=False, verbose=True):
        batch_latents, batch_cameras, input_latents, input_cameras, clip_v_embed = self.prepare_batch(batch, trainer_config)
        res = self.ddim.sample(batch_cameras, input_latents, input_cameras, clip_v_embed, unconditional_scale=cfg_scale, depth=depth,
                               return_intermediates=return_input, verbose=verbose)
        return (res[0], batch_latents, input_latents, batch_cameras, res[1]) if return_input else res

    def sample_scenes(self, batches, trainer_config, cfg_scale, return_input=False, depth=False, verbose=True):
        prepared = [self.prepare_batch(b, trainer_config) for b in batches]
        conds = [(bc, il, ic, ce) for _, bc, il, ic, ce in prepared]
        res = self.ddim.sample_scenes(conds, unconditional_scale=cfg_scale, depth=depth, return_intermediates=return_input,
                                      verbose=verbose)
        if not return_input:
            return [res[n] for n in range(len(batches))]
        x, inter = res
        out = []
        for n, (batch_latents, batch_cameras, input_latents, _, _) in enumerate(prepared):
            its = [{"t": it["t"], "xt": it["xt"][n], "x0": it["x0"][n]} for it in inter]
            out.append((x[n], batch_latents, input_latents, batch_cameras, its))
        return out

    def sample_rig(self, batch, trainer_config, cfg_scale, chunk_views, anchors_per_chunk=1, anchors=None, return_input=False, depth=False,
                   verbose=True):
        batch_latents, batch_cameras, input_latents, input_cameras, clip_v_embed = self.prepare_batch(batch, trainer_config)
        x = self.ddim.sample_rig(batch_cameras, input_latents, input_cameras, clip_v_embed, unconditional_scale=cfg_scale,
                                 chunk_views=chunk_views, anchors_per_chunk=anchors_per_chunk, anchors=anchors, depth=depth, verbose=verbose)
        return (x, batch_latents, input_latents, batch_cameras, []) if return_input else x

    @torch.no_grad()
    def fuse(self, latents, batch_cameras, up=8, decode=True, **kw):
        from .fusion import fuse_views
        if decode:
            kw["rgb"] = self._decoded(latents)
        return fuse_views(latents, batch_cameras, up=up, depth_scale=self.view_attn.depth_scale, depth_shift=self.view_attn.depth_shift,
                          **kw)

    def _decoded(self, latents):
        S = latents.shape[-1]
        flat = latents.reshape(-1, 5, S, S)[:, :4]
        img = torch.cat([self.decode(c) for c in flat.split(self.vae_max_batch)]).float()
        return img.reshape(*latents.shape[:-3], 3, img.shape[-2], img.shape[-1])

    @torch.no_grad()
    def mesh(self, latents, batch_cameras, grid=128, up=8, decode=True, **kw):
        from .fusion import extract_mesh, integrate_tsdf
        if decode:
            kw["rgb"] = self._decoded(latents)
        fill = {"fill": kw.pop("fill")} if "fill" in kw else {}
        vol = integrate_tsdf(latents, batch_cameras, grid=grid, up=up, depth_scale=self.view_attn.depth_scale,
                             depth_shift=self.view_attn.depth_shift, **kw)
        return extract_mesh(vol, **fill)

    @torch.no_grad()
    def render(self, cloud, cameras, size=256, radius=1, **kw):
        from .fusion import render_points
        out = render_points(cloud, cameras, size=size, radius=radius, **kw)
        out._depth_map = (float(self.view_attn.depth_scale), float(self.view_attn.depth_shift))
        return out

    @torch.no_grad()
    def render_mesh(self, mesh, cameras, size=256, **kw):
        from .fusion import render_mesh
        out = render_mesh(mesh, cameras, size=size, **kw)
        out._depth_map = (float(self.view_attn.depth_scale), float(self.view_attn.depth_shift))
        return out

    @torch.no_grad()
    def p_losses(self, batch, trainer_config, noise_source=None, _aux=None):
        return self.p_losses_scenes([batch], trainer_config, noise_source=noise_source, _aux=_aux)

    def _draw(self, batch_latents, D, noise_source):
        V, _, S, _ = batch_latents.shape
        dev = batch_latents.device
        if noise_source is not None:
            ns = noise_source(V, D, S)
            return ns["t"].to(dev), ns["noise"].to(dev), ns["depth_noise"].to(dev), ns["drop_rand"].to(dev)
        t = self.scheduler.sample_random_times(V, share_t=True, device=dev)
        noise = torch.randn_like(batch_latents)
        return t, noise, torch.randn(V, D, S, S, device=dev), torch.rand(V, device=dev)

    def scene_draws(self, latents, noise_source=None):
        D = self.view_attn.n_pts_per_ray
        return [self._draw(bl, D, noise_source) for bl in latents]

    def _prepare_scenes(self, batches, trainer_config):
        if isinstance(batches, dict) or not isinstance(batches, (list, tuple)):
            raise TypeError("a multi-scene training step takes a list of batch dicts")
        if len(batches) == 0:
            raise ValueError("a multi-scene training step needs at least one scene")
        prepared = [b["_prepared"] if isinstance(b, dict) and "_prepared" in b else self.prepare_batch(b, trainer_config) for b in batches]
        V, _, S, _ = prepared[0][0].shape
        for n, pr in enumerate(prepared):
            Vn, _, Sn, _ = pr[0].shape
            if Vn != V:
                raise ValueError(f"scene {n} has {Vn} views, scene 0 has {V}: the scenes of a training step share V")
            if Sn != S:
                raise ValueError(f"scene {n} has {Sn}x{Sn} latents, scene 0 has {S}x{S}: the scenes of a training step share S")
        return prepared

    @torch.no_grad()
    def p_losses_scenes(self, batches, trainer_config, noise_source=None, _aux=None):
        prepared = self._prepare_scenes(batches, trainer_config)
        V = prepared[0][0].shape[0]
        draws = self.scene_draws([pr[0] for pr in prepared], noise_source)
        dev = prepared[0][0].device
        sa, s1 = self.scheduler.sqrt_alphas_cumprod.to(dev), self.scheduler.sqrt_one_minus_alphas_cumprod.to(dev)
        noisy = torch.cat([sa[t].view(V, 1, 1, 1) * pr[0] + s1[t].view(V, 1, 1, 1) * nz
                           for pr, (t, nz, _, _) in zip(prepared, draws)])
        ts = [int(t[0]) for t, _, _, _ in draws]
        conds = [(bc, il, ic, ce) for _, bc, il, ic, ce in prepared]
        prev = [pr[2][:, 4:].clone() for pr in prepared] if self.feed_prev_depth else None
        force = getattr(self, "_force_eager", False)
        self._train_keep_fp32, self._force_eager = True, True
        try:
            if len(prepared) == 1:
                (t, _, dn, dr), = draws
                pred = self.apply_model(noisy, *conds[0], t, prev_depth=None if prev is None else prev[0], depth_noise=dn, drop_rand=dr)
            else:
                pred = self._step_scenes(noisy, conds, ts, prev, torch.cat([d[2] for d in draws]), torch.cat([d[3] for d in draws]))
        finally:
            self._train_keep_fp32, self._force_eager = False, force
        if self.objective == "noise":
            target = torch.cat([d[1] for d in draws])
        elif self.objective == "x_start":
            target = torch.cat([pr[0] for pr in prepared])
        else:
            raise AssertionError(f"objective {self.objective} not implemented")
        assert self.loss_type == "l2", "loss_type 'l2' is the only one the reference implements (:86-87)"
        loss = torch.nn.functional.mse_loss(target, pred).mean()
        if _aux is not None:
            _aux.update(pred=pred, target=target)
        return loss

    def _loss(self, batch, trainer_config, noise_source=None, _aux=None):
        return self.p_losses_scenes(batch if isinstance(batch, (list, tuple)) else [batch], trainer_config, noise_source=noise_source,
                                    _aux=_aux)

    @torch.no_grad()
    def gradients_scenes(self, batches, trainer_config, noise_source=None, only_trainable=False):
        if not isinstance(batches, (list, tuple)):
            raise TypeError("gradients_scenes takes a list of batch dicts (gradients takes one)")
        return self.gradients(list(batches), trainer_config, noise_source=noise_source, only_trainable=only_trainable)

    @torch.no_grad()
    def unet_gradients(self, batch, trainer_config, noise_source=None, only_trainable=False):
        from . import backward_blocks as bb
        from . import backward_unet as bu
        unet = self.unet_model.unet_model
# ... 110 lines not shown
```

Baseline: 124.3 steps/s.

## Precompute per-schedule conditioning tables and fuse volume pyramid pooling

Per-step work that depends only on the timestep schedule or on fixed conditioning (timestep embeddings, time MLP, adaLN modulation gemvs, UNet time biases, CLIP projection, cross-attention vectors, input-latent z-embedding) is computed once into tables outside the graph. Each step then runs a single prologue kernel that zeros the GroupNorm arena and copies the current iteration's rows into place. The three separate area-pool launches for the volume pyramid are replaced by one kernel that reads each 8x8 window once and writes all three levels. This cuts many small launches and redundant reads per step, in exchange for extra cache-invalidation state that must be reset correctly when weights or conditioning change.

After: 126.2 steps/s, median of 6. +1.5%, better.

```diff
diff --git a/include/mvd_hip.h b/include/mvd_hip.h
--- a/include/mvd_hip.h
+++ b/include/mvd_hip.h
@@ -157,6 +157,10 @@
                          const float* beta, long long* gn_stats, int B, int hw, int groups, float eps, int silu, mvd_stream_t stream);
 int mvd_area_pool(const float* vol, void* out_sp, int B, int S, int D, int C, int factor, int ldp, mvd_stream_t stream);
 int mvd_fill_zero(float* p, size_t n, mvd_stream_t stream);
+int mvd_area_pool_pyramid(const float* vol, void* const* out_sp, const int* ldp, int B, int S, int D, int C, mvd_stream_t stream);
+#define MVD_STEP_COPIES 8
+int mvd_step_prologue(void* zero, size_t zero_bytes, const int* iter, int ncopy, const float* const* src, float* const* dst, const int* n,
+                      const int* ld, mvd_stream_t stream);
 
 #define MVD_STEP_STRIDE 8
 int mvd_timestep_embedding(const float* steps, const int* iter, const float* freqs, float* out, int dim,
diff --git a/mvdfusion_amd/csrc/elementwise.hip b/mvdfusion_amd/csrc/elementwise.hip
--- a/mvdfusion_amd/csrc/elementwise.hip
+++ b/mvdfusion_amd/csrc/elementwise.hip
@@ -296,8 +296,90 @@
   }
 }
 
+struct PyramidOut {
+  u16* sp[3];
+  int ld[3];
+};
+
+__device__ __forceinline__ void add2(float2& a, const float2& v) {
+  a.x += v.x;
+  a.y += v.y;
+}
+
+__device__ __forceinline__ void store_sp2(u16* __restrict__ base, size_t row, int ld, int k, float a, float b) {
+  uint32_t h, l;
+  split_op16x2(a, b, h, l);
+  u16* p = base + sp_index(row, ld, k);
+  *(uint32_t*)p = h;
+  *(uint32_t*)(p + 32) = l;
+}
+
+__global__ __launch_bounds__(256) void area_pool_pyramid_kernel(const float2* __restrict__ vol, PyramidOut o, int B, int S, int D, int C2) {
+  const int S8 = S / 8, S4 = S / 4, S2 = S / 2;
+  const size_t total = (size_t)B * S8 * S8 * D * C2;
+  for (size_t e = (size_t)blockIdx.x * 256 + threadIdx.x; e < total; e += (size_t)gridDim.x * 256) {
+    const int c = (int)(e % C2);
+    size_t r = e / C2;
+    const int d = (int)(r % D);
+    r /= D;
+    const int wx = (int)(r % S8);
+    r /= S8;
+    const int wy = (int)(r % S8);
+    const int b = (int)(r / S8);
+    const float2 zero = make_float2(0.f, 0.f);
+    float2 a8 = zero, a4[2] = {zero, zero};
+#pragma unroll
+    for (int p = 0; p < 4; ++p) {
+      float2 v[16];
+#pragma unroll
+      for (int i = 0; i < 16; ++i)
+        v[i] = vol[((((size_t)b * S + wy * 8 + p * 2 + (i >> 3)) * S + wx * 8 + (i & 7)) * D + d) * C2 + c];
+      if ((p & 1) == 0) a4[0] = a4[1] = zero;
+      float2 a2[4] = {zero, zero, zero, zero};
+#pragma unroll
+      for (int i = 0; i < 16; ++i) {
+        add2(a2[(i & 7) >> 1], v[i]);
+        add2(a4[(i & 7) >> 2], v[i]);
+        add2(a8, v[i]);
+      }
+#pragma unroll
+      for (int j = 0; j < 4; ++j)
+        store_sp2(o.sp[0], (((size_t)b * S2 + wy * 4 + p) * S2 + wx * 4 + j) * D + d, o.ld[0], c * 2, a2[j].x * 0.25f, a2[j].y * 0.25f);
+      if ((p & 1) == 1) {
+#pragma unroll
+        for (int j = 0; j < 2; ++j)
+          store_sp2(o.sp[1], (((size_t)b * S4 + wy * 2 + (p >> 1)) * S4 + wx * 2 + j) * D + d, o.ld[1], c * 2, a4[j].x * 0.0625f,
+                    a4[j].y * 0.0625f);
+      }
+    }
+    store_sp2(o.sp[2], (((size_t)b * S8 + wy) * S8 + wx) * D + d, o.ld[2], c * 2, a8.x * 0.015625f, a8.y * 0.015625f);
+  }
+}
+
 __global__ __launch_bounds__(256) void fill_zero_kernel(float* p, size_t n) {
   for (size_t e = (size_t)blockIdx.x * 256 + threadIdx.x; e < n; e += (size_t)gridDim.x * 256) p[e] = 0.f;
+}
+
+struct StepCopies {
+  const float* src[MVD_STEP_COPIES];
+  float* dst[MVD_STEP_COPIES];
+  int n[MVD_STEP_COPIES];
+  int ld[MVD_STEP_COPIES];
+  int count;
+};
+
+__global__ __launch_bounds__(256) void step_prologue_kernel(uint4* __restrict__ zero, size_t nz, const int* __restrict__ iter, StepCopies cp) {
+  const size_t t = (size_t)blockIdx.x * 256 + threadIdx.x, stride = (size_t)gridDim.x * 256;
+  for (size_t e = t; e < nz; e += stride) zero[e] = make_uint4(0u, 0u, 0u, 0u);
+  const size_t it = (size_t)iter[0];
+#pragma unroll
+  for (int j = 0; j < MVD_STEP_COPIES; ++j) {
+    if (j < cp.count) {
+      const float* s = cp.src[j] + it * (size_t)cp.ld[j];
+      float* dst = cp.dst[j];
+      for (size_t e = t; e < (size_t)cp.n[j]; e += stride) dst[e] = s[e];
+    }
+  }
 }
 
 __global__ void timestep_embedding_kernel(const float* __restrict__ steps, const int* __restrict__ iter,
@@ -497,6 +579,46 @@
   if (n == 0) return 0;
   hipLaunchKernelGGL(fill_zero_kernel, dim3(grid_for(n)), dim3(256), 0, (hipStream_t)stream, p, n);
   MVD_CHECK_LAUNCH("mvd_fill_zero");
+  return 0;
+}
+
+extern "C" int mvd_area_pool_pyramid(const float* vol, void* const* out_sp, const int* ldp, int B, int S, int D, int C,
+                                     mvd_stream_t stream) {
+  MVD_CHECK_ARG(vol && out_sp && ldp && C % 32 == 0 && B > 0 && S > 0 && D > 0 && S % 8 == 0,
+                "mvd_area_pool_pyramid: bad arguments (S %% 8 == 0, C %% 32 == 0)");
+  PyramidOut o;
+  for (int i = 0; i < 3; ++i) {
+    MVD_CHECK_ARG(out_sp[i] && ldp[i] >= C && ldp[i] % 32 == 0 && ((uintptr_t)out_sp[i] & 127) == 0,
+                  "mvd_area_pool_pyramid: level %d: ldp=%d must be >= C, %% 32 == 0, planes 128-byte aligned", i + 1, ldp[i]);
+    o.sp[i] = (u16*)out_sp[i];
+    o.ld[i] = ldp[i];
+  }
+  const size_t total = (size_t)B * (S / 8) * (S / 8) * D * (C / 2);
+  hipLaunchKernelGGL(area_pool_pyramid_kernel, dim3(grid_for(total)), dim3(256), 0, (hipStream_t)stream, (const float2*)vol, o, B, S, D,
+                     C / 2);
+  MVD_CHECK_LAUNCH("mvd_area_pool_pyramid");
+  return 0;
+}
+
+extern "C" int mvd_step_prologue(void* zero, size_t zero_bytes, const int* iter, int ncopy, const float* const* src, float* const* dst,
+                                 const int* n, const int* ld, mvd_stream_t stream) {
+  MVD_CHECK_ARG(iter && ncopy >= 0 && ncopy <= MVD_STEP_COPIES && (ncopy == 0 || (src && dst && n && ld)),
+                "mvd_step_prologue: bad arguments (ncopy=%d, at most %d)", ncopy, MVD_STEP_COPIES);
+  MVD_CHECK_ARG((zero || zero_bytes == 0) && ((uintptr_t)zero & 15) == 0 && (zero_bytes & 15) == 0,
+                "mvd_step_prologue: the zeroed range must be 16-byte aligned and a multiple of 16 bytes");
+  StepCopies cp = {};
+  size_t most = zero_bytes / 16;
+  for (int j = 0; j < ncopy; ++j) {
+    MVD_CHECK_ARG(src[j] && dst[j] && n[j] > 0 && ld[j] >= n[j], "mvd_step_prologue: copy %d: n=%d, ld=%d", j, n[j], ld[j]);
+    cp.src[j] = src[j];
+    cp.dst[j] = dst[j];
+    cp.n[j] = n[j];
+    cp.ld[j] = ld[j];
+    if ((size_t)n[j] > most) most = (size_t)n[j];
+  }
+  cp.count = ncopy;
+  hipLaunchKernelGGL(step_prologue_kernel, dim3(grid_for(most)), dim3(256), 0, (hipStream_t)stream, (uint4*)zero, zero_bytes / 16, iter, cp);
+  MVD_CHECK_LAUNCH("mvd_step_prologue");
   return 0;
 }
 
diff --git a/mvdfusion_amd/engine.py b/mvdfusion_amd/engine.py
--- a/mvdfusion_amd/engine.py
+++ b/mvdfusion_amd/engine.py
@@ -51,6 +51,8 @@
     gn_from_producer = True
     ln_fold = True
     gn_fuse = True
+    step_tables = True
+    pool_pyramid = True
 
     def __init__(self, device, prec=hip.PREC_X4, policy=None):
         self.device = torch.device(device)
@@ -76,7 +78,7 @@
         self._cat_done = set()
         self.keep_fp32 = False
 
-    def begin_step(self):
+    def begin_step(self, zero_arena=True):
         self._rot.clear()
         self._gn.clear()
         self._gn_done.clear()
@@ -85,7 +87,7 @@
         self.next_gn = None
         self.next_cat = None
         self._gn_next = 0
-        if self.gn_from_producer:
+        if self.gn_from_producer and zero_arena:
             hip.check(hip.lib().mvd_fill_zero(hip.ptr(self.gn_arena), self.gn_arena.numel() * 2, hip.stream()))
 
     def gn_slot(self, out, B, HW, C):
diff --git a/mvdfusion_amd/hip.py b/mvdfusion_amd/hip.py
--- a/mvdfusion_amd/hip.py
+++ b/mvdfusion_amd/hip.py
@@ -135,6 +135,8 @@
     "mvd_groupnorm_from_stats": (_i, [_vp, _vp, _vp, _vp, _vp, _i, _i, _i, _i, _f, _i, _vp]),
     "mvd_area_pool": (_i, [_vp, _vp, _i, _i, _i, _i, _i, _i, _vp]),
     "mvd_fill_zero": (_i, [_vp, _sz, _vp]),
+    "mvd_area_pool_pyramid": (_i, [_vp, _vp, _vp, _i, _i, _i, _i, _vp]),
+    "mvd_step_prologue": (_i, [_vp, _sz, _vp, _i, _vp, _vp, _vp, _vp, _vp]),
     "mvd_pow2_scale": (_i, [_vp, _sz, _vp, _vp, _vp]),
     "mvd_split_planes_scaled": (_i, [_vp, _vp, _sz, _i, _i, _i, _vp, _vp]),
     "mvd_transpose_planes_scaled": (_i, [_vp, _i, _i, _i, _vp, _i, _vp, _vp]),
@@ -945,6 +947,25 @@
     return y
 
 
+def step_prologue(zero, it, copies):
+    k = len(copies)
+    src = (C.c_void_p * k)(*[t.data_ptr() for t, _ in copies])
+    dst = (C.c_void_p * k)(*[d.data_ptr() for _, d in copies])
+    n = (C.c_int * k)(*[d.numel() for _, d in copies])
+    ld = (C.c_int * k)(*[t.stride(0) for t, _ in copies])
+    for t, d in copies:
+        assert t.dtype == d.dtype == torch.float32 and t.stride(1) == 1 and d.is_contiguous() and t.shape[1] == d.numel(), (t.shape, d.shape)
+    nz = 0 if zero is None else zero.numel() * zero.element_size()
+    assert zero is None or (zero.is_contiguous() and zero.data_ptr() % 16 == 0 and nz % 16 == 0), (zero.shape, zero.dtype)
+    check(lib().mvd_step_prologue(ptr(zero), nz, ptr(it), k, src, dst, n, ld, stream()))
+
+
+def area_pool_pyramid(vol, outs, B, S, D, Cc):
+    sp = (C.c_void_p * 3)(*[o.data_ptr() + 4 * col for o, col, _ in outs])
+    ld = (C.c_int * 3)(*[l for _, _, l in outs])
+    check(lib().mvd_area_pool_pyramid(ptr(vol), sp, ld, B, S, D, Cc, stream()))
+
+
 def groupnorm(x, y, gamma, beta, B, HW, Cc, eps, silu, ws):
     check(lib().mvd_groupnorm_nhwc(ptr(x), ptr(y), ptr(gamma), ptr(beta), B, HW, Cc, 32, eps, int(silu), ptr(ws), ws.numel(),
                                    stream()))
diff --git a/mvdfusion_amd/unet.py b/mvdfusion_amd/unet.py
--- a/mvdfusion_amd/unet.py
+++ b/mvdfusion_amd/unet.py
@@ -242,7 +242,7 @@
     def _resblocks(self):
         return [m for m in self.modules() if isinstance(m, ResBlock)]
 
-    def time_biases(self, ctx, t_sin):
+    def _temb_packed(self):
         if self._temb is None:
             blocks = self._resblocks()
             w = torch.cat([b.emb_layers[1].weight.detach() for b in blocks], 0).contiguous()
@@ -252,17 +252,27 @@
                 offs[b] = (o, o + b.out_channels)
                 o += b.out_channels
             self._temb = (w, bias, offs)
-        w, bias, offs = self._temb
+        return self._temb
+
+    def time_biases(self, ctx, t_sin, table=None):
+        w, bias, offs = self._temb_packed()
         ted = self.model_channels * 4
         R = t_sin.shape[0]
         e1, emb = ctx.ws.get("temb.e1", (R, ted)), ctx.ws.get("temb.emb", (R, ted))
-        out = ctx.ws.get("temb.bias", (R, w.shape[0]))
+        out = ctx.ws.get("temb.bias", (R, w.shape[0])) if table is None else table
         ctx.gemv_rows(self.time_embed[0].weight, self.time_embed[0].bias, t_sin, e1, act_out=hip.ACT_SILU)
         ctx.gemv_rows(self.time_embed[2].weight, self.time_embed[2].bias, e1, emb)
         ctx.gemv_rows(w, bias, emb, out, act_in=hip.ACT_SILU)
+        if table is None:
+            ctx.emb_bias = {b: out[:, lo:hi] for b, (lo, hi) in offs.items()}
+
+    def bind_time_biases(self, ctx):
+        w, _, offs = self._temb_packed()
+        out = ctx.ws.get("temb.bias", (1, w.shape[0]))
         ctx.emb_bias = {b: out[:, lo:hi] for b, (lo, hi) in offs.items()}
-
-    def cross_attn_vectors(self, ctx):
+        return out
+
+    def _xattn_packed(self):
         if self._xattn is None:
             sts = [m for m in self.modules() if isinstance(m, SpatialTransformer)]
             ws, bs, offs, o = [], [], {}, 0
@@ -274,15 +284,22 @@
                 offs[st] = (o, o + st.in_channels)
                 o += st.in_channels
             self._xattn = (torch.cat(ws, 0).contiguous(), torch.cat(bs, 0).contiguous(), offs, o)
-        w, bias, offs, total = self._xattn
+        return self._xattn
+
+    def cross_attn_vectors(self, ctx, launch=True):
+        w, bias, offs, total = self._xattn_packed()
         out = ctx.ws.get("xattn.vec", (ctx.context.shape[0], total))
-        ctx.gemv_rows(w, bias, ctx.context, out)
+        if launch:
+            ctx.gemv_rows(w, bias, ctx.context, out)
         ctx.xattn_vec = {st: out[:, lo:hi] for st, (lo, hi) in offs.items()}
 
     def run(self, ctx, x_in, t_sin, S):
         B = ctx.B
-        self.time_biases(ctx, t_sin)
-        self.cross_attn_vectors(ctx)
+        if t_sin is None:
+            self.bind_time_biases(ctx)
+        else:
+            self.time_biases(ctx, t_sin)
+        self.cross_attn_vectors(ctx, launch=t_sin is not None)
         hs = []
         H = W = S
         h = x_in
@@ -387,6 +404,7 @@
         levels = [self.level0_operand(ctx, B, S, D)]
         Cc = vol.shape[-1]
         chans = self.level_channels()
+        lds = []
         for i in range(1, len(self.unet_model.channel_mult)):
             f = 2 ** i
             rows = B * (S // f) * (S // f) * D
@@ -396,6 +414,11 @@
             else:
                 ld, col = Cc, 0
                 o = ctx.ws.planes(f"vol{i}", rows, Cc)
-            hip.check(hip.lib().mvd_area_pool(hip.ptr(vol), hip.c_void_p(o.data_ptr() + 4 * col), B, S, D, Cc, f, ld, hip.stream()))
             levels.append((o, col))
+            lds.append(ld)
+        if ctx.pool_pyramid and len(levels) == 4 and S % 8 == 0:
+            hip.area_pool_pyramid(vol, [(o, col, ld) for (o, col), ld in zip(levels[1:], lds)], B, S, D, Cc)
+            return levels
+        for i, ((o, col), ld) in enumerate(zip(levels[1:], lds), start=1):
+            hip.check(hip.lib().mvd_area_pool(hip.ptr(vol), hip.c_void_p(o.data_ptr() + 4 * col), B, S, D, Cc, 2 ** i, ld, hip.stream()))
         return levels
diff --git a/mvdfusion_amd/view_attn_efficient2.py b/mvdfusion_amd/view_attn_efficient2.py
--- a/mvdfusion_amd/view_attn_efficient2.py
+++ b/mvdfusion_amd/view_attn_efficient2.py
@@ -224,8 +224,25 @@
         return (V >= 1 and 1 <= R <= 16 and (T // R * Vp) % 64 == 0 and T % R == 0 and self.hidden_size == 256 and len(blocks) == 3 and
                 all(b.num_heads == 8 and b.mlp.fc1.out_features == 512 for b in blocks))
 
+    def embed_input_latents(self, ctx, input_latents, N, S):
+        z = self.z_embedder[0]
+        in_feat = ctx.ws.get("ga.infeat", (N, S, S, 256))
+        hip.check(hip.lib().mvd_zembed(hip.ptr(input_latents), hip.ptr(z.weight), hip.ptr(z.bias), hip.ptr(in_feat), N, S, hip.stream()))
+
+    def adaln_table(self, ctx, c, out):
+        for bi, blk in enumerate(self.aggregation_transformer.layer_list):
+            lin = blk.adaLN_modulation[1]
+            ctx.gemv_rows(lin.weight, lin.bias, c, out[:, bi * 1536:(bi + 1) * 1536], act_in=hip.ACT_SILU)
+        return out
+
+    def adaln_slots(self, ctx):
+        vecs = self.packed_fused(ctx.device)[1]
+        return [((bi * 1536, (bi + 1) * 1536), vecs[bi * _G4_VEC_BLOCK:bi * _G4_VEC_BLOCK + 1536])
+                for bi in range(len(self.aggregation_transformer.layer_list))]
+
     def run(self, ctx, x, depth_noise, steps, it, cams_rec, in_cam_rec, input_latents, c, vol_out, V, S, D, q0=0, Vq=None,
-            vol_planes=None, vol_planes_col=0, fused=None, depth_src=None, depth_steps=None, scenes=1, steps_scene_stride=0):
+            vol_planes=None, vol_planes_col=0, fused=None, depth_src=None, depth_steps=None, scenes=1, steps_scene_stride=0,
+            hoisted=False):
         Vq = V if Vq is None else Vq
         N = int(scenes)
         L = hip.lib()
@@ -237,8 +254,9 @@
         feat = ctx.ws.get("ga.feat", (N * V, S, S, 256))
         in_feat = ctx.ws.get("ga.infeat", (N, S, S, 256))
         hip.check(L.mvd_zembed(hip.ptr(x), hip.ptr(z.weight), hip.ptr(z.bias), hip.ptr(feat), N * V, S, hip.stream()))
-        hip.check(L.mvd_zembed(hip.ptr(input_latents), hip.ptr(z.weight), hip.ptr(z.bias), hip.ptr(in_feat), N, S,
-                               hip.stream()))
+        if not hoisted:
+            hip.check(L.mvd_zembed(hip.ptr(input_latents), hip.ptr(z.weight), hip.ptr(z.bias), hip.ptr(in_feat), N, S,
+                                   hip.stream()))
         nseq = N * Vq * S * S * D
         W = self.window
         R = self.rows_per_point(V)
@@ -255,7 +273,7 @@
             fused = self.fused_supported(V, T // N)
         sst = int(steps_scene_stride)
         if sst:
-            assert N > 1 and c.shape[0] == N, (N, tuple(c.shape))
+            assert N > 1 and c.shape[0] == N and not hoisted, (N, tuple(c.shape), hoisted)
             if fused is False or not self.fused_supported(V, T // N):
                 raise NotImplementedError(f"GridAttn.run: per-scene timesteps need the fused aggregation kernel (V={V}, T={T // N} per scene); "
                                           "the unfused chain shares one adaLN modulation")
@@ -267,9 +285,10 @@
             vecs = vecs.view(1, nv)
             if sst:
                 vecs = ctx.ws.get("ga.vecs_scenes", (N, nv)).copy_(vecs.expand(N, nv))
-            for bi, blk in enumerate(self.aggregation_transformer.layer_list):
-                lin = blk.adaLN_modulation[1]
-                ctx.gemv_rows(lin.weight, lin.bias, c, vecs[:, bi * _G4_VEC_BLOCK:bi * _G4_VEC_BLOCK + 1536], act_in=hip.ACT_SILU)
+            if not hoisted:
+                for bi, blk in enumerate(self.aggregation_transformer.layer_list):
+                    lin = blk.adaLN_modulation[1]
+                    ctx.gemv_rows(lin.weight, lin.bias, c, vecs[:, bi * _G4_VEC_BLOCK:bi * _G4_VEC_BLOCK + 1536], act_in=hip.ACT_SILU)
             pool = ctx.ws.planes("ga.pool", nseq, self.hidden_size)
             hip.check(L.mvd_gridattn_fused_window(hip.ptr(dsrc), hip.ptr(depth_noise), hip.ptr(dsteps), hip.ptr(it), hip.ptr(grid_lin),
                                                   hip.ptr(feat), hip.ptr(in_feat), hip.ptr(cams_rec), hip.ptr(in_cam_rec), hip.ptr(stream),
diff --git a/mvdfusion_amd/viewfusion_zero_depth_rgb.py b/mvdfusion_amd/viewfusion_zero_depth_rgb.py
--- a/mvdfusion_amd/viewfusion_zero_depth_rgb.py
+++ b/mvdfusion_amd/viewfusion_zero_depth_rgb.py
@@ -65,6 +65,9 @@
         self.n_rows = 1
         self.steps_scene_stride = 0
         self.done = 0
+        self.schedule_per_scene = False
+        self._cond_stale = self._sched_stale = True
+        self._row0 = torch.zeros(1, dtype=torch.int32, device=dev)
 
     def set_conditioning(self, batch_cameras, input_latents, input_cameras, clip_v_embed):
         self.set_conditioning_scenes([(batch_cameras, input_latents, input_cameras, clip_v_embed)])
@@ -78,9 +81,11 @@
             self.in_cam[n:n + 1].copy_(pack_cameras(ic).to(self.cams.device))
             self.input_latents[n:n + 1].copy_(il.reshape(1, 5, S, S))
             self.clip_v_embed[n * V:(n + 1) * V].copy_(ce.reshape(V, 796))
+        self._cond_stale = True
 
     def set_schedule(self, steps_table, depth_noise, ddim_noise):
         self._set_tables(steps_table, depth_noise, ddim_noise, scene_stride=0)
+        self.schedule_per_scene = False
 
     def set_schedule_scenes(self, steps_table, depth_noise, ddim_noise=None):
         if self.cfg:
@@ -92,6 +97,7 @@
         if ddim_noise is None:
             ddim_noise = torch.zeros(1, self.N * self.V, 5, self.S, self.S)
         self._set_tables(steps_table, depth_noise, ddim_noise, scene_stride=1 if self.N > 1 else 0)
+        self.schedule_per_scene = True
 
     def _set_tables(self, steps_table, depth_noise, ddim_noise, scene_stride):
         dev = self.ctx.device
@@ -109,6 +115,7 @@
         self.steps_nodiv.copy_(self.steps)
         self.steps_nodiv[:, 1] = 1.0
         self.steps_scene_stride = scene_stride
+        self._sched_stale = True
         self.n_rows = int(steps_table.shape[0]) - (self.N - 1) * scene_stride
         self.rewind()
 
@@ -155,34 +162,37 @@
         V, S, D, B, q0, Vq, N = self.V, self.S, self.D, self.B, self.q0, self.Vq, self.N
         NVq = N * Vq
         ctx.B, ctx.D = B, D
-        ctx.begin_step()
+        tables = self.use_tables()
+        ctx.begin_step(zero_arena=not tables)
         st = hip.stream
         sst, R = self.steps_scene_stride, self.t_rows
         if sst and do_update:
             raise ValueError("StepEngine: per-scene timesteps (set_schedule_scenes) are a training step: no DDIM update")
+        if tables:
+            hip.step_prologue(ctx.gn_arena if ctx.gn_from_producer else None, self.iter, self._table_copies())
+        else:
+            self._cond_stale = self._sched_stale = True
         if self.pin is not None:
             mode, K = self.pin
             pn = self.pin_noise if mode == 1 else None
             hip.check(L.mvd_pin_views(hip.ptr(self.x), hip.ptr(self.x0), hip.ptr(self.known), hip.ptr(pn), N * K * 5 * S * S,
                                       hip.ptr(self.steps), hip.ptr(self.iter), N, V, K, S, mode, st()))
-        ts = ctx.ws.get("vf.tsin", (R, 256))
-        te1 = ctx.ws.get("vf.te1", (R, 256))
         c = ctx.ws.get("vf.c", (R, 256))
-        hip.check(L.mvd_timestep_embedding_scenes(hip.ptr(self.steps), hip.ptr(self.iter), hip.ptr(self.f256), hip.ptr(ts), 256, R, sst,
-                                                  st()))
-        ctx.gemv_rows(m.time_embed[0].weight, m.time_embed[0].bias, ts, te1, act_out=hip.ACT_SILU)
-        ctx.gemv_rows(m.time_embed[2].weight, m.time_embed[2].bias, te1, c)
+        if not tables:
+            ts = ctx.ws.get("vf.tsin", (R, 256))
+            te1 = ctx.ws.get("vf.te1", (R, 256))
+            hip.check(L.mvd_timestep_embedding_scenes(hip.ptr(self.steps), hip.ptr(self.iter), hip.ptr(self.f256), hip.ptr(ts), 256, R, sst,
+                                                      st()))
+            ctx.gemv_rows(m.time_embed[0].weight, m.time_embed[0].bias, ts, te1, act_out=hip.ACT_SILU)
+            ctx.gemv_rows(m.time_embed[2].weight, m.time_embed[2].bias, te1, c)
         dsrc, dsteps = self.depth_geo()
         m.view_attn.run(ctx, self.x, self.depth_noise, self.steps, self.iter, self.cams, self.in_cam,
                         self.input_latents, c, self.vol, V, S, D, q0=q0, Vq=Vq, vol_planes=self.vol_planes,
                         vol_planes_col=self.vol_col, depth_src=None if self.depth_mode == 0 else dsrc,
-                        depth_steps=None if self.depth_mode == 0 else dsteps, scenes=N, steps_scene_stride=sst)
-        p = m.cc_projection
-        c1 = ctx.ws.get("vf.cc1", (NVq, 768))
-        c2 = ctx.ws.get("vf.cc2", (NVq, 768))
-        ctx.gemv_rows(p[0].weight, p[0].bias, self.clip_v_embed[q0:q0 + NVq], c1, act_out=hip.ACT_SILU)
-        ctx.gemv_rows(p[2].weight, p[2].bias, c1, c2, act_out=hip.ACT_SILU)
-        ctx.gemv_rows(p[4].weight, p[4].bias, c2, self.context[:NVq])
+                        depth_steps=None if self.depth_mode == 0 else dsteps, scenes=N, steps_scene_stride=sst, hoisted=tables,
+                        fused=self._ga_fused() if tables else None)
+        if not tables:
+            self._project_clip()
         if self.drop_masks is not None:
             clip_m, vol_m, cat_m = self.drop_masks
             self.context[:NVq] *= clip_m[:, None]
@@ -200,9 +210,11 @@
             xin[:NVq, :, 37:42] *= cm
         unet = m.unet_model.unet_model
         ctx.vol_levels = m.unet_model.volume_pyramid(ctx, self.vol.view(B, S, S, D, 768), B, S, D)
-        tsu = ctx.ws.get("vf.tsin_unet", (R, unet.model_channels))
-        hip.check(L.mvd_timestep_embedding_scenes(hip.ptr(self.steps), hip.ptr(self.iter), hip.ptr(self.funet), hip.ptr(tsu),
-                                                  unet.model_channels, R, sst, st()))
+        tsu = None
+        if not tables:
+            tsu = ctx.ws.get("vf.tsin_unet", (R, unet.model_channels))
+            hip.check(L.mvd_timestep_embedding_scenes(hip.ptr(self.steps), hip.ptr(self.iter), hip.ptr(self.funet), hip.ptr(tsu),
+                                                      unet.model_channels, R, sst, st()))
         y = unet.run(ctx, self.x_in, tsu, S)
         hip.check(L.mvd_cfg_ddim_update(hip.ptr(y), 8, hip.ptr(xq), hip.ptr(x0q), hip.ptr(epsq),
                                         hip.ptr(self.ddim_noise[:, q0:q0 + NVq]), N * V * 5 * S * S, hip.ptr(self.steps),
@@ -210,17 +222,76 @@
         if do_update:
             hip.check(L.mvd_advance_iter(hip.ptr(self.iter), st()))
 
+    def _project_clip(self):
+        p, ctx, NVq = self.m.cc_projection, self.ctx, self.N * self.Vq
+        c1 = ctx.ws.get("vf.cc1", (NVq, 768))
+        c2 = ctx.ws.get("vf.cc2", (NVq, 768))
+        ctx.gemv_rows(p[0].weight, p[0].bias, self.clip_v_embed[self.q0:self.q0 + NVq], c1, act_out=hip.ACT_SILU)
+        ctx.gemv_rows(p[2].weight, p[2].bias, c1, c2, act_out=hip.ACT_SILU)
+        ctx.gemv_rows(p[4].weight, p[4].bias, c2, self.context[:NVq])
+
+    def use_tables(self):
+        return bool(self.ctx.step_tables and not self.schedule_per_scene and self.steps_scene_stride == 0 and self.drop_masks is None and
+                    not self.ctx.keep_fp32)
+
+    def _ga_fused(self):
+        va = self.m.view_attn
+        return va.fused_supported(self.V, self.Vq * self.S * self.S * self.D * va.rows_per_point(self.V))
+
+    def _schedule_tables(self):
+        ws, unet, n = self.ctx.ws, self.m.unet_model.unet_model, int(self.steps.shape[0])
+        width = unet._temb_packed()[0].shape[0]
+        return (ws.get("tab.c", (n, 256)), ws.get("tab.adaln", (n, 3 * 1536)) if self._ga_fused() else None,
+                ws.get("tab.temb", (n, width)))
+
+    def _table_copies(self):
+        ctx, unet = self.ctx, self.m.unet_model.unet_model
+        c_tab, ada_tab, temb_tab = self._schedule_tables()
+        cp = [(temb_tab, unet.bind_time_biases(ctx)[0])]
+        if ada_tab is None:
+            cp.append((c_tab, ctx.ws.get("vf.c", (1, 256))[0]))
+        else:
+            cp += [(ada_tab[:, lo:hi], dst) for (lo, hi), dst in self.m.view_attn.adaln_slots(ctx)]
+        return cp
+
+    def fill_tables(self):
+        m, ctx, L, st = self.m, self.ctx, hip.lib(), hip.stream
+        unet = m.unet_model.unet_model
+        if self._cond_stale:
+            self._project_clip()
+            ctx.context = self.context
+            unet.cross_attn_vectors(ctx)
+            m.view_attn.embed_input_latents(ctx, self.input_latents, self.N, self.S)
+            self._cond_stale = False
+        if self._sched_stale:
+            n = int(self.steps.shape[0])
+            c_tab, ada_tab, temb_tab = self._schedule_tables()
+            for freqs, dim, tag in ((self.f256, 256, "tab.tsin"), (self.funet, unet.model_channels, "tab.tsin_unet")):
+                hip.check(L.mvd_timestep_embedding_scenes(hip.ptr(self.steps), hip.ptr(self._row0), hip.ptr(freqs),
+                                                          hip.ptr(ctx.ws.get(tag, (n, dim))), dim, n, 1 if n > 1 else 0, st()))
+            te1 = ctx.ws.get("tab.te1", (n, 256))
+            ctx.gemv_rows(m.time_embed[0].weight, m.time_embed[0].bias, ctx.ws.get("tab.tsin", (n, 256)), te1, act_out=hip.ACT_SILU)
+            ctx.gemv_rows(m.time_embed[2].weight, m.time_embed[2].bias, te1, c_tab)
+            if ada_tab is not None:
+                m.view_attn.adaln_table(ctx, c_tab, ada_tab)
+            unet.time_biases(ctx, ctx.ws.get("tab.tsin_unet", (n, unet.model_channels)), table=temb_tab)
+            self._sched_stale = False
+
     @property
     def t_rows(self):
         return self.N if self.steps_scene_stride else 1
 
     def step(self, cfg_scale, do_update, use_graph=True):
-        key = (float(cfg_scale), bool(do_update), int(self.depth_mode), self.steps_scene_stride, self.pin)
+        tables = self.use_tables()
+        key = (float(cfg_scale), bool(do_update), int(self.depth_mode), self.steps_scene_stride, self.pin, tables,
+               bool(self.ctx.pool_pyramid))
         if self.done >= self.n_rows:
             raise IndexError(f"StepEngine.step: iteration {self.done} is past the {self.n_rows}-row step table "
                              "(set_schedule() / rewind() before stepping again)")
         if do_update:
             self.done += 1
+        if tables:
+            self.fill_tables()
         if not use_graph:
             return self.enqueue(cfg_scale, do_update)
         g = self.graphs.get(key)
@@ -371,6 +442,7 @@
             for e in self._engines.values():
                 e.graphs.clear()
                 e.prefetchers.clear()
+                e._cond_stale = e._sched_stale = True
         else:
             self._engines.clear()
 
```
